# slyforce/MusicStyleTransfer

Hardware: AMD Instinct MI355X
Metric: piano-roll frames/s (VAE train step) (higher is better)
Workload: dtype bf16; 1 GPU; BASELINE configs[1]: single-track piano-roll VAE train step, T=256, pitch=128, latent=64, batch=64/GPU, bf16; encoder 256x2x8h, decoder 128x1x8h (scripts/train-vae.sh), dropout 0.2; Xavier-initialised weights; global_batch=64, seq_len=256, pitches=128, latent=64, parallelism=dp1, params=1885440

## Files before the change

### include/mst_hip.h

```cpp
#ifndef MST_HIP_H
#define MST_HIP_H

#include <stdint.h>

#ifdef __cplusplus
extern "C" {
#endif

typedef void* mst_stream_t;

enum mst_status {
  MST_OK = 0,
  MST_ERR_INVALID = -1,
  MST_ERR_LAUNCH = -2,
  MST_ERR_UNSUPPORTED = -3
};

enum mst_dtype { MST_BF16 = 0, MST_F16 = 1, MST_F32 = 2 };

enum mst_act { MST_ACT_NONE = 0, MST_ACT_RELU = 1 };

int mst_version(void);
const char* mst_last_error(void);

int mst_graph_begin(mst_stream_t stream);
int mst_graph_end(mst_stream_t stream, void** graph_exec_out);
int mst_graph_end_counted(mst_stream_t stream, void** graph_exec_out, int32_t* nodes_out, int32_t* kernel_nodes_out);
int mst_graph_launch(void* graph_exec, mst_stream_t stream);
int mst_graph_destroy(void* graph_exec);

int mst_event_create(void** ev_out);
int mst_event_record(void* ev, mst_stream_t stream);
int mst_event_sync(void* ev);
int mst_event_elapsed_ms(void* ev_start, void* ev_stop, float* ms_out);
int mst_event_destroy(void* ev);

typedef struct mst_gemm_args {
  int32_t dtype;
  int32_t c_f32;
  int64_t M, N, K;
  const void* A; int64_t lda;
  const void* B; int64_t ldb;
  void* C; int64_t ldc;
  const float* bias;
  const void* resid; int64_t ldr;
  int32_t act;
  const void* gate; int64_t ldg;
  float alpha;
  const float* rowadd; int64_t ldra; int64_t rowadd_period;
  const float* grpadd; int64_t ldga; const int32_t* grp_index;
  int64_t a_rows_per_group, a_group_stride, a_group_offset;
  int64_t c_rows_per_group, c_group_stride, c_group_offset;
  float dropout_p; uint64_t dropout_seed; uint32_t dropout_site;
  int32_t self_resid;
  const uint64_t* dropout_seed_ptr;
  int32_t a_u8;
  int32_t resid_phys;
} mst_gemm_args;

int mst_gemm_nt(const mst_gemm_args* args, mst_stream_t stream);
int mst_gemm_nt_form(const mst_gemm_args* args);

int mst_gemm_nt_pair(const mst_gemm_args* args0, const mst_gemm_args* args1, mst_stream_t stream);

typedef struct mst_bce_args {
  const uint8_t* labels;
  int64_t T;
  float label_smoothing;
  int32_t downweight;
  float* loss;
  void* probs; int64_t ldp;
  void* logits; int64_t ldl;
  float gscale;
  uint64_t* counts;
} mst_bce_args;
#define MST_ROLL_SLOTS 256
int mst_gemm_sigmoid_bce(const mst_gemm_args* args, const mst_bce_args* bce, mst_stream_t stream);

typedef struct mst_ln_args {
  int32_t mode;
  const float* gamma;
  const float* beta;
  float eps;
  void* out; int64_t ld_out;
  float* mean; float* rstd;
  const void* x; int64_t ld_x;
  float* dgamma; float* dbeta;
  int32_t mask_mode;
  float* partials;
} mst_ln_args;

int mst_gemm_nt_ln(const mst_gemm_args* args, const mst_ln_args* ln, mst_stream_t stream);
int mst_gemm_sigmoid_bce_dgrad_ln(const mst_gemm_args* args, const mst_bce_args* bce, const mst_gemm_args* dgrad,
                                  const mst_ln_args* ln, mst_stream_t stream);
int64_t mst_gemm_nt_ln_parts(int64_t M);
int mst_gemm_sigmoid_bce_form(const mst_gemm_args* args, const mst_bce_args* bce, const mst_gemm_args* dgrad, const mst_ln_args* ln,
                              int64_t* form);

int mst_ffn_ln_fwd(const mst_gemm_args* ff1, const mst_gemm_args* ff2, const mst_ln_args* ln, mst_stream_t stream);
int mst_ffn_ln_bwd(const mst_gemm_args* ff2_dgrad, const mst_gemm_args* ff1_dgrad, const mst_ln_args* ln, mst_stream_t stream);
typedef struct mst_ln_bwd_in {
  const void* dy; int64_t ld_dy;
  const void* x;  int64_t ld_x;
  const float* gamma; const float* mean; const float* rstd;
  void* dx; int64_t ld_dx;
  void* dx_masked; int64_t ld_dxm;
  float* dgamma; float* dbeta; float* partials;
  int32_t mask_mode;
  float dropout_p; uint64_t dropout_seed; const uint64_t* dropout_seed_ptr; uint32_t dropout_site;
} mst_ln_bwd_in;
int mst_ffn_ln_bwd_lead(const mst_ln_bwd_in* lead, const mst_gemm_args* ff2_dgrad, const mst_gemm_args* ff1_dgrad,
                        const mst_ln_args* ln, mst_stream_t stream);
int mst_proj_ffn_ln_fwd(const mst_gemm_args* proj, const mst_ln_args* ln1, const mst_gemm_args* ff1, const mst_gemm_args* ff2,
                        const mst_ln_args* ln2, mst_stream_t stream);
int mst_dec_tail_step(const mst_gemm_args* proj, const mst_ln_args* ln1, const mst_gemm_args* ff1, const mst_gemm_args* ff2,
                      const mst_ln_args* ln3, const mst_gemm_args* out, const mst_bce_args* bce, const mst_gemm_args* out_dgrad,
                      const mst_ln_args* ln3_bwd, const mst_gemm_args* ff2_dgrad, const mst_gemm_args* ff1_dgrad,
                      const mst_ln_args* ln1_bwd, mst_stream_t stream);

typedef struct mst_partial_sum {
  const float* src; int64_t n_parts; int64_t stride; int64_t len;
  float* dst; float scale;
} mst_partial_sum;
int mst_partial_sums(const mst_partial_sum* jobs, int n, mst_stream_t stream);

typedef struct mst_wgrad_args {
  int32_t dtype;
  int64_t M, N, K;
  const void* A; int64_t lda;
  const void* B; int64_t ldb;
  float* dW; int64_t ldw;
  float* db;
  float scale;
  int64_t a_rows_per_group, a_group_stride, a_group_offset;
  int64_t b_rows_per_group, b_group_stride, b_group_offset;
  int32_t a_u8;
} mst_wgrad_args;

typedef struct mst_outer_job {
  const float* L; const void* R; int32_t r_dtype; int64_t r_stride;
  int64_t B, J, I;
  float* out; float* obias;
} mst_outer_job;
int mst_outer_jobs(const mst_outer_job* jobs, int n, mst_stream_t stream);
int mst_gemm_wgrad_batch_flush(const mst_wgrad_args* list, int n, float* scratch, int64_t scratch_bytes,
                               const mst_partial_sum* sums, int n_sums, const mst_outer_job* outers, int n_outers,
                               mst_stream_t stream);
int mst_class_table_grad(const int32_t* classes, const float* tvec, float* dcls, int64_t ld_cls, int64_t B, int64_t Dd,
                         mst_stream_t stream);
int mst_gemm_wgrad_batch_flush_cls(const mst_wgrad_args* list, int n, float* scratch, int64_t scratch_bytes,
                                   const mst_partial_sum* sums, int n_sums, const mst_outer_job* outers, int n_outers,
                                   const int32_t* cls_classes, const float* cls_tvec, float* cls_dcls, int64_t cls_ld,
                                   int64_t cls_B, int64_t cls_Dd, mst_stream_t stream);
int mst_gemm_wgrad_plan(const mst_wgrad_args* list, int n, int64_t scratch_bytes, int64_t* plan);

int mst_embed_fwd(int dtype, int64_t B, int64_t T, int64_t D,
                  const int32_t* tokens, const float* table, int64_t ldt,
                  const int32_t* classes, const float* cls_table, int64_t ldc,
                  const float* pos, int64_t ldp, float alpha,
                  void* out, int64_t ld_out, int64_t S_out, int64_t s_off,
                  uint8_t* keymask, mst_stream_t stream);

int mst_embed_bwd(int dtype, int64_t B, int64_t T, int64_t D,
                  const int32_t* tokens, float* dtable, int64_t ldt,
                  const int32_t* classes, float* dcls, int64_t ldc, float alpha,
                  const void* dX, int64_t ld_dx, int64_t S_out, int64_t s_off,
                  mst_stream_t stream);

int mst_group_colsum(int dtype, int64_t B, int64_t T, int64_t D, const void* X, int64_t ldx,
                     int64_t S_out, int64_t s_off, const int32_t* idx, float* dst, int64_t ldd,
                     float alpha, mst_stream_t stream);

int mst_mask_from_lengths(int64_t B, int64_t S, const int32_t* lens, int32_t add,
                          uint8_t* keymask, mst_stream_t stream);

int mst_attn_keysoftmax_fwd(int dtype, int64_t B, int64_t S, int64_t H, int64_t dh,
                            const void* qkv, int64_t ld_qkv, int64_t k_off, int64_t q_off, int64_t v_off,
                            const uint8_t* keymask, float* lse,
                            void* out, int64_t ld_out,
                            int64_t q_limit ,
                            mst_stream_t stream);

int mst_attn_qkv_fwd(int dtype, int64_t B, int64_t S, int64_t H, int64_t dh, const void* x, int64_t ld_x, const void* w,
                     int64_t ld_w, const float* bias, void* qkv, int64_t ld_qkv, int64_t k_off, int64_t q_off, int64_t v_off,
                     const uint8_t* keymask, float* lse, void* out, int64_t ld_out, int64_t q_limit, mst_stream_t stream);
int mst_attn_keysoftmax_bwd(int dtype, int64_t B, int64_t S, int64_t H, int64_t dh,
                            const void* qkv, int64_t ld_qkv, int64_t k_off, int64_t q_off, int64_t v_off,
                            const uint8_t* keymask, const float* lse,
                            const void* dout, int64_t ld_dout,
                            void* dqkv, int64_t ld_dqkv, float* delta,
                            int64_t q_limit ,
                            mst_stream_t stream);
int mst_attn_proj_bwd(int dtype, int64_t B, int64_t S, int64_t H, int64_t dh, const void* qkv, int64_t ld_qkv, int64_t k_off,
                      int64_t q_off, int64_t v_off, const uint8_t* keymask, const float* lse, const void* dproj, int64_t ld_dproj,
                      const void* wt, int64_t ld_wt, void* dout_out, int64_t ld_dout, void* dqkv, int64_t ld_dqkv, float* delta,
                      mst_stream_t stream);

int mst_attn_fwd_form(int dtype, int64_t B, int64_t S, int64_t H, int64_t dh, int64_t ld_qkv, int64_t k_off, int64_t q_off,
                      int64_t v_off, int64_t ld_out, int64_t q_limit, int fused, int64_t ld_x, int64_t ld_w, int64_t* form);
int mst_attn_bwd_form(int dtype, int64_t B, int64_t S, int64_t H, int64_t dh, int64_t ld_qkv, int64_t k_off, int64_t q_off,
                      int64_t v_off, int64_t ld_dout, int64_t ld_dqkv, int64_t q_limit, int64_t* form);

int mst_attn_causal_fwd(int dtype, int64_t B, int64_t S, int64_t H, int64_t dh,
                        const void* qkv, int64_t ld_qkv, int64_t k_off, int64_t q_off, int64_t v_off,
                        const uint8_t* keymask, float* lse, void* out, int64_t ld_out, mst_stream_t stream);
int mst_attn_causal_bwd(int dtype, int64_t B, int64_t S, int64_t H, int64_t dh,
                        const void* qkv, int64_t ld_qkv, int64_t k_off, int64_t q_off, int64_t v_off,
                        const uint8_t* keymask, const float* lse, const void* dout, int64_t ld_dout,
                        void* dqkv, int64_t ld_dqkv, float* delta, mst_stream_t stream);

int mst_layernorm_fwd(int dtype, int64_t M, int64_t D, const void* x, int64_t ldx,
                      const float* gamma, const float* beta, float eps,
                      void* y, int64_t ldy, float* mean, float* rstd,
                      int64_t row_id_stride ,
                      mst_stream_t stream);

int mst_layernorm_bwd(int dtype, int64_t M, int64_t D, const void* x, int64_t ldx,
                      const float* gamma, const float* mean, const float* rstd,
                      const void* dy, int64_t ldy, void* dx, int64_t ld_dx,
                      void* dx_masked, int64_t ld_dxm, float* dgamma, float* dbeta,
                      int mask_mode, float dropout_p, uint64_t dropout_seed, uint32_t dropout_site,
                      const uint64_t* dropout_seed_ptr,
                      int64_t row_id_stride ,
                      float* partials ,
                      mst_stream_t stream);
int64_t mst_layernorm_bwd_parts(int64_t M, int64_t D);

int mst_latent_fwd(int dtype, int64_t B, int64_t De, int64_t Z, int64_t Dd,
                   const void* enc_out, int64_t enc_sample_stride,
                   const float* Wl, const float* bl, const float* eps,
                   const float* Wh, const float* bh,
                   const int32_t* classes, const float* cls_d, int64_t ld_cls,
                   const float* pos_d, float alpha_d,
                   float* mu, float* sigma, float* z, float* kl,
                   void* dec_in, int64_t dec_sample_stride, mst_stream_t stream);
int mst_latent_fwd_proj(int dtype, int64_t B, int64_t De, int64_t Z, int64_t Dd,
                        const void* enc_out, int64_t enc_sample_stride,
                        const float* Wl, const float* bl, const float* eps,
                        const float* Wh, const float* bh,
                        const int32_t* classes, const float* cls_d, int64_t ld_cls,
                        const float* pos_d, float alpha_d,
                        float* mu, float* sigma, float* z, float* kl,
                        void* dec_in, int64_t dec_sample_stride,
                        const void* Wq, int64_t ld_wq, const float* bq, void* qkv0, int64_t qkv_sample_stride, int64_t nq,
                        mst_stream_t stream);
int mst_latent_rows(int dtype, int64_t N, int64_t M, int64_t Z, int64_t Dd,
                    const float* zsrc, const float* ssrc, const int32_t* a, const int32_t* b, const float* w, int mode,
                    float tau, uint64_t seed, const uint64_t* seed_ptr, uint32_t site, int64_t row0,
                    const float* Wh, const float* bh,
                    const int32_t* ca, const int32_t* cb, const float* cw, const float* cls_d, int64_t ld_cls, int64_t n_classes,
                    const float* pos_d, float alpha_d,
                    float* z_out, void* dec_in, int64_t dec_stride, mst_stream_t stream);

int mst_latent_bwd_vec(int dtype, int64_t B, int64_t De, int64_t Z, int64_t Dd, const float* Wl, const float* eps, const float* Wh,
                       const int32_t* classes, const float* mu, const float* sigma, const void* d_dec_in, int64_t dec_sample_stride,
                       float alpha_d, float kl_weight, float gscale, float enc_scale, float* dcls_d, int64_t ld_cls,
                       void* d_enc_out, int64_t denc_sample_stride, float* scratch, mst_stream_t stream);
int mst_latent_bwd_vec_proj(int dtype, int64_t B, int64_t De, int64_t Z, int64_t Dd, const float* Wl, const float* eps, const float* Wh,
                            const int32_t* classes, const float* mu, const float* sigma,
                            const void* dq0, int64_t dq_sample_stride, const void* Wt, int64_t ld_wt, int64_t nq,
                            const void* resid0, int64_t resid_sample_stride,
                            float alpha_d, float kl_weight, float gscale, float enc_scale, float* dcls_d, int64_t ld_cls,
                            void* d_enc_out, int64_t denc_sample_stride, float* scratch, mst_stream_t stream);

int mst_latent_bwd_vec_sched(int dtype, int64_t B, int64_t De, int64_t Z, int64_t Dd, const float* Wl, const float* eps, const float* Wh,
                             const int32_t* classes, const float* mu, const float* sigma, const void* d_dec_in, int64_t dec_sample_stride,
                             float alpha_d, const float* sched, const float* kl, float gscale, float enc_scale, float* dcls_d,
                             int64_t ld_cls, void* d_enc_out, int64_t denc_sample_stride, float* scratch, mst_stream_t stream);
int mst_latent_bwd_vec_proj_sched(int dtype, int64_t B, int64_t De, int64_t Z, int64_t Dd, const float* Wl, const float* eps,
                                  const float* Wh, const int32_t* classes, const float* mu, const float* sigma,
                                  const void* dq0, int64_t dq_sample_stride, const void* Wt, int64_t ld_wt, int64_t nq,
                                  const void* resid0, int64_t resid_sample_stride,
                                  float alpha_d, const float* sched, const float* kl, float gscale, float enc_scale, float* dcls_d,
                                  int64_t ld_cls, void* d_enc_out, int64_t denc_sample_stride, float* scratch, mst_stream_t stream);

int mst_latent_form(int64_t De, int64_t Z, int64_t Dd, int64_t nq, const void* Wl, int64_t* form);

int mst_reparam_kl_fwd(int64_t B, int64_t Z, const float* mu, const float* sigma, const float* eps,
                       float* z, float* kl, mst_stream_t stream);
int mst_reparam_kl_bwd(int64_t B, int64_t Z, const float* mu, const float* sigma, const float* eps,
                       const float* dz, float kl_weight, float* dmu, float* dsigma, mst_stream_t stream);

typedef struct mst_row_tail_args {
  int32_t dtype;
  int64_t B, D;
  const void* att; int64_t rs_att;
  const void* resid; int64_t rs_res;
  const void* Wp; int64_t ldwp; const float* bp;
  const float* g1; const float* be1;
  const void* W1; int64_t ldw1; const float* b1;
  const void* W2; int64_t ldw2; const float* b2;
  const float* g2; const float* be2;
  void* h1; void* x1; void* h2; void* x2; int64_t rs_d;
  void* a; int64_t rs_a;
  float* mean1; float* rstd1; float* mean2; float* rstd2; int64_t stat_stride;
  float eps;
  float dropout_p; uint64_t dropout_seed; const uint64_t* dropout_seed_ptr; uint32_t site0;
  int64_t phys_stride;
  uint32_t* sync;
  uint32_t* status;
} mst_row_tail_args;
int mst_row_tail_fwd(const mst_row_tail_args* args, mst_stream_t stream);
int mst_row_tail_fwd_ride(const mst_row_tail_args* args, const mst_gemm_args* rider, uint32_t* queue, mst_stream_t stream);
int mst_row_tail_fwd_ride_shadows(const mst_row_tail_args* args, const mst_gemm_args* rider, uint32_t* queue, int sh_dtype,
                                  const float* sh_w, void* sh_wt16, const int64_t* sh_desc, const int64_t* sh_prefix, int64_t sh_n_mat,
                                  int64_t sh_tiles, mst_stream_t stream);
typedef struct mst_row_tail_bwd_args {
  int32_t dtype;
  int64_t B, D;
  const void* dy; int64_t rs_dy;
  const void* h2; const void* h1; int64_t rs_d;
  const void* a; int64_t rs_a;
  const float* mean1; const float* rstd1; const float* mean2; const float* rstd2; int64_t stat_stride;
  const float* g1; const float* g2;
  const void* W2t; int64_t ldw2t;
  const void* W1t; int64_t ldw1t;
  const void* Wpt; int64_t ldwpt;
  void* dh; void* dhm; void* dx1; void* dh1m; int64_t rs_c;
  void* dpre; int64_t rs_dpre;
  void* dh1; int64_t rs_dh1;
  void* datt; int64_t rs_datt;
  float* dg1; float* db1; float* dg2; float* db2;
  float dropout_p; uint64_t dropout_seed; const uint64_t* dropout_seed_ptr; uint32_t site0;
  int64_t phys_stride;
  uint32_t* sync;
  uint32_t* status;
} mst_row_tail_bwd_args;
int mst_row_tail_bwd(const mst_row_tail_bwd_args* args, mst_stream_t stream);
int mst_row_tail_bwd_ride(const mst_row_tail_bwd_args* args, const mst_gemm_args* rider, uint32_t* queue, mst_stream_t stream);
int mst_row_tail_form(int backward, int dtype, int64_t D, const mst_gemm_args* rider, int64_t sh_tiles, int64_t* form);

int mst_attn_decode(int dtype, int64_t B, int64_t H, int64_t dh, int64_t n_keys, int64_t t_max, const void* cache,
                    int64_t ld, int64_t k_off, int64_t q_off, int64_t v_off, int mode, void* out, int64_t ld_out,
                    mst_stream_t stream);

int mst_beam_step(int64_t B, int64_t K, int64_t V, int64_t i, int64_t L, const float* probs, int64_t ldp, const float* scores_in,
                  float* scores_out, const int32_t* seqs_in, int32_t* seqs_out, int32_t* hyp_src, int32_t* word, int32_t* active,
                  int32_t eos, int32_t pad, mst_stream_t stream);
int mst_beam_gather(const void* in, void* out, const int32_t* src, int64_t N, int64_t n_rows, int64_t row_bytes, int64_t t_max,
                    mst_stream_t stream);
int mst_beam_gather_cols(const void* in, void* out, const int32_t* src, int64_t N, int64_t n_rows, int64_t row_bytes, int64_t t_max,
                         int64_t skip_begin, int64_t skip_bytes, mst_stream_t stream);
int mst_sample_step(int64_t N, int64_t V, int64_t i, int64_t L, const float* probs, int64_t ldp, int32_t* seqs, float* scores,
                    int32_t* word, int32_t* active, uint64_t seed, int32_t eos, int32_t pad, mst_stream_t stream);
int mst_frame_step(int dtype, int64_t N, int64_t P, int64_t i, int64_t L, const void* logits, int64_t ldl, float tau, int mode, float thr,
                   const uint64_t* seed_ptr, uint8_t* frames, int64_t ldf, uint8_t* roll, int64_t ldr, float* scores, float* probs_out,
                   mst_stream_t stream);
int mst_token_step(int dtype, int64_t N, int64_t V, int64_t i, int64_t L, const void* logits, int64_t ldl, float tau, int32_t top_k,
                   float top_p, const uint64_t* seed_ptr, int32_t* seqs, float* scores, int32_t* word, int32_t* active,
                   int32_t* kept_out, int32_t eos, int32_t pad, mst_stream_t stream);

#define MST_CE_MAX_WORKGROUPS 4096
int mst_softmax_ce(int dtype, int64_t B, int64_t T, int64_t V,
                   const void* logits, int64_t ld, const int32_t* labels,
                   float* loss, float* probs, int64_t ldp,
                   void* dlogits, int64_t ldd, float gscale,
                   int pre_zeroed ,
                   float* tok_parts, int top_k, mst_stream_t stream);

int mst_ce_from_probs(int dtype, int64_t B, int64_t T, int64_t V, const void* probs, int64_t ldp,
                      const int32_t* labels, float* loss, mst_stream_t stream);
int mst_bce_from_probs(int dtype, int64_t B, int64_t n_per_sample, const void* probs, const uint8_t* labels,
                       float label_smoothing, int downweight, float* loss, mst_stream_t stream);

int mst_sigmoid_bce(int dtype, int64_t B, int64_t T, int64_t P,
                    const void* logits, int64_t ld, const uint8_t* labels,
                    float label_smoothing, int downweight, int32_t* npos,
                    float* loss, void* probs, int64_t ldp,
                    void* dlogits, int64_t ldd, float gscale,
                    int pre_zeroed , mst_stream_t stream);
int mst_sigmoid_bce_counts(int dtype, int64_t B, int64_t T, int64_t P,
                           const void* logits, int64_t ld, const uint8_t* labels,
                           float label_smoothing, int downweight, int32_t* npos,
                           float* loss, void* probs, int64_t ldp,
                           void* dlogits, int64_t ldd, float gscale,
                           int pre_zeroed, uint64_t* counts, mst_stream_t stream);
int mst_sigmoid_bce_form(int dtype, int64_t B, int64_t T, int64_t P,
                         const void* logits, int64_t ld, const uint8_t* labels,
                         float label_smoothing, int downweight, int32_t* npos,
                         float* loss, void* probs, int64_t ldp,
                         void* dlogits, int64_t ldd, float gscale,
                         int pre_zeroed, int64_t* form);

int mst_loss_combine(int64_t B, const float* recon, const float* kl, float kl_weight,
                     float* total, float* metric_acc, mst_stream_t stream);

typedef struct mst_step_metrics {
  int64_t B; const float* recon; const float* kl; float kl_weight; float* total; float* metric;
  uint32_t* status; const uint32_t* expect_ptr0; uint32_t expect_val0; const uint32_t* expect_ptr1; uint32_t expect_val1;
  const float* fin_recon; const float* fin_kl; int64_t fin_B;
} mst_step_metrics;
#define MST_TAIL_SPIN_FWD 1u
#define MST_TAIL_SPIN_BWD 2u
#define MST_STEP_INCOMPLETE 16u
int mst_adam_flat(int dtype, int64_t n, float* w, const float* grad, float* m, float* v,
                  void* w16, double lr, double beta1, double beta2, float eps, float wd,
                  float rescale, float clip, int32_t* step_state ,
                  int advance_step ,
                  const mst_step_metrics* metrics, mst_stream_t stream);
int mst_loss_combine_v(const mst_step_metrics* metrics, mst_stream_t stream);

int mst_adam_flat_emb(int dtype, int64_t n, float* w, const float* grad, float* m, float* v, void* w16, double lr, double beta1,
                      double beta2, float eps, float wd, float rescale, float clip, int32_t* step_state,
                      const mst_step_metrics* metrics, int64_t base, const int64_t* emb, int64_t n_emb, void* wt16, mst_stream_t stream);

int mst_adam_flat_sched(int dtype, int64_t n, float* w, const float* grad, float* m, float* v, void* w16, double lr, double beta1,
                        double beta2, float eps, float wd, float rescale, float clip, int32_t* step_state,
                        const mst_step_metrics* metrics, const float* sched, mst_stream_t stream);
int mst_adam_flat_emb_sched(int dtype, int64_t n, float* w, const float* grad, float* m, float* v, void* w16, double lr, double beta1,
                            double beta2, float eps, float wd, float rescale, float clip, int32_t* step_state,
                            const mst_step_metrics* metrics, const float* sched, int64_t base, const int64_t* emb, int64_t n_emb,
                            void* wt16, mst_stream_t stream);

int64_t mst_grad_sumsq_parts(void);
int mst_grad_sumsq(int64_t n, const float* grad, int64_t cut, float rescale_lo, float rescale_hi, float* parts, mst_stream_t stream);
// ... 46 lines not shown
```

### musicstyletransfer_amd/csrc/ffn_ln.hip

```cpp
#include "ffn_ln.hpp"
#include "gemm_checks.hpp"

namespace mst {

template <typename T, int BN, int WGM, int WGN, int MODE, bool LEAD, bool FULL, bool EXTRA = false>
__global__ __launch_bounds__(WGM * WGN * 64) void ffn_ln_kernel(mst_gemm_args g1, mst_gemm_args g2, mst_ln_args ln, mst_ln_bwd_in lead,
                                                                mst_gemm_args gx, mst_ln_args lnx) {
  extern __shared__ __attribute__((aligned(16))) unsigned char smem[];
  ffn_ln_body<T, BN, WGM, WGN, MODE, LEAD, FULL, EXTRA>(smem, g1, g2, ln, lead, gx, lnx, nullptr, [] {});
}

template <typename T, int BN>
static int launch_ffn_ln(const mst_gemm_args& g1, const mst_gemm_args& g2, const mst_ln_args& ln, const mst_ln_bwd_in* lead, hipStream_t s,
                         const mst_gemm_args* gx = nullptr, const mst_ln_args* lnx = nullptr) {
  constexpr int BM = 64;
  const int ex = gx ? 1 : 0;
  const size_t lds_loop = (size_t)2 * BN * 64 * 2 + (size_t)2 * BM * (BN + 8) * 2 + (size_t)g1.N * 4 + (size_t)6 * BN * 4;
  const size_t lds_epi = (size_t)BM * (BN + 4) * 4;
  const size_t lds = lds_loop > lds_epi ? lds_loop : lds_epi;
  const int full = g1.M % BM == 0 ? 1 : 0;
  const int mi = ex ? 6 + full : (lead ? 2 : (ln.mode == 2 ? 1 : 0)) * 2 + full;
  typedef void (*kern_t)(mst_gemm_args, mst_gemm_args, mst_ln_args, mst_ln_bwd_in, mst_gemm_args, mst_ln_args);
  const kern_t fns[8] = {&ffn_ln_kernel<T, BN, 2, 4, 1, false, false>, &ffn_ln_kernel<T, BN, 2, 4, 1, false, true>,
                         &ffn_ln_kernel<T, BN, 2, 4, 2, false, false>, &ffn_ln_kernel<T, BN, 2, 4, 2, false, true>,
                         &ffn_ln_kernel<T, BN, 2, 4, 2, true, false>, &ffn_ln_kernel<T, BN, 2, 4, 2, true, true>,
                         &ffn_ln_kernel<T, BN, 2, 4, 1, false, false, true>, &ffn_ln_kernel<T, BN, 2, 4, 1, false, true, true>};
  static size_t granted[8] = {64 * 1024, 64 * 1024, 64 * 1024, 64 * 1024, 64 * 1024, 64 * 1024, 64 * 1024, 64 * 1024};
  if (const int rc = lds_opt_in(reinterpret_cast<const void*>(fns[mi]), lds, &granted[mi], "ffn_ln_kernel")) return rc;
  const mst_ln_bwd_in none = {};
  const mst_gemm_args no_gemm = {};
  const mst_ln_args no_ln = {};
  hipLaunchKernelGGL(fns[mi], dim3((unsigned)cdiv(g1.M, BM)), dim3(512), lds, s, g1, g2, ln, lead ? *lead : none,
                     gx ? *gx : no_gemm, lnx ? *lnx : no_ln);
  MST_CHECK_LAUNCH("ffn_ln_kernel");
  return MST_OK;
}

int check_ffn_ln(const char* who, const mst_gemm_args* first, const mst_gemm_args* second, const mst_ln_args* ln, int mode,
                 const mst_ln_bwd_in* lead, const mst_gemm_args* extra, const mst_ln_args* extra_ln) {
  MST_CHECK_ARG(first != nullptr && second != nullptr && ln != nullptr, "%s: null args", who);
  const mst_gemm_args& a = *first;
  const mst_gemm_args& b = *second;
  const mst_ln_args& l = *ln;
  int rc = check_gemm_common(a);
  if (rc) return rc;
  rc = check_gemm_common(b);
  if (rc) return rc;
  MST_CHECK_ARG(a.dtype == b.dtype && a.M == b.M, "%s: the two GEMMs must share dtype and M", who);
  MST_CHECK_ARG((b.N == 256 || b.N == 128) && a.K == b.N, "%s: the model width (first K = second N) must be 128 or 256 (got %lld, %lld)", who,
                (long long)a.K, (long long)b.N);
  MST_CHECK_ARG(a.N == b.K && a.N % b.N == 0, "%s: the hidden width (first N = second K) must be a multiple of the model width", who);
  MST_CHECK_ARG(b.A == a.C && b.lda == a.ldc, "%s: the second GEMM's A operand must be the first one's output (it is consumed on chip)", who);
  MST_CHECK_ARG(!a.c_f32 && !b.c_f32 && !b.gate && !a.rowadd && !b.rowadd && !a.grpadd && !b.grpadd && !a.resid && !a.self_resid &&
                b.act == MST_ACT_NONE && a.c_rows_per_group <= 0 && b.a_rows_per_group <= 0 && b.c_rows_per_group <= 0,
                "%s: fp32 outputs, row-indexed adds, row remaps, a gate or activation on the second GEMM and a residual on the first are not supported", who);
  MST_CHECK_ARG(a.a_rows_per_group <= 0 || (a.a_rows_per_group % 64 == 0 && a.M % a.a_rows_per_group == 0 && a.a_group_offset >= 0 &&
                                            a.a_group_stride >= a.a_rows_per_group + a.a_group_offset && a.M < (1ll << 31)),
                "%s: row groups must be whole 64-row tiles (rows per group %lld, stride %lld, offset %lld, M %lld)", who,
                (long long)a.a_rows_per_group, (long long)a.a_group_stride, (long long)a.a_group_offset, (long long)a.M);
  MST_CHECK_ARG(a.lda % 8 == 0 && a.ldc % 8 == 0 && a.ldc >= a.N && b.ldc % 8 == 0 && b.ldc >= b.N, "%s: leading dimensions must be multiples of 8", who);
  MST_CHECK_ARG((uint64_t)a.N * (uint64_t)a.ldb < (1ull << 32) && (uint64_t)b.N * (uint64_t)b.ldb < (1ull << 32), "%s: weight matrices too large", who);
  MST_CHECK_ARG(!b.resid || (b.ldr % 8 == 0 && b.ldr >= b.N && (uintptr_t)b.resid % 16 == 0), "%s: bad residual layout", who);
  MST_CHECK_ARG(!a.bias || (uintptr_t)a.bias % 16 == 0, "%s: the first GEMM's bias must be 16-byte aligned", who);
  MST_CHECK_ARG(a.dropout_p == 0.f || a.N % 4 == 0, "%s: dropout needs widths that are multiples of 4", who);
  MST_CHECK_ARG(l.mode == mode && l.gamma && l.mean && l.rstd, "%s: LayerNorm arguments of the wrong form", who);
  if (mode == 1) {
    MST_CHECK_ARG(!a.gate, "%s: a gate belongs to the backward form", who);
    MST_CHECK_ARG(l.beta && l.out && l.ld_out % 8 == 0 && l.ld_out >= b.N && (uintptr_t)l.out % 16 == 0,
                  "%s: the LayerNorm arguments are those of mst_gemm_nt_ln's forward form", who);
  } else {
    MST_CHECK_ARG(a.gate && a.ldg % 8 == 0 && a.ldg >= a.N && (uintptr_t)a.gate % 16 == 0, "%s: the first GEMM needs the forward activation as its gate", who);
    MST_CHECK_ARG(a.act == MST_ACT_NONE && a.dropout_p == 0.f && !b.self_resid, "%s: activation / dropout / self_resid belong to the forward form", who);
    MST_CHECK_ARG(l.x && l.ld_x % 8 == 0 && (uintptr_t)l.x % 16 == 0 && (l.partials || (l.dgamma && l.dbeta)) && (uintptr_t)l.partials % 16 == 0,
                  "%s: backward needs x and dgamma + dbeta (or partials)", who);
    MST_CHECK_ARG(l.mask_mode >= 0 && l.mask_mode <= 2 &&
                  (l.mask_mode != 1 || (l.out && l.ld_out % 8 == 0 && l.ld_out >= b.N && (uintptr_t)l.out % 16 == 0)),
                  "%s: mask_mode must be 0, 1 (with out) or 2", who);
  }
  if (lead) {
    const mst_ln_bwd_in& q = *lead;
    MST_CHECK_ARG(mode == 2, "%s: a leading LayerNorm belongs to the backward form", who);
    MST_CHECK_ARG(q.dy && q.x && q.gamma && q.mean && q.rstd && q.dx && (q.partials || (q.dgamma && q.dbeta)), "%s: leading LayerNorm: null pointer", who);
    MST_CHECK_ARG(q.ld_dy % 8 == 0 && q.ld_x % 8 == 0 && q.ld_dx % 8 == 0 && q.ld_dy >= b.N && q.ld_x >= b.N && q.ld_dx >= b.N &&
                  ((uintptr_t)q.dy | (uintptr_t)q.x | (uintptr_t)q.dx | (uintptr_t)q.partials) % 16 == 0, "%s: leading LayerNorm: bad layout", who);
    MST_CHECK_ARG(q.mask_mode == 0 || (q.mask_mode == 1 && q.dx_masked && q.ld_dxm % 8 == 0 && q.ld_dxm >= b.N && (uintptr_t)q.dx_masked % 16 == 0),
                  "%s: leading LayerNorm: mask_mode must be 0 or 1 (with dx_masked)", who);
    MST_CHECK_ARG(q.dropout_p >= 0.f && q.dropout_p < 1.f, "%s: leading LayerNorm: dropout_p must be in [0,1)", who);
    const void* tile = q.mask_mode == 1 ? q.dx_masked : q.dx;
    const int64_t tile_ld = q.mask_mode == 1 ? q.ld_dxm : q.ld_dx;
    MST_CHECK_ARG(a.A == tile && a.lda == tile_ld, "%s: the first GEMM's A operand must be the leading LayerNorm's (masked) output", who);
  }
  if (extra) {
    const mst_gemm_args& x = *extra;
    rc = check_gemm_common(x);
    if (rc) return rc;
    MST_CHECK_ARG(x.dtype == a.dtype && x.M == a.M && x.N == b.N && x.K == b.N, "%s: the extra GEMM is width x width on the same rows", who);
    MST_CHECK_ARG(!x.c_f32 && !x.gate && !x.rowadd && !x.grpadd && x.act == MST_ACT_NONE && x.a_rows_per_group <= 0 && x.c_rows_per_group <= 0 &&
                  x.ldc % 8 == 0 && x.ldc >= x.N && (uint64_t)x.N * (uint64_t)x.ldb < (1ull << 32),
                  "%s: the extra GEMM takes no gate, activation, row-indexed add or row remap", who);
    MST_CHECK_ARG(mode == 1 && extra_ln != nullptr, "%s: the projection (with its LayerNorm) rides in front of the forward form", who);
    const mst_ln_args& q = *extra_ln;
    MST_CHECK_ARG(q.mode == 1 && q.gamma && q.beta && q.mean && q.rstd && q.out == a.A && q.ld_out == a.lda,
                  "%s: the leading LayerNorm's output must be the first GEMM's A operand", who);
    MST_CHECK_ARG(!x.resid || (x.ldr % 8 == 0 && x.ldr >= x.N && (uintptr_t)x.resid % 16 == 0), "%s: bad residual layout", who);
  }
  return MST_OK;
}

}

using namespace mst;

static int ffn_ln_impl(const char* who, const mst_gemm_args* first, const mst_gemm_args* second, const mst_ln_args* ln, int mode,
                       mst_stream_t stream, const mst_ln_bwd_in* lead = nullptr, const mst_gemm_args* extra = nullptr,
                       const mst_ln_args* extra_ln = nullptr) {
  const int rc = check_ffn_ln(who, first, second, ln, mode, lead, extra, extra_ln);
  if (rc) return rc;
  const mst_gemm_args &a = *first, &b = *second;
  const mst_ln_args& l = *ln;
  hipStream_t s = (hipStream_t)stream;
  return dispatch_act(a.dtype, [&](auto tag) -> int {
    typedef decltype(tag) T;
    if (b.N == 256) return launch_ffn_ln<T, 256>(a, b, l, lead, s, extra, extra_ln);
    return launch_ffn_ln<T, 128>(a, b, l, lead, s, extra, extra_ln);
  });
}

extern "C" int mst_proj_ffn_ln_fwd(const mst_gemm_args* proj, const mst_ln_args* ln1, const mst_gemm_args* ff1, const mst_gemm_args* ff2,
                                   const mst_ln_args* ln2, mst_stream_t stream) {
  MST_CHECK_ARG(proj != nullptr && ln1 != nullptr, "mst_proj_ffn_ln_fwd: null args");
  return ffn_ln_impl("mst_proj_ffn_ln_fwd", ff1, ff2, ln2, 1, stream, nullptr, proj, ln1);
}

extern "C" int mst_ffn_ln_bwd_lead(const mst_ln_bwd_in* lead, const mst_gemm_args* ff2_dgrad, const mst_gemm_args* ff1_dgrad,
                                   const mst_ln_args* ln, mst_stream_t stream) {
  MST_CHECK_ARG(lead != nullptr, "mst_ffn_ln_bwd_lead: null args");
  return ffn_ln_impl("mst_ffn_ln_bwd_lead", ff2_dgrad, ff1_dgrad, ln, 2, stream, lead);
}

extern "C" int mst_ffn_ln_fwd(const mst_gemm_args* ff1, const mst_gemm_args* ff2, const mst_ln_args* ln, mst_stream_t stream) {
  return ffn_ln_impl("mst_ffn_ln_fwd", ff1, ff2, ln, 1, stream);
}
extern "C" int mst_ffn_ln_bwd(const mst_gemm_args* ff2_dgrad, const mst_gemm_args* ff1_dgrad, const mst_ln_args* ln, mst_stream_t stream) {
  return ffn_ln_impl("mst_ffn_ln_bwd", ff2_dgrad, ff1_dgrad, ln, 2, stream);
}

#ifdef MST_FFN_STAMPS
extern "C" int mst_debug_ffn_stamps(uint64_t* host_out) {
  return hipMemcpyFromSymbol(host_out, HIP_SYMBOL(mst::g_ffn_stamps), sizeof(uint64_t) * (8 + 48 * 4)) == hipSuccess ? 0 : -1;
}
#endif
```

### musicstyletransfer_amd/csrc/ffn_ln.hpp

```cpp
#pragma once
#include <type_traits>
#include "gemm_ln.hpp"

namespace mst {

template <typename T, int BN, int WGM, int WGN, int MODE, bool LEAD, bool FULL, bool EXTRA, bool X_IN_LDS = false, bool KEEP_OUT = false,
          bool PAR_READY = false, typename Hook>
__device__ __forceinline__ void ffn_ln_body(unsigned char* smem, mst_gemm_args g1, mst_gemm_args g2, const mst_ln_args ln,
                                            const mst_ln_bwd_in lead, mst_gemm_args gx, const mst_ln_args lnx, float* par,
                                            Hook&& before_epilogue) {
  constexpr bool HEAD = EXTRA;
  static_assert(!(X_IN_LDS && (LEAD || EXTRA)), "a tile left in LDS is the block's own input");
  static_assert(!EXTRA || MODE == 1, "the extra GEMM is the forward form's head");
  constexpr int BM = 64, BK = 64, CHUNKS = BK / 8;
  constexpr int NT = WGM * WGN * 64;
  constexpr int WTM = BM / WGM, WTN = BN / WGN, TM = WTM / 16, TN = WTN / 16;
  constexpr int B_CH = BN * CHUNKS / NT;
  constexpr int LDA = BN + 8;
  constexpr int KST = BN / BK;
  static_assert(BN * CHUNKS % NT == 0 && (BM * BN / 8) % NT == 0, "tile/threads mismatch");
  typedef typename Act<T>::vec8 vec8;
  u32x4* sB = reinterpret_cast<u32x4*>(smem);
  T* sH = reinterpret_cast<T*>(smem + (size_t)2 * BN * BK * 2);
  T* sX = sH + BM * LDA;
  float* sBias1 = PAR_READY ? par : reinterpret_cast<float*>(sX + BM * LDA);
  float* sPar = sBias1 + g1.N;
  const int tid = threadIdx.x, lane = tid & 63, wave = tid >> 6;
  const int wm = wave / WGN, wn = wave % WGN, frow = lane & 15, fq = lane >> 4;
  int64_t m0 = xcd_chunk(blockIdx.x, gridDim.x) * BM;
  if (g1.a_rows_per_group > 0) {
    const uint32_t grp = (uint32_t)m0 / (uint32_t)g1.a_rows_per_group;
    m0 += (int64_t)grp * (g1.a_group_stride - g1.a_rows_per_group) + g1.a_group_offset;
    g1.M = g2.M = gx.M = (g1.M / g1.a_rows_per_group) * g1.a_group_stride;
  }
  const int64_t F = g1.N;
  FFN_STAMP(0); FFN_RT(190);
  const int64_t Mg = FULL ? (int64_t)1 << 62 : g1.M;
  if constexpr (!PAR_READY)
  for (int i = tid * 4; i < (int)F; i += NT * 4)
    *reinterpret_cast<f32x4*>(sBias1 + i) = g1.bias ? *reinterpret_cast<const f32x4*>(g1.bias + i) : f32x4{0.f, 0.f, 0.f, 0.f};
  const uint64_t seed2 = g2.dropout_seed ^ ((g2.dropout_p > 0.f && g2.dropout_seed_ptr) ? g2.dropout_seed_ptr[0] : 0ull);
  const uint64_t seedx = EXTRA ? gx.dropout_seed ^ ((gx.dropout_p > 0.f && gx.dropout_seed_ptr) ? gx.dropout_seed_ptr[0] : 0ull) : 0ull;
  if constexpr (!PAR_READY)
  for (int i = tid; i < BN; i += NT) {
    sPar[i] = g2.bias ? g2.bias[i] : 0.f;
    sPar[BN + i] = ln.gamma[i];
    sPar[2 * BN + i] = (MODE == 1) ? ln.beta[i] : 0.f;
    if constexpr (HEAD) {
      sPar[3 * BN + i] = gx.bias ? gx.bias[i] : 0.f;
      sPar[4 * BN + i] = lnx.gamma[i];
      sPar[5 * BN + i] = lnx.beta[i];
    }
  }
  const int n_chunks = (int)(F / BN);
  const int rot = (int)((blockIdx.x / 8) % (unsigned)n_chunks);
  auto phys = [&](int c) { const int pc = c + rot; return pc >= n_chunks ? pc - n_chunks : pc; };
  const T* __restrict__ W1 = reinterpret_cast<const T*>(g1.B);
  const T* __restrict__ W2 = reinterpret_cast<const T*>(g2.B);
  const T* __restrict__ WX = reinterpret_cast<const T*>(gx.B);

  uint32_t off1[B_CH], off2[B_CH], offx[B_CH];
  int b_lds[B_CH];
#pragma unroll
  for (int i = 0; i < B_CH; ++i) {
    const int c = tid + i * NT;
    const int row = c / CHUNKS, ch = c % CHUNKS;
    off1[i] = (uint32_t)row * (uint32_t)g1.ldb + (uint32_t)ch * 8u;
    off2[i] = (uint32_t)row * (uint32_t)g2.ldb + (uint32_t)ch * 8u;
    offx[i] = EXTRA ? (uint32_t)row * (uint32_t)gx.ldb + (uint32_t)ch * 8u : 0u;
    b_lds[i] = row * CHUNKS + (ch ^ (row & 7));
  }
  constexpr int SPC = 2 * KST;
  constexpr int RING = BN >= 256 ? 4 : 2, AHEAD = RING - 1;
  static_assert(SPC % RING == 0, "ring slots must repeat per chunk");
  u32x4 ring[RING][B_CH];
  auto load_stage = [&](int c, int s, u32x4 (&rb)[B_CH]) {
    if (HEAD && c < 0) {
      const T* base = WX + s * BK;
#pragma unroll
      for (int i = 0; i < B_CH; ++i) rb[i] = *reinterpret_cast<const u32x4*>(base + offx[i]);
    } else if (s < KST) {
      const T* base = W1 + (int64_t)phys(c) * BN * g1.ldb + s * BK;
#pragma unroll
      for (int i = 0; i < B_CH; ++i) rb[i] = *reinterpret_cast<const u32x4*>(base + off1[i]);
    } else {
      const T* base = W2 + (int64_t)phys(c) * BN + (s - KST) * BK;
#pragma unroll
      for (int i = 0; i < B_CH; ++i) rb[i] = *reinterpret_cast<const u32x4*>(base + off2[i]);
    }
  };
  auto load_piece = [&](int c, int s, u32x4 (&rb)[B_CH], auto ic) {
    constexpr int i = decltype(ic)::value;
    const T* base;
    uint32_t off;
    if (HEAD && c < 0) { base = WX + s * BK; off = offx[i]; }
    else if (s < KST) { base = W1 + (int64_t)phys(c) * BN * g1.ldb + s * BK; off = off1[i]; }
    else { base = W2 + (int64_t)phys(c) * BN + (s - KST) * BK; off = off2[i]; }
    rb[i] = *reinterpret_cast<const u32x4*>(base + off);
  };
  auto store_stage = [&](int buf, const u32x4 (&rb)[B_CH]) {
#pragma unroll
    for (int i = 0; i < B_CH; ++i) sB[buf * BN * CHUNKS + b_lds[i]] = rb[i];
  };
  {
    auto pro = [&](auto jc) {
      constexpr int j = decltype(jc)::value;
      if constexpr (HEAD) {
        static_assert(!HEAD || AHEAD <= KST, "the head GEMM's stages cover the prologue");
        if (j < AHEAD) load_stage(-1, j, ring[j % RING]);
      } else {
        if (j < AHEAD && (j < SPC || n_chunks > 1)) load_stage(j / SPC, j % SPC, ring[j % RING]);
      }
    };
    pro(std::integral_constant<int, 0>()); pro(std::integral_constant<int, 1>()); pro(std::integral_constant<int, 2>());
    pro(std::integral_constant<int, 3>()); pro(std::integral_constant<int, 4>()); pro(std::integral_constant<int, 5>());
    pro(std::integral_constant<int, 6>());
    static_assert(AHEAD <= 7, "the prologue list covers seven stages");
  }
  if constexpr (LEAD) {
    constexpr int CPR = BN / 8, RSTEP = NT / CPR, ITERS = BM / RSTEP;
    const int ch = tid % CPR, nc = ch * 8, row0 = tid / CPR;
    const float inv_n = 1.f / (float)BN;
    const bool has_drop = lead.dropout_p > 0.f && lead.mask_mode == 1;
    const uint64_t dseed = lead.dropout_seed ^ ((has_drop && lead.dropout_seed_ptr) ? lead.dropout_seed_ptr[0] : 0ull);
    const uint32_t dkey = dropout_key(dseed, lead.dropout_site), dthr = dropout_thr(lead.dropout_p);
    const float inv_keep = dropout_inv_keep(lead.dropout_p);
    float gam8[8], dg8[8], db8[8];
#pragma unroll
    for (int e = 0; e < 8; ++e) { gam8[e] = lead.gamma[nc + e]; dg8[e] = 0.f; db8[e] = 0.f; }
    u32x4 dyv[ITERS], xv[ITERS];
    float mean_r[ITERS], rstd_r[ITERS];
#pragma unroll
    for (int it = 0; it < ITERS; ++it) {
      const int64_t m = m0 + row0 + it * RSTEP;
      dyv[it] = u32x4{0u, 0u, 0u, 0u}; xv[it] = dyv[it]; mean_r[it] = 0.f; rstd_r[it] = 0.f;
      if (m < Mg) {
        dyv[it] = *reinterpret_cast<const u32x4*>(reinterpret_cast<const T*>(lead.dy) + m * lead.ld_dy + nc);
        xv[it] = *reinterpret_cast<const u32x4*>(reinterpret_cast<const T*>(lead.x) + m * lead.ld_x + nc);
        mean_r[it] = lead.mean[m];
        rstd_r[it] = lead.rstd[m];
      }
    }
#pragma unroll
    for (int it = 0; it < ITERS; ++it) {
      const int row = row0 + it * RSTEP;
      const int64_t m = m0 + row;
      Pack8 db, xb;
      db.u = dyv[it]; xb.u = xv[it];
      float xh[8], g[8], s1 = 0.f, s2 = 0.f;
#pragma unroll
      for (int e = 0; e < 8; ++e) {
        const float d = bits_to_f32<T>(db.h[e]);
        xh[e] = (bits_to_f32<T>(xb.h[e]) - mean_r[it]) * rstd_r[it];
        g[e] = d * gam8[e];
        s1 += g[e];
        s2 += g[e] * xh[e];
        dg8[e] += d * xh[e];
        db8[e] += d;
      }
      s1 = row_sum<CPR>(s1) * inv_n;
      s2 = row_sum<CPR>(s2) * inv_n;
      uint32_t keep8 = 0xFFu;
      if (has_drop) {
        const uint64_t w = (uint64_t)(m * BN + nc) >> 2;
        keep8 = dropout_keep4k(dkey, w, dthr) | (dropout_keep4k(dkey, w + 1, dthr) << 4);
      }
      Pack8 ob, mb;
#pragma unroll
      for (int e = 0; e < 8; ++e) {
        const float o = rstd_r[it] * (g[e] - s1 - xh[e] * s2);
        const float k = has_drop ? (((keep8 >> e) & 1u) ? inv_keep : 0.f) : 1.f;
        ob.h[e] = f32_to_bits<T>(o);
        mb.h[e] = f32_to_bits<T>(o * k);
      }
      if (m < Mg) {
        *reinterpret_cast<u32x4*>(reinterpret_cast<T*>(lead.dx) + m * lead.ld_dx + nc) = ob.u;
        if (lead.mask_mode == 1) *reinterpret_cast<u32x4*>(reinterpret_cast<T*>(lead.dx_masked) + m * lead.ld_dxm + nc) = mb.u;
      }
      *reinterpret_cast<u32x4*>(sX + row * LDA + nc) = (m < Mg) ? (lead.mask_mode == 1 ? mb.u : ob.u) : u32x4{0u, 0u, 0u, 0u};
    }
    float* red = reinterpret_cast<float*>(smem);
    static_assert((size_t)2 * RSTEP * BN * 4 <= (size_t)2 * BN * BK * 2, "reduction scratch must fit the weight stages");
#pragma unroll
    for (int e = 0; e < 8; ++e) {
      red[row0 * BN + nc + e] = dg8[e];
      red[(RSTEP + row0) * BN + nc + e] = db8[e];
    }
    __syncthreads();
    for (int c = tid; c < 2 * BN; c += NT) {
      const int which = c / BN, col = c % BN;
      float sm = 0.f;
      for (int r = 0; r < RSTEP; ++r) sm += red[(which * RSTEP + r) * BN + col];
      if (lead.partials) lead.partials[(int64_t)blockIdx.x * 2 * BN + c] = sm;
      else atomicAdd((which ? lead.dbeta : lead.dgamma) + col, sm);
    }
    __syncthreads();
  } else if constexpr (!X_IN_LDS)
  {
    const T* X = reinterpret_cast<const T*>(HEAD ? gx.A : g1.A);
    const int64_t ldx = HEAD ? gx.lda : g1.lda;
    constexpr int CPR = BN / 8;
#pragma unroll
    for (int i = 0; i < BM * CPR / NT; ++i) {
      const int c = tid + i * NT, row = c / CPR, ch = c % CPR;
      u32x4 v = {0u, 0u, 0u, 0u};
      if (m0 + row < Mg) v = *reinterpret_cast<const u32x4*>(X + (m0 + row) * ldx + ch * 8);
      *reinterpret_cast<u32x4*>(sX + row * LDA + ch * 8) = v;
    }
  }
  auto mma_stage = [&](f32x4 (&acc)[TN][TM], const T* sA, int buf, const u32x4 (&rb)[B_CH], auto&& hook) {
    const u32x4* cB = sB + buf * BN * CHUNKS;
#pragma unroll
    for (int ks = 0; ks < BK / 32; ++ks) {
      vec8 xf[TM], wf[TN];
      const int kc = ks * 4 + fq;
#pragma unroll
      for (int i = 0; i < TM; ++i)
        xf[i] = __builtin_bit_cast(vec8, *reinterpret_cast<const u32x4*>(sA + (wm * WTM + i * 16 + frow) * LDA + kc * 8));
#pragma unroll
      for (int j = 0; j < TN; ++j) {
        const int row = wn * WTN + j * 16 + frow;
        wf[j] = __builtin_bit_cast(vec8, cB[row * CHUNKS + (kc ^ (row & 7))]);
      }
      auto row = [&](auto jc) {
        constexpr int j = decltype(jc)::value;
        if constexpr (j < TN) {
#pragma unroll
          for (int i = 0; i < TM; ++i) acc[j][i] = Act<T>::mfma16(wf[j], xf[i], acc[j][i]);
          if (ks == 0) hook(std::integral_constant<int, j>()); else hook(std::integral_constant<int, TN + j>());
        }
      };
      static_assert(TN <= 4, "row list");
      row(std::integral_constant<int, 0>()); row(std::integral_constant<int, 1>());
      row(std::integral_constant<int, 2>()); row(std::integral_constant<int, 3>());
    }
  };
  auto no_hook = [](auto) {};

  f32x4 acc1[TN][TM], acc2[TN][TM];
#pragma unroll
  for (int j = 0; j < TN; ++j)
#pragma unroll
    for (int i = 0; i < TM; ++i) acc2[j][i] = f32x4{0.f, 0.f, 0.f, 0.f};
  const float p1 = g1.dropout_p;
  const bool drop1 = MODE == 1 && p1 > 0.f;
  const uint64_t seed1 = g1.dropout_seed ^ ((drop1 && g1.dropout_seed_ptr) ? g1.dropout_seed_ptr[0] : 0ull);
  const uint32_t dkey1 = dropout_key(seed1, g1.dropout_site), dthr1 = dropout_thr(p1);
  const float inv_keep1 = dropout_inv_keep(p1);
  const bool idx32 = (uint64_t)g1.M * (uint64_t)F < (1ull << 32);
  const bool relu1 = MODE == 1 && g1.act == MST_ACT_RELU;
  const bool step_form1 = MODE == 1 && relu1 && drop1 && idx32 && g1.alpha == 1.f;
  uint32_t rowmul[TM];
#pragma unroll
  for (int i = 0; i < TM; ++i) rowmul[i] = (uint32_t)(m0 + wm * WTM + i * 16 + frow) * (uint32_t)(F >> 1) * DROPOUT_MUL;
  T* Aout = reinterpret_cast<T*>(g1.C);

  auto extra_gemm = [&](int cx) {
#pragma unroll
    for (int j = 0; j < TN; ++j)
#pragma unroll
      for (int i = 0; i < TM; ++i) acc1[j][i] = f32x4{0.f, 0.f, 0.f, 0.f};
    store_stage(0, ring[0]);
    __syncthreads();
    auto xstage = [&](auto sc) {
      constexpr int s = decltype(sc)::value;
      if constexpr (s < KST) {
        constexpr int t = s + AHEAD;
        if constexpr (t < KST) load_stage(cx, t, ring[t % RING]);
        else if constexpr (HEAD) load_stage(0, t - KST, ring[t % RING]);
        mma_stage(acc1, sX + s * BK, s & 1, ring[s % RING], no_hook);
        if constexpr (s + 1 < KST) store_stage((s + 1) & 1, ring[(s + 1) % RING]);
        __syncthreads();
      }
    };
    static_assert(!EXTRA || (KST <= 4 && KST % RING == 0), "the extra GEMM stage list / ring slots");
    xstage(std::integral_constant<int, 0>()); xstage(std::integral_constant<int, 1>());
    xstage(std::integral_constant<int, 2>()); xstage(std::integral_constant<int, 3>());
  };
  if constexpr (HEAD) {
    extra_gemm(-1);
    gemm_epilogue_ln<T, BM, BN, WGM, WGN, 1>(gx, lnx, smem, acc1, m0, nullptr, 0, sX, LDA, sPar + 3 * BN, &seedx);
    __syncthreads();
  }
  store_stage(0, ring[0]);
  __syncthreads();
  FFN_STAMP(1);
  for (int c = 0; c < n_chunks; ++c) {
    const int pc = phys(c);
#pragma unroll
    for (int j = 0; j < TN; ++j)
#pragma unroll
      for (int i = 0; i < TM; ++i) acc1[j][i] = f32x4{0.f, 0.f, 0.f, 0.f};
    constexpr int OUT_CH = BM * (BN / 8) / NT;
    u32x4 gv[OUT_CH];
    if constexpr (MODE == 2) {
      const T* G = reinterpret_cast<const T*>(g1.gate);
#pragma unroll
      for (int i = 0; i < OUT_CH; ++i) {
        const int cc = tid + i * NT, row = cc / (BN / 8), ch = cc % (BN / 8);
        gv[i] = u32x4{0u, 0u, 0u, 0u};
        if (m0 + row < Mg) gv[i] = *reinterpret_cast<const u32x4*>(G + (m0 + row) * g1.ldg + (int64_t)pc * BN + ch * 8);
      }
    }
    auto stage = [&](auto sc) {
      constexpr int s = decltype(sc)::value;
      if constexpr (s < SPC) {
        constexpr bool IL = BN >= 256 && B_CH <= 2 * TN;
        constexpr int t = s + AHEAD;
        const int tc = t < SPC ? c : (c + 1 < n_chunks ? c + 1 : c);
        const bool more = s + 1 < SPC || c + 1 < n_chunks;
        auto piece = [&](auto kc) {
          constexpr int k = decltype(kc)::value;
          if constexpr (IL && k < B_CH) {
            __builtin_amdgcn_sched_barrier(0);
            load_piece(tc, t % SPC, ring[t % RING], kc);
            if (more) sB[((s + 1) & 1) * BN * CHUNKS + b_lds[k]] = ring[(s + 1) % RING][k];
            __builtin_amdgcn_sched_barrier(0);
          }
        };
        if constexpr (!IL) load_stage(tc, t % SPC, ring[t % RING]);
        FFN_STAMP(8 + (c * SPC + s) * 4);
        if constexpr (s < KST) mma_stage(acc1, sX + s * BK, s & 1, ring[s % RING], piece);
        else mma_stage(acc2, sH + (s - KST) * BK, s & 1, ring[s % RING], piece);
        FFN_STAMP(8 + (c * SPC + s) * 4 + 1);
        if constexpr (s == KST - 1) {
          auto chunk_epilogue = [&](auto step_form) {
            constexpr bool STEP = decltype(step_form)::value;
            const uint32_t cmul = ((uint32_t)pc * (BN / 2) + (uint32_t)((wn * WTN + fq * 4) / 2)) * DROPOUT_MUL;
#pragma unroll
            for (int j = 0; j < TN; ++j) {
              const int n = wn * WTN + j * 16 + fq * 4;
              const int64_t col = (int64_t)pc * BN + n;
              const f32x4 b4 = *reinterpret_cast<const f32x4*>(sBias1 + col);
#pragma unroll
              for (int i = 0; i < TM; ++i) {
                const int row = wm * WTM + i * 16 + frow;
                float tv[4];
                if constexpr (STEP) {
#pragma unroll
                  for (int e = 0; e < 4; ++e) tv[e] = fmaxf(acc1[j][i][e] + b4[e], 0.f);
                  dropout_apply4_pre(dkey1, rowmul[i] + cmul + (uint32_t)(j * 8) * DROPOUT_MUL, dthr1, inv_keep1, tv);
                } else {
#pragma unroll
                  for (int e = 0; e < 4; ++e) {
                    tv[e] = (acc1[j][i][e] + b4[e]) * g1.alpha;
                    if (relu1) tv[e] = fmaxf(tv[e], 0.f);
                  }
                  if (drop1) dropout_apply4(dkey1, (uint64_t)((m0 + row) * F + col) >> 2, dthr1, inv_keep1, tv);
                }
                uint16_t hb[4];
#pragma unroll
                for (int e = 0; e < 4; ++e) hb[e] = f32_to_bits<T>(tv[e]);
                *reinterpret_cast<u32x2*>(sH + row * LDA + n) =
                    u32x2{(uint32_t)hb[0] | ((uint32_t)hb[1] << 16), (uint32_t)hb[2] | ((uint32_t)hb[3] << 16)};
              }
            }
          };
          if (step_form1) chunk_epilogue(std::true_type()); else chunk_epilogue(std::false_type());
        }
        if (!IL && more) store_stage((s + 1) & 1, ring[(s + 1) % RING]);
        FFN_STAMP(8 + (c * SPC + s) * 4 + 2);
        __syncthreads();
        FFN_STAMP(8 + (c * SPC + s) * 4 + 3);
        if constexpr (s == KST - 1) {
          constexpr int CPR = BN / 8;
#pragma unroll
          for (int i = 0; i < BM * CPR / NT; ++i) {
            const int cc = tid + i * NT, row = cc / CPR, ch = cc % CPR;
            u32x4 v = *reinterpret_cast<const u32x4*>(sH + row * LDA + ch * 8);
            if constexpr (MODE == 2) {
              Pack8 pv, pg;
              pv.u = v; pg.u = gv[i];
#pragma unroll
              for (int e = 0; e < 8; ++e)
                if (!(bits_to_f32<T>(pg.h[e]) > 0.f)) pv.h[e] = 0;
              v = pv.u;
              *reinterpret_cast<u32x4*>(sH + row * LDA + ch * 8) = v;
            }
            if (m0 + row < Mg) *reinterpret_cast<u32x4*>(Aout + (m0 + row) * g1.ldc + (int64_t)pc * BN + ch * 8) = v;
          }
          if constexpr (MODE == 2) __syncthreads();
        }
      }
    };
    static_assert(SPC <= 8, "the stage list below covers eight stages per chunk");
    stage(std::integral_constant<int, 0>()); stage(std::integral_constant<int, 1>());
    stage(std::integral_constant<int, 2>()); stage(std::integral_constant<int, 3>());
    stage(std::integral_constant<int, 4>()); stage(std::integral_constant<int, 5>());
    stage(std::integral_constant<int, 6>()); stage(std::integral_constant<int, 7>());
  }
  const bool resid_is_x = g2.resid == g1.A && g2.ldr == g1.lda;
  FFN_STAMP(2);
  before_epilogue();
  gemm_epilogue_ln<T, BM, BN, WGM, WGN, MODE>(g2, ln, smem, acc2, m0, resid_is_x ? sX : nullptr, LDA, KEEP_OUT ? sX : nullptr, KEEP_OUT ? LDA : 0,
                                              sPar, &seed2);
  FFN_STAMP(3); FFN_RT(191);
}

}
```

### musicstyletransfer_amd/csrc/runtime.hip

```cpp
#include <stdarg.h>
#include <string.h>
#include "common.hpp"

namespace mst {
static thread_local char g_err[512] = "";
void set_error(const char* fmt, ...) {
  va_list ap;
  va_start(ap, fmt);
  vsnprintf(g_err, sizeof(g_err), fmt, ap);
  va_end(ap);
}
}

using namespace mst;

extern "C" int mst_version(void) { return 115; }
extern "C" const char* mst_last_error(void) { return g_err; }

#define HIP_TRY(expr)                                             \
  do {                                                            \
    hipError_t e__ = (expr);                                      \
    if (e__ != hipSuccess) {                                      \
      set_error("%s: %s", #expr, hipGetErrorString(e__));         \
      return MST_ERR_LAUNCH;                                      \
    }                                                             \
  } while (0)

extern "C" int mst_graph_begin(mst_stream_t stream) {
  HIP_TRY(hipStreamBeginCapture((hipStream_t)stream, hipStreamCaptureModeThreadLocal));
  return MST_OK;
}
static hipError_t count_nodes(hipGraph_t g, int32_t* nodes_out, int32_t* kernel_nodes_out) {
  size_t n = 0;
  hipError_t e = hipGraphGetNodes(g, nullptr, &n);
  if (e != hipSuccess) return e;
  int32_t kernels = 0;
  if (n > 0 && kernel_nodes_out) {
    hipGraphNode_t* nodes = new hipGraphNode_t[n];
    e = hipGraphGetNodes(g, nodes, &n);
    for (size_t i = 0; e == hipSuccess && i < n; ++i) {
      hipGraphNodeType t;
      e = hipGraphNodeGetType(nodes[i], &t);
      kernels += (e == hipSuccess && t == hipGraphNodeTypeKernel);
    }
    delete[] nodes;
    if (e != hipSuccess) return e;
  }
  if (nodes_out) *nodes_out = (int32_t)n;
  if (kernel_nodes_out) *kernel_nodes_out = kernels;
  return hipSuccess;
}

extern "C" int mst_graph_end(mst_stream_t stream, void** graph_exec_out) {
  return mst_graph_end_counted(stream, graph_exec_out, nullptr, nullptr);
}
extern "C" int mst_graph_end_counted(mst_stream_t stream, void** graph_exec_out, int32_t* nodes_out, int32_t* kernel_nodes_out) {
  MST_CHECK_ARG(graph_exec_out != nullptr, "mst_graph_end: null output");
  hipGraph_t g = nullptr;
  HIP_TRY(hipStreamEndCapture((hipStream_t)stream, &g));
  hipError_t ec = (nodes_out || kernel_nodes_out) ? count_nodes(g, nodes_out, kernel_nodes_out) : hipSuccess;
  if (ec != hipSuccess) {
    (void)hipGraphDestroy(g);
    set_error("hipGraphGetNodes: %s", hipGetErrorString(ec));
    return MST_ERR_LAUNCH;
  }
  hipGraphExec_t ge = nullptr;
  hipError_t e = hipGraphInstantiate(&ge, g, nullptr, nullptr, 0);
  (void)hipGraphDestroy(g);
  if (e != hipSuccess) {
    set_error("hipGraphInstantiate: %s", hipGetErrorString(e));
    return MST_ERR_LAUNCH;
  }
  *graph_exec_out = (void*)ge;
  return MST_OK;
}
extern "C" int mst_graph_launch(void* graph_exec, mst_stream_t stream) {
  HIP_TRY(hipGraphLaunch((hipGraphExec_t)graph_exec, (hipStream_t)stream));
  return MST_OK;
}
extern "C" int mst_graph_destroy(void* graph_exec) {
  if (graph_exec) HIP_TRY(hipGraphExecDestroy((hipGraphExec_t)graph_exec));
  return MST_OK;
}

extern "C" int mst_event_create(void** ev_out) {
  MST_CHECK_ARG(ev_out != nullptr, "mst_event_create: null output");
  hipEvent_t ev;
  HIP_TRY(hipEventCreate(&ev));
  *ev_out = (void*)ev;
  return MST_OK;
}
extern "C" int mst_event_record(void* ev, mst_stream_t stream) {
  HIP_TRY(hipEventRecord((hipEvent_t)ev, (hipStream_t)stream));
  return MST_OK;
}
extern "C" int mst_event_sync(void* ev) {
  HIP_TRY(hipEventSynchronize((hipEvent_t)ev));
  return MST_OK;
}
extern "C" int mst_event_elapsed_ms(void* a, void* b, float* ms_out) {
  HIP_TRY(hipEventElapsedTime(ms_out, (hipEvent_t)a, (hipEvent_t)b));
  return MST_OK;
}
extern "C" int mst_event_destroy(void* ev) {
  if (ev) HIP_TRY(hipEventDestroy((hipEvent_t)ev));
  return MST_OK;
}

__global__ void selftest_kernel(int32_t* flags) {
  __shared__ __bf16 tile[32 * 32];
  const int l = threadIdx.x;
  auto Aval = [](int i, int k) { return (float)(((i * 3 + k * 5) % 7) - 3); };
  auto Bval = [](int k, int j) { return (float)(((k * 2 + j * 7) % 5) - 2); };

  {
    bf16x8 a, b;
    for (int j = 0; j < 8; ++j) {
      a[j] = (__bf16)Aval(l & 15, 8 * (l >> 4) + j);
      b[j] = (__bf16)Bval(8 * (l >> 4) + j, l & 15);
    }
    f32x4 d = {0, 0, 0, 0};
    d = __builtin_amdgcn_mfma_f32_16x16x32_bf16(a, b, d, 0, 0, 0);
    int ok = 1;
    for (int r = 0; r < 4; ++r) {
      int row = 4 * (l >> 4) + r, col = l & 15;
      float ref = 0;
      for (int k = 0; k < 32; ++k) ref += Aval(row, k) * Bval(k, col);
      ok &= (d[r] == ref);
    }
    ok = __all(ok);
    if (l == 0) flags[0] = ok;
  }
  f32x16 X;
  {
    bf16x8 a, b;
    for (int j = 0; j < 8; ++j) {
      a[j] = (__bf16)Aval(l & 31, 8 * (l >> 5) + j);
      b[j] = (__bf16)Bval(8 * (l >> 5) + j, l & 31);
    }
    f32x16 d;
    for (int r = 0; r < 16; ++r) d[r] = 0;
    d = __builtin_amdgcn_mfma_f32_32x32x16_bf16(a, b, d, 0, 0, 0);
    int ok = 1;
    for (int r = 0; r < 16; ++r) {
      int row = (r & 3) + 8 * (r >> 2) + 4 * (l >> 5), col = l & 31;
      float ref = 0;
      for (int k = 0; k < 16; ++k) ref += Aval(row, k) * Bval(k, col);
      ok &= (d[r] == ref);
    }
    ok = __all(ok);
    if (l == 0) flags[1] = ok;
    X = d;
  }
  auto Tval = [](int r, int c) { return (float)((r * 37 + c * 11) % 251); };
  for (int i = l; i < 32 * 32; i += 64) tile[i] = (__bf16)Tval(i / 32, i % 32);
  __syncthreads();
  {
    int g_i = l & 15, q = g_i >> 2, p = g_i & 3;
    int r0 = 8 + 4 * (l >> 5), c0 = 16 * ((l >> 4) & 1);
    const __bf16* addr = &tile[(r0 + q) * 32 + c0 + 4 * p];
    i16x4 v = __builtin_amdgcn_ds_read_tr16_b64_v4i16(
        (__attribute__((address_space(3))) i16x4*)(uintptr_t)(addr));
    int ok = 1;
    for (int e = 0; e < 4; ++e) {
      uint16_t bits = (uint16_t)v[e];
      float got = bits_to_f32<__bf16>(bits);
      ok &= (got == Tval(r0 + e, c0 + g_i));
    }
    ok = __all(ok);
    if (l == 0) flags[2] = ok;
  }
  {
    auto B2 = [](int r, int n) { return (float)(((r * 3 + n * 2) % 3) - 1); };
    f32x16 y;
    for (int r = 0; r < 16; ++r) y[r] = 0;
    for (int s = 0; s < 2; ++s) {
      bf16x8 a, b;
      for (int j = 0; j < 8; ++j) {
        a[j] = (__bf16)X[8 * s + j];
        int xr = 16 * s + 8 * (j >> 2) + 4 * (l >> 5) + (j & 3);
        b[j] = (__bf16)B2(xr, l & 31);
      }
      y = __builtin_amdgcn_mfma_f32_32x32x16_bf16(a, b, y, 0, 0, 0);
    }
    int ok = 1;
    for (int r = 0; r < 16; ++r) {
      int c = (r & 3) + 8 * (r >> 2) + 4 * (l >> 5), n = l & 31;
      float ref = 0;
      for (int xr = 0; xr < 32; ++xr) {
        float x = 0;
        for (int k = 0; k < 16; ++k) x += Aval(xr, k) * Bval(k, c);
        ref += x * B2(xr, n);
      }
      ok &= (y[r] == ref);
    }
    ok = __all(ok);
    if (l == 0) flags[3] = ok;
  }
}

extern "C" int mst_selftest(int32_t* out_flags_device, mst_stream_t stream) {
  MST_CHECK_ARG(out_flags_device != nullptr, "mst_selftest: null output");
  hipLaunchKernelGGL(selftest_kernel, dim3(1), dim3(64), 0, (hipStream_t)stream, out_flags_device);
  MST_CHECK_LAUNCH("selftest_kernel");
  return MST_OK;
}
```

### musicstyletransfer_amd/engine.py

```python
import contextlib
import math
import os
import warnings
from collections import OrderedDict, namedtuple

import numpy as np
import torch

from . import ops as o
from ._lib import CE_MAX_WORKGROUPS, ROLL_SLOTS
from .ops import roundup


class VAEConfig:

    def __init__(self, kind, in_dim, out_dim, num_classes, latent_dim, e_model, e_layers, e_heads, d_model, d_layers,
                 d_heads, e_dropout=0.0, d_dropout=0.0, d_causal=False):
        assert kind in ("token", "pianoroll")
        assert e_model % e_heads == 0 and d_model % d_heads == 0
        self.kind = kind
        self.in_dim, self.out_dim = in_dim, out_dim
        self.num_classes, self.latent_dim = num_classes, latent_dim
        self.e_model, self.e_layers, self.e_heads = e_model, e_layers, e_heads
        self.d_model, self.d_layers, self.d_heads = d_model, d_layers, d_heads
# ... 149 lines not shown
        self.tail_checked = False
        self.tail_policy = os.environ.get("MST_TAIL_FAILURE", "fallback")
        self.tail_failures = []
        self._tail_listeners = []
        self._rng_state_infer = None
        self.tok_parts = torch.zeros(CE_MAX_WORKGROUPS, 4, **f32) if cfg.kind == "token" else None
        self.roll_counts = torch.zeros(ROLL_SLOTS, 4, dtype=torch.int64, device=device) if cfg.kind == "pianoroll" else None
        if params_np is None:
            params_np = xavier_init(cfg, np.random.default_rng(seed))
        self.load_numpy(params_np)

    def rng_state(self, seed=0):
        if self._rng_state is None:
            self._rng_state = torch.tensor([0, 0, seed ^ 0x5DEECE66D, 0], dtype=torch.int64, device=self.device)
        return self._rng_state

    def grad_parts(self):
        if self._grad_parts is None:
            self._grad_parts = torch.zeros(o.grad_sumsq_parts(), dtype=torch.float32, device=self.device)
        return self._grad_parts

    def enable_ema(self):
        if self.ema is None:
            self.ema = self.w.clone()
        return self.ema

    def swap_ema(self):
        if self.ema is None:
            raise RuntimeError("this store keeps no average of its weights (StepPlan(ema_decay=...) / enable_ema())")
        o.ema_swap(self.w, self.ema, self.w16)
        self.refresh_shadows()
        self.ema_swapped = not self.ema_swapped

    @contextlib.contextmanager
    def ema_weights(self):
        self.swap_ema()
        try:
            yield self
        finally:
            self.swap_ema()

    def rng_state_inference(self):
        if self._rng_state_infer is None:
            self._rng_state_infer = torch.tensor([0, 0, 0x1F123BB5 ^ 0x5DEECE66D, 0], dtype=torch.int64, device=self.device)
        return self._rng_state_infer

    def on_tail_failure(self, callback):
        self._tail_listeners.append(callback)

    def handle_step_status(self, flags, skipped):
        o.zero(self._metric_buf[4:6])
        self.tail_failures.append((int(flags), int(skipped)))
        self.tail_fused = False
        msg = (f"the one-launch position-0 tail of the top encoder layer failed (status flags {int(flags):#x}: "
               f"{'forward barrier timed out; ' if flags & 1 else ''}{'backward barrier timed out; ' if flags & 2 else ''}"
               f"{'tail incomplete at the end of a step; ' if flags & 16 else ''}"
               f"{int(skipped)} step(s) skipped without touching the model)")
        if self.tail_policy == "raise":
            raise RuntimeError(msg + " — MST_TAIL_FAILURE=raise")
        warnings.warn(msg + "; falling back to the five-launch form for the rest of the run", RuntimeWarning)
        for cb in self._tail_listeners:
            cb()

    def poll_status(self, reduce=None):
        if getattr(self, "_poll_host", None) is None:
            self._poll_host = torch.zeros(2, dtype=torch.float32).pin_memory()
            self._poll_dev = torch.zeros(2, dtype=torch.float32, device=self.device)
            self._poll_event = torch.cuda.Event()
            self._poll_pending = False
        handled = False
        if self._poll_pending and self._poll_event.query():
            self._poll_pending = False
            flags, skipped = (int(v) for v in self._poll_host.tolist())
            if flags or skipped:
                if reduce is not None:
                    self.tail_fused = False
                    raise RuntimeError(f"a one-launch position-0 tail failed on at least one rank (status words summed over the ranks: "
                                       f"{flags}, {skipped} skipped step(s)); the replicas are no longer identical — restart from the "
                                       "last checkpoint with MST_ROW_TAIL=0")
                cur = self.step_status[:2].tolist()
                self.handle_step_status(cur[0] or flags, cur[1] or skipped)
                handled = True
        if not self._poll_pending:
            self._poll_dev.copy_(self.step_status[:2])
            if reduce is not None:
                reduce(self._poll_dev)
            self._poll_host.copy_(self._poll_dev, non_blocking=True)
            self._poll_event.record()
            self._poll_pending = True
        return handled

    def read_metrics(self, reset=True):
        buf = self._metric_buf.cpu()
        acc = buf[:3].tolist()
        flags, skipped, nonfinite = buf[4:7].view(torch.int32).tolist()
        if nonfinite:
            self.nonfinite_steps += int(nonfinite)
            o.zero(self._metric_buf[6:7])
            warnings.warn(f"{int(nonfinite)} training step(s) skipped: a per-sample loss was not finite (an fp16 activation overflow or "
                          "sigma = 0 under log(sigma^2)); parameters, moments and the step count were left as they were", RuntimeWarning)
        if flags or skipped:
            self.handle_step_status(flags, skipped)
        out = {"kl_sum": acc[0], "total_sum": acc[1], "count": acc[2], "skipped_steps": skipped, "nonfinite_steps": int(nonfinite)}
        beta_t, _, f_lr, sched_t = buf[8:12].tolist()
        if sched_t > 0:
            out.update(kl_weight=beta_t, lr_scale=f_lr)
        _, _, norm_sum, norm_max, g_steps, g_clipped = buf[12:18].tolist()
        if g_steps > 0:
            out.update(grad_norm=norm_sum / g_steps, grad_norm_max=norm_max, clip_frac=g_clipped / g_steps)
        if self.tok_parts is not None:
            t = self.tok_parts.cpu().double().sum(0).tolist()
            out.update(nll_sum=t[0], acc_hits=t[1], topk_hits=t[2], n_tokens=t[3])
        if self.roll_counts is not None:
            c = self.roll_counts.cpu().sum(0).tolist()
            out.update(roll_tp=int(c[0]), roll_pred=int(c[1]), roll_pos=int(c[2]), roll_cells=int(c[3]))
        if reset:
            o.zero(self.metric_acc)
            if g_steps > 0:
                o.zero(self.gstat[2:6])
            if self.tok_parts is not None:
                o.zero(self.tok_parts)
            if self.roll_counts is not None:
                o.zero(self.roll_counts)
        return out

    def wgrad_scratch(self, n_floats=16 * 1024 * 1024 + 256 * 256):
        for t in self._wgrad_scratch:
            if t.numel() >= n_floats:
                return t
        t = torch.empty(n_floats, dtype=torch.float32, device=self.device)
        self._wgrad_scratch.append(t)
        return t

    def _view(self, flat, name):
        shape = self.shapes[name]
        off = self.offsets[name]
        return flat[off: off + int(np.prod(shape))].view(*shape)

    def p(self, name):
        return self._view(self.w, name)

    def grad(self, name):
        return self._view(self.g, name)

    def h(self, name):
        return self._view(self.w16, name)

    def fused(self, flat, prefix, what):
        D = self.shapes[f"{prefix}.att.W_k.weight"][0]
        off = self.offsets[f"{prefix}.att.W_k.{what}"]
        return flat[off: off + 3 * D * D].view(3 * D, D) if what == "weight" else flat[off: off + 3 * D]

    def t(self, name):
        so, r, c = self.t_specs[name]
        off = self.t_off[name]
        return self.wt16[off: off + c * roundup(r, 8)].view(c, roundup(r, 8))

    def _layer_params(self, side, i):
        pre = f"{side}.layer{i}"

        def dense(name):
            w, b = f"{pre}.{name}.weight", f"{pre}.{name}.bias"
            return Dense(self.h(w), self.p(b), self.t(w), self.grad(w), self.grad(b))

        def norm(name):
            g, b = f"{pre}.{name}.gamma", f"{pre}.{name}.beta"
            return Norm(self.p(g), self.p(b), self.grad(g), self.grad(b), f"{pre}.{name}")

        kqv = Dense(self.fused(self.w16, pre, "weight"), self.fused(self.w, pre, "bias"), self.t(f"{pre}.att.W_kqv"),
                    self.fused(self.g, pre, "weight"), self.fused(self.g, pre, "bias"))
        dec = side == "decoder"
        return LayerParams(kqv, dense("att.W_proj"), dense("ff1"), dense("ff2"), norm("ln1"), norm("ln3" if dec else "ln2"),
                           self_resid=dec, mask_mode=2 if dec else 1)

    def layer(self, side, i):
        return self._layers[side, i]

    def load_numpy(self, params_np):
        host = np.zeros(self.n, np.float32)
        for name, shape in self.shapes.items():
            a = np.asarray(params_np[name], np.float32)
            assert tuple(a.shape) == tuple(shape), f"{name}: expected {shape}, got {a.shape}"
            host[self.offsets[name]: self.offsets[name] + a.size] = a.reshape(-1)
        self.w.copy_(torch.from_numpy(host))
        self.refresh_shadows()

    def to_numpy(self, which="w"):
        if which == "ema" and self.ema is None:
            raise RuntimeError("this store keeps no average of its weights (StepPlan(ema_decay=...) / enable_ema())")
        host = getattr(self, which).detach().cpu().numpy()
        return OrderedDict((n, host[self.offsets[n]: self.offsets[n] + int(np.prod(s))].reshape(s).copy())
                           for n, s in self.shapes.items())

    def shadowed_names(self):
        names = set()
        for key in self.t_specs:
            if key.endswith(".att.W_kqv"):
                p = key[: -len("W_kqv")]
                names.update({p + "W_k.weight", p + "W_q.weight", p + "W_v.weight"})
            else:
                names.add(key)
        return names

    def as_consumed_numpy(self):
        w = self.to_numpy("w")
        w16 = self.w16.detach().float().cpu().numpy()
        for n in self.shadowed_names():
            s = self.shapes[n]
            w[n] = w16[self.offsets[n]: self.offsets[n] + int(np.prod(s))].reshape(s).copy()
        return w

    def load_ema_numpy(self, params_np=None):
        self.enable_ema()
        if params_np is None:
            self.ema.copy_(self.w)
            return
        host = np.zeros(self.n, np.float32)
        for name, shape in self.shapes.items():
            a = np.asarray(params_np[name], np.float32)
            assert tuple(a.shape) == tuple(shape), f"{name}: expected {shape}, got {a.shape}"
            host[self.offsets[name]: self.offsets[name] + a.size] = a.reshape(-1)
        self.ema.copy_(torch.from_numpy(host))

    def refresh_shadows(self):
        o.cast_to_act(self.w, self.w16)
        o.transpose_shadows(self.w, self.wt16, self.t_desc, self.t_prefix, len(self.t_specs), self.t_tiles)


class _Layer:
    pass


Dense = namedtuple("Dense", "w b t dw db")
Norm = namedtuple("Norm", "gamma beta dgamma dbeta site")
LayerParams = namedtuple("LayerParams", "kqv proj ff1 ff2 ln1 ln2 self_resid mask_mode")

Rows = namedtuple("Rows", "view c_remap ln")
ALL_ROWS = Rows(lambda buf: buf, (0, 0, 0), {})


def position0_rows(B, S):
    return Rows(lambda buf: buf.view(B, S, -1)[:, 0, :], (1, S, 0), dict(M=B, row_id_stride=S))


class Dropout(namedtuple("Dropout", "p seed_ptr site0")):

    def at(self, k):
        return dict(dropout_p=self.p, dropout_site=self.site0 + k, dropout_seed_ptr=self.seed_ptr) if self.p > 0 else {}


NO_DROPOUT = Dropout(0.0, None, 0)


def row_block_fwd(P, L, x_in, rows, drop, form, row_groups=None, tail=None, launch=True):
    D, v = P.proj.w.shape[0], rows.view
    if form == "tail":
        o.row_tail_fwd(v(L.att), v(x_in), P.proj.w, P.proj.b, P.ln1.gamma, P.ln1.beta, P.ff1.w, P.ff1.b, P.ff2.w, P.ff2.b, P.ln2.gamma,
                       P.ln2.beta, v(L.h1), v(L.x1), v(L.a), v(L.h2), v(L.x2), L.mean1, L.rstd1, L.mean2, L.rstd2, dropout_p=drop.p,
                       dropout_seed_ptr=drop.seed_ptr, site0=drop.site0, **tail)
        return L.x2
    proj = dict(N=D, K=D, bias=P.proj.b, resid=v(x_in), **drop.at(0))
    ff1 = dict(K=D, bias=P.ff1.b, act=o.ACT_RELU, **drop.at(1))
    ff2 = dict(K=4 * D, bias=P.ff2.b, **drop.at(2))
    ff2.update(dict(self_resid=True) if P.self_resid else dict(resid=v(L.x1)))
    if form == "fused":
        head = dict(att=L.att, W=P.proj.w, h1=L.h1, gamma=P.ln1.gamma, beta=P.ln1.beta, mean=L.mean1, rstd=L.rstd1, **proj)
        kw = dict(x=L.x1, W1=P.ff1.w, a_out=L.a, W2=P.ff2.w, h_out=L.h2, gamma=P.ln2.gamma, beta=P.ln2.beta, y_out=L.x2, mean=L.mean2,
                  rstd=L.rstd2, ff1=ff1, ff2=ff2, proj=head, row_groups=row_groups)
        if not launch:
            return kw
        o.ffn_ln_fwd(**kw)
        return L.x2
    o.gemm_nt(v(L.att), P.proj.w, L.h1, c_remap=rows.c_remap, **proj)
    o.layernorm_fwd(v(L.h1), P.ln1.gamma, P.ln1.beta, v(L.x1), L.mean1, L.rstd1, D=D, **rows.ln)
    o.gemm_nt(v(L.x1), P.ff1.w, L.a, c_remap=rows.c_remap, **ff1)
    o.gemm_nt(v(L.a), P.ff2.w, L.h2, c_remap=rows.c_remap, **ff2)
    o.layernorm_fwd(v(L.h2), P.ln2.gamma, P.ln2.beta, v(L.x2), L.mean2, L.rstd2, D=D, **rows.ln)
    return L.x2


def _lead_mask(P, t, drop):
    if P.mask_mode == 2:
        return dict(mask_mode=2, **drop.at(2))
    return dict(mask_mode=1, dx_masked=t.dhm, **drop.at(2)) if drop.p > 0 else {}


def no_partials(norm, parts):
    return None


def ffn_bwd_parts(L, row_groups=None):
    M = L.h1.shape[0]
    return o.gemm_nt_ln_parts(M if row_groups is None else M // row_groups[1] * row_groups[0])


def ffn_bwd_kw(P, L, t, drop, partials_buf, row_groups=None):
    dff = t.dhm if (drop.p > 0 and not P.self_resid) else t.dh
    ln1 = dict(dx_masked=t.dh1m, mask_mode=1, **drop.at(0)) if drop.p > 0 else {}
    return dict(dff=dff, W2t=P.ff2.t, dpre_out=t.dpre, gate=L.a, W1t=P.ff1.t, dx_out=t.dh1, x=L.h1, gamma=P.ln1.gamma, mean=L.mean1,
                rstd=L.rstd1, dgamma=P.ln1.dgamma, dbeta=P.ln1.dbeta, alpha=1.0 / (1.0 - drop.p) if drop.p > 0 else 1.0,
                resid=None if P.self_resid else t.dh, partials=partials_buf, row_groups=row_groups, **ln1)


def row_block_bwd(P, L, t, dy, rows, drop, form, partials, dy_done=False, row_groups=None, tail=None, launch=True, proj_dgrad=True):
    D, v = P.proj.w.shape[0], rows.view
    if form == "tail":
        o.row_tail_bwd(v(dy), v(L.h2), v(L.h1), v(L.a), L.mean1, L.rstd1, L.mean2, L.rstd2, P.ln1.gamma, P.ln2.gamma, P.ff2.t, P.ff1.t,
                       P.proj.t, t.dh, t.dhm, t.dx1, t.dh1m, t.dpre, v(t.dh1), v(t.datt), P.ln1.dgamma, P.ln1.dbeta, P.ln2.dgamma,
                       P.ln2.dbeta, dropout_p=drop.p, dropout_seed_ptr=drop.seed_ptr, site0=drop.site0, **tail)
        return t.dhm, t.dh1m
    M = L.h1.shape[0]
    lead = None
    if not dy_done and form == "fused" and P.mask_mode == 1:
        lead = dict(dy=dy, x=L.h2, gamma=P.ln2.gamma, mean=L.mean2, rstd=L.rstd2, dx=t.dh, dgamma=P.ln2.dgamma, dbeta=P.ln2.dbeta,
                    partials=partials(P.ln2, o.gemm_nt_ln_parts(M)), **_lead_mask(P, t, drop))
    elif not dy_done:
        mask = _lead_mask(P, t, drop)
        if P.mask_mode == 2:
            mask["dropout_site"] = drop.site0 + 2
        o.layernorm_bwd(v(L.h2), P.ln2.gamma, L.mean2, L.rstd2, v(dy), t.dh, P.ln2.dgamma, P.ln2.dbeta, D=D,
                        partials=partials(P.ln2, o.layernorm_bwd_parts(M, D)), **rows.ln, **mask)
    dff = t.dhm if (drop.p > 0 and not P.self_resid) else t.dh
    resid_ff = None if P.self_resid else t.dh
    inv_keep = 1.0 / (1.0 - drop.p) if drop.p > 0 else 1.0
    ln1 = dict(dx_masked=t.dh1m, mask_mode=1, **drop.at(0)) if drop.p > 0 else {}
    if form == "fused":
        buf = partials(P.ln1, ffn_bwd_parts(L, row_groups))
        if launch:
            o.ffn_ln_bwd(lead=lead, **ffn_bwd_kw(P, L, t, drop, buf, row_groups))
        elif lead is not None:
            raise ValueError("row_block_bwd(launch=False) needs dy_done: the block that ran elsewhere has no leading LayerNorm backward")
    else:
        o.gemm_nt(dff, P.ff2.t, t.dpre, N=4 * D, K=D, gate=v(L.a), alpha=inv_keep)
        if form == "ln_fused":
            o.gemm_nt_ln_bwd(t.dpre, P.ff1.t, t.dh1, L.h1, P.ln1.gamma, L.mean1, L.rstd1, P.ln1.dgamma, P.ln1.dbeta, N=D, K=4 * D,
                             resid=resid_ff, partials=partials(P.ln1, o.gemm_nt_ln_parts(M)), **ln1)
        else:
            o.gemm_nt(t.dpre, P.ff1.t, t.dx1, N=D, K=4 * D, resid=resid_ff)
            o.layernorm_bwd(v(L.h1), P.ln1.gamma, L.mean1, L.rstd1, t.dx1, v(t.dh1), P.ln1.dgamma, P.ln1.dbeta, D=D,
                            partials=partials(P.ln1, o.layernorm_bwd_parts(M, D)), **rows.ln, **ln1)
    dproj = t.dh1m if drop.p > 0 else v(t.dh1)
    if proj_dgrad:
        o.gemm_nt(dproj, P.proj.t, t.datt, N=D, K=D, c_remap=rows.c_remap)
    return dff, dproj


def layer_wgrads(P, L, t, x_in, dff, dproj, rows):
    D, v = P.proj.w.shape[0], rows.view
    return [o.wgrad_problem(dff, v(L.a), P.ff2.dw, P.ff2.db, N=D, K=4 * D),
            o.wgrad_problem(t.dpre, v(L.x1), P.ff1.dw, P.ff1.db, N=4 * D, K=D),
            o.wgrad_problem(dproj, v(L.att), P.proj.dw, P.proj.db, N=D, K=D),
            o.wgrad_problem(t.dqkv, x_in, P.kqv.dw, P.kqv.db, N=3 * D, K=D)]


def row_tail_selfcheck(store, B=64, S=2):
    store.tail_checked = True
    cfg, dev, adt = store.cfg, store.device, store.act_dtype
    D, F = cfg.e_model, 4 * cfg.e_model
    if not (o.can_row_tail(B, D) and store.tail_fused and cfg.e_layers >= 1):
        return True
    f32 = dict(dtype=torch.float32, device=dev)
    P = store.layer("encoder", cfg.e_layers - 1)
    scratch = lambda n: n._replace(dgamma=torch.zeros(D, **f32), dbeta=torch.zeros(D, **f32))
    P = P._replace(ln1=scratch(P.ln1), ln2=scratch(P.ln2))

    def rnd(n, width, site):
        a = torch.zeros(n, width, **f32)
        o.randn(a, seed=0x7A11, site=site)
        t = torch.zeros(n, width, dtype=adt, device=dev)
        o.cast_to_act(a, t)
        return t

    z = lambda n, w: torch.zeros(n, w, dtype=adt, device=dev)
    att, xin = rnd(B * S, D, 1), rnd(B * S, D, 2)
    status = torch.zeros(2, dtype=torch.int32, device=dev)
    sync = torch.zeros(8, dtype=torch.int32, device=dev)
    rows = position0_rows(B, S)

    def fbufs():
        L = _Layer()
        L.att, L.h1, L.x1, L.a, L.h2, L.x2 = att, z(B * S, D), z(B * S, D), z(B * S, F), z(B * S, D), z(B * S, D)
        L.mean1, L.rstd1, L.mean2, L.rstd2 = (torch.zeros(B * S, **f32) for _ in range(4))
        return L

    u, f = fbufs(), fbufs()
    tail = dict(stat_stride=S, phys_stride=S, status=status[0:1])
    row_block_fwd(P, u, xin, rows, NO_DROPOUT, "launches")
    row_block_fwd(P, f, xin, rows, NO_DROPOUT, "tail", tail=dict(tail, sync=sync[0:3]))
    dy = rnd(B * S, D, 3)

    def bbufs():
        t = _Layer()
        t.dh, t.dhm, t.dx1, t.dh1m, t.dpre, t.dh1, t.datt = z(B, D), z(B, D), z(B, D), z(B, D), z(B, F), z(B * S, D), z(B * S, D)
        return t

    ub, fb = bbufs(), bbufs()
    row_block_bwd(P, u, ub, dy, rows, NO_DROPOUT, "launches", no_partials)
    row_block_bwd(P, u, fb, dy, rows, NO_DROPOUT, "tail", no_partials, tail=dict(tail, sync=sync[4:7]))
    torch.cuda.current_stream().synchronize()
    want_f, want_b = o.row_tail_barriers(D)
    sy, stv = sync.cpu().tolist(), status.cpu().tolist()
    why = []
    if stv[0]:
        why.append(f"status flags {stv[0]:#x}")
    if sy[0] != want_f or sy[4] != want_b:
        why.append(f"barrier counters {sy[0]} / {sy[4]} instead of {want_f} / {want_b}")
    ulp = 2.0 ** -7 if adt == torch.bfloat16 else 2.0 ** -10
    host = lambda t: t.float().cpu().numpy()
    for k in ("h1", "x1", "a", "h2", "x2"):
        a, b = host(rows.view(getattr(f, k))), host(rows.view(getattr(u, k)))
        if not np.all(np.abs(a - b) <= 4 * ulp * np.maximum(np.abs(b), 1.0)):
            why.append(f"forward {k}: max difference {np.abs(a - b).max():.3g}")
    for k in ("dh", "dpre", "dx1", "dh1", "datt"):
        a, b = host(getattr(fb, k)), host(getattr(ub, k))
        if not np.abs(a - b).max() <= 4 * ulp * max(float(np.abs(b).max()), 1e-6) + 1e-6:
            why.append(f"backward {k}: max difference {np.abs(a - b).max():.3g} (scale {np.abs(b).max():.3g})")
    if why:
        store.tail_fused = False
        warnings.warn("the one-launch position-0 tail failed its start-up check on this device (" + "; ".join(why) +
                      "): using the five-launch form", RuntimeWarning)
    return not why


Forms = namedtuple("Forms", "tails riders shadows fuse_bce bce_dgrad skip_row0 cls_fold ffn_e ffn_d ln_bwd_e ln_bwd_d sched dec_tail gnorm ema "
                            "attn_proj_e attn_proj_d")


def roll_scores(tp, pred, pos, cells):
    nan = float("nan")
    return dict(precision=tp / pred if pred else nan, recall=tp / pos if pos else nan,
                f1=2 * tp / (pred + pos) if pred + pos else nan,
                cell_acc=(cells - pred - pos + 2 * tp) / cells if cells else nan)


def check_schedule(kl_warmup_steps=0, kl_cycle_steps=0, kl_free_bits=0.0, lr_warmup_steps=0):
    for name, val in (("kl_warmup_steps", kl_warmup_steps), ("kl_cycle_steps", kl_cycle_steps), ("lr_warmup_steps", lr_warmup_steps)):
        if int(val) != val or val < 0:
            raise ValueError(f"{name} must be a non-negative integer, not {val!r}")
    if not kl_free_bits >= 0:
        raise ValueError(f"kl_free_bits must be >= 0 nats per sample, not {kl_free_bits!r}")
    if kl_cycle_steps > 0 and kl_warmup_steps == 0:
        raise ValueError("kl_cycle_steps restarts the KL warm-up: it needs kl_warmup_steps > 0")
    if kl_cycle_steps > 0 and kl_warmup_steps > kl_cycle_steps:
        raise ValueError(f"kl_warmup_steps ({kl_warmup_steps}) must not exceed kl_cycle_steps ({kl_cycle_steps})")


def check_clip(clip_global_norm=0.0):
    if not (0 <= clip_global_norm < float("inf")):
        raise ValueError(f"clip_global_norm must be 0 (off) or a positive finite norm, not {clip_global_norm!r}")


def clip_scale(norm, max_norm):
    c = np.float32(max_norm) / (np.float32(norm) + np.float32(1e-8))
    return c if c < np.float32(1) else np.float32(1)


def check_ema(ema_decay=0.0):
    if not (0 <= ema_decay < 1):
        raise ValueError(f"ema_decay must be 0 (off) or lie in (0, 1), not {ema_decay!r}")


def ema_decay_at(t, decay):
    tf = np.float32(t)
    d = (np.float32(1) + tf) / (np.float32(10) + tf)
    return min(np.float32(decay), d)


def ema_update(e, w_new, d):
    d = np.float32(d)
    omd = np.float32(1) - d
    a = d * np.asarray(e, np.float32)
    b = omd * np.asarray(w_new, np.float32)
    return a + b


def schedule_values(t, kl_weight=1.0, kl_warmup_steps=0, kl_cycle_steps=0, lr_warmup_steps=0):
    f_lr = min(1.0, t / lr_warmup_steps) if lr_warmup_steps > 0 else 1.0
    u = (t - 1) % kl_cycle_steps + 1 if kl_cycle_steps > 0 else t
    ramp = min(1.0, u / kl_warmup_steps) if kl_warmup_steps > 0 else 1.0
    return float(np.float32(float(np.float32(kl_weight)) * ramp)), f_lr


class StepPlan:

    def __init__(self, store, B, T, lr=3e-4, clip_gradient=1.0, kl_weight=1.0, label_smoothing=0.0,
                 negative_label_downscaling=False, global_batch=None, gscale=None, want_probs=False, seed=0,
                 internal_eps=False, optimizer_params=None, sample_offset=0, site_base=0,
                 kl_warmup_steps=0, kl_cycle_steps=0, kl_free_bits=0.0, lr_warmup_steps=0, clip_global_norm=0.0, ema_decay=0.0):
        cfg = store.cfg
        self.store, self.cfg, self.B, self.T = store, cfg, B, T
        self.dev, self.adt = store.device, store.act_dtype
        self.lr, self.clip, self.kl_weight = lr, clip_gradient, kl_weight
        check_schedule(kl_warmup_steps, kl_cycle_steps, kl_free_bits, lr_warmup_steps)
        self.schedule = dict(kl_warmup_steps=int(kl_warmup_steps), kl_cycle_steps=int(kl_cycle_steps), kl_free_bits=float(kl_free_bits),
                             lr_warmup_steps=int(lr_warmup_steps))
        self.scheduled = any(self.schedule.values())
        check_clip(clip_global_norm)
        self.clip_global_norm = float(clip_global_norm)
        self.grad_parts = store.grad_parts() if self.clip_global_norm > 0 else None
        check_ema(ema_decay)
        self.ema_decay = float(ema_decay)
        if self.ema_decay > 0:
            store.enable_ema()
        self.ls, self.nld = label_smoothing, negative_label_downscaling
        self.global_batch = global_batch or B
        self.sample_offset, self.site_base = int(sample_offset), int(site_base)
        if (self.sample_offset * cfg.latent_dim) % 2:
            raise ValueError("sample_offset * latent_dim must be even (eps is drawn in Box-Muller pairs)")
        self.gscale = gscale if gscale is not None else (1024.0 if self.adt == torch.float16 else 1.0)
        self.gscale_enc = 1.0
        self.want_probs, self.internal_eps = want_probs, internal_eps
        self.opt = dict(beta1=0.9, beta2=0.999, eps=1e-8, wd=0.0)
        if optimizer_params:
            for k_src, k_dst in (("beta1", "beta1"), ("beta2", "beta2"), ("epsilon", "eps"), ("wd", "wd")):
                if k_src in optimizer_params:
                    self.opt[k_dst] = float(optimizer_params[k_src])
        dev, adt = self.dev, self.adt
        De, Dd, Z = cfg.e_model, cfg.d_model, cfg.latent_dim
        Se, Sd = T, T + 1
        self.Me, self.Md = B * Se, B * Sd
        f32 = dict(dtype=torch.float32, device=dev)

        def act(rows, width):
            return torch.zeros(rows, roundup(width, 8), dtype=adt, device=dev)

        self.ride = (cfg.kind != "token" and cfg.d_layers >= 1 and cfg.e_layers >= 1 and Dd in (128, 256) and
                     o.can_ride(B * T, 3 * Dd, Dd, T) and o.can_ride(B * T, Dd, 3 * Dd, T))
        self.shadows_on_tail = True
        self.dec_tail = True
        self.n_cu = torch.cuda.get_device_properties(self.dev).multi_processor_count if self.dev.type == "cuda" else 0
        self.forms = self._resolve_forms()
        if cfg.kind == "token":
            seg = [("tokens", B * T * 4), ("labels", B * T * 4)]
        else:
            self.ld_roll = roundup(cfg.in_dim + (cfg.num_classes if self.forms.cls_fold else 0), 8)
            seg = [("roll", B * T * self.ld_roll), ("labels", B * T * cfg.out_dim)]
        seg += [("seq_lens", B * 4), ("classes", B * 4)]
        self.in_layout, off = {}, 0
        for name, nbytes in seg:
            self.in_layout[name] = (off, nbytes)
            off = roundup(off + nbytes, 16)
        self.own_inbuf = torch.zeros(off, dtype=torch.uint8, device=dev)
        self.bind_inputs(self.own_inbuf)
        self.eps = torch.zeros(B, Z, **f32)
        self.rng_state = store.rng_state(seed)
        self._outers = []
        self._cls_job = None

        self.pos_e = torch.from_numpy(positional_table(De, Se)).to(dev)
        self.pos_d = torch.from_numpy(positional_table(Dd, Sd)).to(dev)
        self.keymask_e = torch.zeros(B, Se, dtype=torch.uint8, device=dev)
        self.keymask_d = torch.zeros(B, Sd, dtype=torch.uint8, device=dev)

        def layers(n, M, D, H, S):
            out = []
            for _ in range(n):
                L = _Layer()
                L.qkv, L.att, L.h1, L.x1 = act(M, 3 * D), act(M, D), act(M, D), act(M, D)
                L.a, L.h2, L.x2 = act(M, 4 * D), act(M, D), act(M, D)
                L.lse = torch.zeros(2, B, H, S, **f32)
                L.mean1, L.rstd1 = torch.zeros(M, **f32), torch.zeros(M, **f32)
                L.mean2, L.rstd2 = torch.zeros(M, **f32), torch.zeros(M, **f32)
                out.append(L)
            return out

        self.x0_e = act(self.Me, De)
        self.enc = layers(cfg.e_layers, self.Me, De, cfg.e_heads, Se)
        self.x0_d = act(self.Md, Dd)
        self.dec = layers(cfg.d_layers, self.Md, Dd, cfg.d_heads, Sd)
        self.mu, self.sigma, self.z = torch.zeros(B, Z, **f32), torch.zeros(B, Z, **f32), torch.zeros(B, Z, **f32)
        self.kl, self.total = torch.zeros(B, **f32), torch.zeros(B, **f32)
        nb4 = (B + 3) // 4 * 4
        self._recon_buf = torch.zeros(nb4 + 8 + 24 + 64, **f32)
        self.recon = self._recon_buf[:B]
        self.sync_words = self._recon_buf[nb4: nb4 + 8].view(torch.int32)
        self.ride_queues = self._recon_buf[nb4 + 32:].view(torch.int32)
        self.metric_acc = store.metric_acc
        self.track_token_metrics = False
        self.track_roll_metrics = False
        self.logits = None if self.forms.fuse_bce else act(B * T, cfg.out_dim)
        self.dlogits = act(B * T, cfg.out_dim)
        if cfg.kind == "token":
            self.probs = torch.zeros(B * T, cfg.out_dim, **f32) if want_probs else None
        else:
            self.probs = act(B * T, cfg.out_dim) if want_probs else None
        self.npos = torch.zeros(B, dtype=torch.int32, device=dev)

        def bwd_bufs(M, D, H, S):
            t = _Layer()
            t.dx_a, t.dx_b = act(M, D), act(M, D)
            t.dh, t.dhm = act(M, D), act(M, D)
            t.dh1, t.dh1m = act(M, D), act(M, D)
            t.dpre, t.dx1 = act(M, 4 * D), act(M, D)
            t.datt, t.dqkv = act(M, D), act(M, 3 * D)
            t.delta = torch.zeros(B, H, S, **f32)
            return t

        self.be_l = [bwd_bufs(self.Me, De, cfg.e_heads, Se) for _ in range(cfg.e_layers)]
        self.bd_l = [bwd_bufs(self.Md, Dd, cfg.d_heads, Sd) for _ in range(cfg.d_layers)]
        self._wgrads = []
        self.wgrad_scratch = store.wgrad_scratch()
        self._ln_part, self._psums = {}, []
        for side, n_l, M, D in (("encoder", cfg.e_layers, self.Me, De), ("decoder", cfg.d_layers, self.Md, Dd)):
            rows = max(o.layernorm_bwd_parts(M, D), o.gemm_nt_ln_parts(M))
            for i in range(n_l):
                for ln in ("ln1", "ln2" if side == "encoder" else "ln3"):
                    self._ln_part[f"{side}.layer{i}.{ln}"] = torch.zeros(rows, 2 * D, **f32)
        self.lat_scratch = torch.zeros(B * (Dd + 2 * Z), **f32)
        self.d_dec_out = act(self.Md, Dd)
        self.d_enc_out = act(self.Me, De)
        c = _Layer()
        c.dh, c.dhm, c.dx1, c.dh1m = act(B, De), act(B, De), act(B, De), act(B, De)
        c.dpre = act(B, 4 * De)
        self.sp_dh1 = c.dh1 = act(self.Me, De)
        self.sp_datt = c.datt = act(self.Me, De)
        c.dqkv, c.delta = self.be_l[-1].dqkv, self.be_l[-1].delta
        self.top = c
        self.graph = None
        self.graph_late = None
        self.graph_opt = None
        self._tick_adam = False
        self._infer = False
        self._tail_used = dict(fwd=False, bwd=False)
        if o.can_row_tail(B, De) and store.tail_fused and not store.tail_checked:
            row_tail_selfcheck(store)

    @property
    def e_p(self):
        return 0.0 if self._infer else self.cfg.e_dropout

    @property
    def d_p(self):
        return 0.0 if self._infer else self.cfg.d_dropout

    def _resolve_forms(self, with_grad=False):
        cfg, st, B, T = self.cfg, self.store, self.B, self.T
        De, Dd = cfg.e_model, cfg.d_model
        roll = cfg.kind == "pianoroll"
        tails = bool(o.can_row_tail(B, De) and st.tail_fused)
        riders = bool(self.ride and tails)
        shadows = "own" if not st.shadows_deferred else ("tail" if self.shadows_on_tail and riders else "begin")
        fuse_bce = roll and o.can_fuse_bce(cfg.out_dim, T, self.nld) and o.bce_fusion_pays(cfg.out_dim)
        ffn_d, ln_bwd_d = o.ffn_fusion_pays(Dd, 4 * Dd), o.ln_bwd_fusion_pays(Dd)
        bce_dgrad = fuse_bce and ln_bwd_d
        skip_row0 = cfg.d_layers > 0 and T % 64 == 0 and ffn_d
        return Forms(
            tails=tails, riders=riders, shadows=shadows, fuse_bce=fuse_bce,
            bce_dgrad=bce_dgrad,
            skip_row0=skip_row0,
            dec_tail=bool(with_grad and not self._infer and self.dec_tail and bce_dgrad and ffn_d and skip_row0 and
                          o.dec_tail_pays(Dd, 4 * Dd, cfg.out_dim, T, B * T // 64, self.n_cu)),
            cls_fold=(roll and cfg.in_dim % 8 == 0 and roundup(cfg.in_dim + cfg.num_classes, 256) == roundup(cfg.in_dim, 256) and
                      st.offsets["encoder.class2hid.weight"] == st.offsets["encoder.embedding.weight"] + cfg.in_dim * De),
            ffn_e=o.ffn_fusion_pays(De, 4 * De), ffn_d=ffn_d, ln_bwd_e=o.ln_bwd_fusion_pays(De), ln_bwd_d=ln_bwd_d,
            sched=self.scheduled,
            gnorm=self.clip_global_norm > 0,
            ema=self.ema_decay > 0,
            attn_proj_e=self._attn_proj(T, cfg.e_heads, De), attn_proj_d=not cfg.d_causal and self._attn_proj(T + 1, cfg.d_heads, Dd))

    def _attn_proj(self, S, H, D):
        return bool(o.attn_bwd_form(self.adt, self.B, S, H, D // H, 0, D, 2 * D, 3 * D, D, 3 * D, proj=True)["proj"])

    def _guard(self):
        fwd, bwd = o.row_tail_barriers(self.cfg.e_model)
        exp = []
        if self._tail_used["fwd"]:
            exp.append((self.sync_words[0:1], fwd))
        if self._tail_used["bwd"]:
            exp.append((self.sync_words[4:5], bwd))
        g = dict(status=self.store.step_status, expect=exp)
        if self.global_batch == self.B:
            g["finite"] = (self.recon, self.kl)
        return g

    def bind_inputs(self, buf):
        cfg, B, T = self.cfg, self.B, self.T
        need = max(a + n for a, n in self.in_layout.values())
        if not (buf.dtype == torch.uint8 and buf.is_contiguous() and buf.is_cuda and buf.data_ptr() % 16 == 0 and buf.numel() >= need):
            raise ValueError("bind_inputs: need a contiguous, 16-byte aligned device uint8 blob of pack_batch()'s size")
        self.inbuf = buf

        def inview(name, dtype, *shape):
            a, n = self.in_layout[name]
            return buf[a: a + n].view(dtype).view(*shape)

        if cfg.kind == "token":
            self.tokens = inview("tokens", torch.int32, B, T)
            self.labels = inview("labels", torch.int32, B, T)
        else:
            self.roll_cls = inview("roll", torch.uint8, B * T, self.ld_roll)
            self.roll = self.roll_cls[:, : roundup(cfg.in_dim, 8)]
            self.labels = inview("labels", torch.uint8, B * T, cfg.out_dim)
        self.seq_lens = inview("seq_lens", torch.int32, B)
        self.classes = inview("classes", torch.int32, B)

    def load_batch(self, x, seq_lens, classes, labels, eps=None):
        def dev(a, dtype):
            t = torch.as_tensor(np.asarray(a)) if not torch.is_tensor(a) else a
            return t.to(device=self.dev, dtype=dtype, non_blocking=True)

        cfg, B, T = self.cfg, self.B, self.T
        if cfg.kind == "token":
            self.tokens.copy_(dev(x, torch.int32).view(B, T))
            self.labels.copy_(dev(labels, torch.int32).view(B, T))
        else:
            self.roll[:, : cfg.in_dim].copy_(dev(x, torch.uint8).view(B * T, cfg.in_dim))
            self.labels.copy_(dev(labels, torch.uint8).view(B * T, cfg.out_dim))
        self.seq_lens.copy_(dev(seq_lens, torch.int32))
        self.classes.copy_(dev(classes, torch.int32))
        if self.forms.cls_fold:
            w = self.ld_roll - cfg.in_dim
            onehot = (self.classes.view(B, 1).to(torch.int64) == torch.arange(w, device=self.dev).view(1, w)).to(torch.uint8)
            self.roll_cls.view(B, T, -1)[:, :, cfg.in_dim:].copy_(onehot.view(B, 1, w).expand(B, T, w))
        if eps is not None:
            self.eps.copy_(dev(eps, torch.float32))

    def pack_into(self, blob, x, seq_lens, classes, labels):
        cfg, B, T = self.cfg, self.B, self.T
        assert blob.dtype == torch.uint8 and not blob.is_cuda and blob.numel() >= self.inbuf.numel()
        raw = blob.numpy()

        def seg(name, dtype, *shape):
            a, n = self.in_layout[name]
            return raw[a: a + n].view(dtype).reshape(*shape)

        def as_np(a):
            return a.cpu().numpy() if torch.is_tensor(a) else np.asarray(a)

        if cfg.kind == "token":
            np.copyto(seg("tokens", np.int32, B, T), as_np(x).reshape(B, T), casting="unsafe")
            np.copyto(seg("labels", np.int32, B, T), as_np(labels).reshape(B, T), casting="unsafe")
        else:
            ldp = self.ld_roll
            roll = seg("roll", np.uint8, B * T, ldp)
            np.copyto(roll[:, : cfg.in_dim], as_np(x).reshape(B * T, cfg.in_dim), casting="unsafe")
            if self.forms.cls_fold:
                w = ldp - cfg.in_dim
                roll.reshape(B, T, ldp)[:, :, cfg.in_dim:] = (as_np(classes).reshape(B, 1, 1).astype(np.int64) ==
                                                              np.arange(w).reshape(1, 1, w)).astype(np.uint8)
            elif ldp != cfg.in_dim:
                roll[:, cfg.in_dim:] = 0
            np.copyto(seg("labels", np.uint8, B * T, cfg.out_dim), as_np(labels).reshape(B * T, cfg.out_dim), casting="unsafe")
        np.copyto(seg("seq_lens", np.int32, B), as_np(seq_lens).reshape(B), casting="unsafe")
        np.copyto(seg("classes", np.int32, B), as_np(classes).reshape(B), casting="unsafe")
        return blob

    def pack_batch(self, x, seq_lens, classes, labels):
        return self.pack_into(torch.zeros(self.inbuf.numel(), dtype=torch.uint8), x, seq_lens, classes, labels)

    def load_packed(self, blob):
        self.inbuf.copy_(blob, non_blocking=True)

    def _drop(self, p, site):
        return dict(dropout_p=p, dropout_site=site, dropout_seed_ptr=self.rng_state) if p > 0 else {}

    def _dropout(self, p, site0):
        return Dropout(p, self.rng_state if p > 0 else None, site0)

    def _site_e(self, i):
        return self.site_base + 3 * i

    def _site_d(self, i):
        return self.site_base + 3 * (self.cfg.e_layers + i)

    def _late_shadows(self):
        st = self.store
        return dict(w=st.w, wt16=st.wt16, desc=st.t_desc_late, prefix=st.t_prefix_late, n_mat=st.t_n_late, tiles=st.t_tiles_late)

    def _top_encoder_layer_fwd(self, i, L, x_in):
        cfg, st, B, S, F = self.cfg, self.store, self.B, self.T, self.forms
        D, H = cfg.e_model, cfg.e_heads
        P = st.layer("encoder", i)
        o.attn_qkv_fwd(x_in, P.kqv.w, P.kqv.b, L.qkv, self.keymask_e, L.lse, L.att, B, S, H, D // H, 0, D, 2 * D, q_limit=1)
        self._tail_used["fwd"] = F.tails
        tail = None
        if F.tails:
            tail = dict(sync=self.sync_words[0:3], stat_stride=S, phys_stride=S, status=st.step_status[0:1], queue=self.ride_queues[0:1])
            if F.riders:
                Pd, Dd, Sd = st.layer("decoder", 0), cfg.d_model, S + 1
                tail["rider"] = dict(A=self.x0_d, B=Pd.kqv.w, C_out=self.dec[0].qkv, M=B * S, N=3 * Dd, K=Dd, bias=Pd.kqv.b,
                                     a_remap=(S, Sd, 1), c_remap=(S, Sd, 1))
                if F.shadows == "tail":
                    tail["shadows"] = self._late_shadows()
        return row_block_fwd(P, L, x_in, position0_rows(B, S), self._dropout(self.e_p, self._site_e(i)),
                             "tail" if F.tails else "launches", tail=tail)

    def _layer_fwd(self, side, i, L, x_in, keymask, D, H, S, p, site0):
        F = self.forms
        dh = D // H
        if side == "encoder" and i == self.cfg.e_layers - 1:
            return self._top_encoder_layer_fwd(i, L, x_in)
        P = self.store.layer(side, i)
        causal = side == "decoder" and self.cfg.d_causal
        if side == "decoder" and i == 0 and F.riders:
            (o.attn_causal_fwd if causal else o.attn_fwd)(L.qkv, keymask, L.lse, L.att, self.B, S, H, dh, 0, D, 2 * D)
        elif causal:
            o.gemm_nt(x_in, P.kqv.w, L.qkv, N=3 * D, K=D, bias=P.kqv.b)
            o.attn_causal_fwd(L.qkv, keymask, L.lse, L.att, self.B, S, H, dh, 0, D, 2 * D)
        else:
            o.attn_qkv_fwd(x_in, P.kqv.w, P.kqv.b, L.qkv, keymask, L.lse, L.att, self.B, S, H, dh, 0, D, 2 * D)
        fused = F.ffn_e if side == "encoder" else F.ffn_d
        if F.dec_tail and side == "decoder" and i == self.cfg.d_layers - 1:
            return L.x2
        return row_block_fwd(P, L, x_in, ALL_ROWS, self._dropout(p, site0), "fused" if fused else "launches",
                             row_groups=self._row0_groups(side, i))

    def _row0_groups(self, side, i):
        if side == "decoder" and i == self.cfg.d_layers - 1 and self.forms.skip_row0:
            return (self.T, self.T + 1, 1)
        return None

    def forward(self, inference=False, upto=None, with_grad=False):
        if with_grad and (inference or upto):
            raise ValueError("forward(with_grad=True) is the forward pass of a training step")
        if upto not in (None, "latent") or (upto and not inference):
            raise ValueError("forward(upto=...) takes 'latent', in inference mode only")
        cfg, st, B, T = self.cfg, self.store, self.B, self.T
        self._infer = bool(inference)
        F = self.forms = self._resolve_forms(with_grad)
        self._tail_used = dict(fwd=False, bwd=False)
        De, Dd = cfg.e_model, cfg.d_model
        Se, Sd = T, T + 1
        sq_e, sq_d = math.sqrt(float(De)), math.sqrt(float(Dd))
        self._wgrads, self._psums, self._outers, self._cls_job = [], [], [], None
        need_rng = self.e_p > 0 or self.d_p > 0 or self.internal_eps
        rng = st.rng_state_inference() if self._infer else self.rng_state
        tick = self._tick_adam and not self._infer
        begin = dict(rng_state=rng if need_rng else None,
                     adam_state=st.step_state if tick else None, lr=self.lr, beta1=self.opt["beta1"],
                     beta2=self.opt["beta2"], eps_out=self.eps if self.internal_eps else None,
                     eps_index0=self.sample_offset * cfg.latent_dim, lens=self.seq_lens,
                     mask_e=self.keymask_e if cfg.kind != "token" else None, add_e=0, mask_d=self.keymask_d, add_d=1,
                     zero_a=self._recon_buf, zero_b=st.g if tick else None)
        if F.shadows == "begin":
            begin["shadows"] = self._late_shadows()
        if F.sched and tick:
            begin["schedule"] = dict(block=st.sched, kl_weight=self.kl_weight, **self.schedule)
        ride = cfg.kind != "token"
        if not ride:
            o.step_begin(**begin)
        if cfg.kind == "token":
            o.embed_fwd(self.tokens, st.p("encoder.embedding.weight"), self.pos_e, self.x0_e.view(B, Se, -1), 0, sq_e,
                        classes=self.classes, cls_table=st.p("encoder.class2hid.weight"), keymask=self.keymask_e)
        else:
            o.gemm_nt_pair(dict(A=self.roll, B=st.t("encoder.embedding.weight"), C_out=self.x0_e, N=De, alpha=sq_e,
                                grpadd=st.p("encoder.class2hid.weight"), grp_index=self.classes, rowadd=self.pos_e, rowadd_period=T),
                           dict(A=self.roll, B=st.t("decoder.embedding.weight"), C_out=self.x0_d, M=B * T, N=Dd, alpha=sq_d,
                                rowadd=self.pos_d[1:], rowadd_period=T, c_remap=(T, Sd, 1)),
                           begin=begin if ride else None)
        x = self.x0_e
        for i, L in enumerate(self.enc):
            x = self._layer_fwd("encoder", i, L, x, self.keymask_e, De, cfg.e_heads, Se, self.e_p, self._site_e(i))
        self.enc_out = x
        lat = (x.view(B, Se, -1), st.p("encoder.latent_proj.weight"), st.p("encoder.latent_proj.bias"), self.eps,
               st.p("decoder.latent2hid.weight"), st.p("decoder.latent2hid.bias"), self.classes,
               st.p("decoder.class2hid.weight"), self.pos_d, sq_d, self.mu, self.sigma, self.z, self.kl,
               self.x0_d.view(B, Sd, -1))
        proj0 = None
        if F.riders:
            Pd = st.layer("decoder", 0)
            proj0 = (Pd.kqv.w, Pd.kqv.b, self.dec[0].qkv.view(B, Sd, -1))
        o.latent_fwd(*lat, proj=proj0)
        if upto == "latent":
            return
        if cfg.kind == "token":
            o.embed_fwd(self.tokens, st.p("decoder.embedding.weight"), self.pos_d, self.x0_d.view(B, Sd, -1), 1, sq_d)
        x = self.x0_d
        site_d = self._site_d(0)
        for i, L in enumerate(self.dec):
            x = self._layer_fwd("decoder", i, L, x, self.keymask_d, Dd, cfg.d_heads, Sd, self.d_p, site_d + 3 * i)
        self.dec_out = x
        if not F.fuse_bce:
            o.gemm_nt(x, st.h("decoder.output_layer.weight"), self.logits, M=B * T, K=Dd, bias=st.p("decoder.output_layer.bias"),
                      a_remap=(T, Sd, 1))

    def losses(self, with_grad=True, combine=True):
        cfg, B, T, F = self.cfg, self.B, self.T, self.forms
        dl = self.dlogits if with_grad else None
        counts = self.store.roll_counts if self.track_roll_metrics else None
        if cfg.kind == "token":
            o.softmax_ce(self.logits, self.labels, self.recon, B, T, cfg.out_dim, probs=self.probs, dlogits=dl,
                         gscale=self.gscale, pre_zeroed=True,
                         tok_parts=self.store.tok_parts if self.track_token_metrics else None)
        elif F.fuse_bce:
            dgrad = None
            if F.dec_tail and not with_grad:
                raise RuntimeError("forward(with_grad=True) left the last decoder layer to losses(with_grad=True)")
            if with_grad and F.bce_dgrad:
                last, Dd, Sd = cfg.d_layers - 1, cfg.d_model, T + 1
                dgrad = dict(A=self.dlogits, B=self.store.t("decoder.output_layer.weight"), dX_out=self.bd_l[last].dh, M=B * T, N=Dd,
                             K=self.dlogits.shape[1], c_remap=(T, Sd, 1),
                             **self._out_ln_bwd("decoder", last, self.dec[last], cfg.d_dropout, self._site_d(0) + 3 * last,
                                                self.bd_l[last], B * T))
            loss = dict(A=self.dec_out, B=self.store.h("decoder.output_layer.weight"), labels=self.labels, loss=self.recon, T=T,
                        dlogits=dl, probs=self.probs, label_smoothing=self.ls, downweight=self.nld, gscale=self.gscale, M=B * T,
                        K=cfg.d_model, bias=self.store.p("decoder.output_layer.bias"), a_remap=(T, T + 1, 1), counts=counts)
            if F.dec_tail:
                L, t, P = self.dec[last], self.bd_l[last], self.store.layer("decoder", last)
                drop, groups = self._dropout(self.d_p, self._site_d(0) + 3 * last), self._row0_groups("decoder", last)
                x_in = self.dec[last - 1].x2 if last > 0 else self.x0_d
                o.dec_tail_step(row_block_fwd(P, L, x_in, ALL_ROWS, drop, "fused", row_groups=groups, launch=False), loss, dgrad,
                                ffn_bwd_kw(P, L, t, drop, self._ln_partials_buf(P.ln1, ffn_bwd_parts(L, groups)), groups))
            else:
                o.gemm_sigmoid_bce(dgrad=dgrad, **loss)
        else:
            o.sigmoid_bce(self.logits, self.labels, self.recon, B, T, cfg.out_dim, label_smoothing=self.ls,
                          downweight=self.nld, npos=self.npos, probs=self.probs, dlogits=dl, gscale=self.gscale,
                          pre_zeroed=True, counts=counts)
        if combine:
            o.loss_combine(self.recon, self.kl, self.kl_weight, self.total, self.metric_acc, guard=self._guard())

    LN_PARTIALS_MIN = 32

    def _ln_partials_buf(self, norm, parts):
        return self._ln_part[norm.site] if parts >= self.LN_PARTIALS_MIN else None

    def _ln_partials(self, norm, parts):
        buf, dg, db = self._ln_partials_buf(norm, parts), norm.dgamma, norm.dbeta
        if buf is None:
            return None
        D = dg.numel()
        if db.data_ptr() == dg.data_ptr() + 4 * D:
            self._psums.append(o.partial_sum_job(buf, parts, dg, length=2 * D))
        else:
            self._psums += [o.partial_sum_job(buf, parts, dg, length=D), o.partial_sum_job(buf, parts, db, col_off=D, length=D)]
        return buf

    def _flush_grads(self):
        o.gemm_wgrad_batch(self._wgrads, scratch=self.wgrad_scratch, sums=self._psums, outers=self._outers, cls=self._cls_job)
        self.last_wgrad_launch = (self._wgrads, self._psums)
        self._wgrads, self._psums, self._outers, self._cls_job = [], [], [], None

    def _out_ln_bwd(self, side, i, L, p, site0, t, M):
        P = self.store.layer(side, i)
        return dict(x=L.h2, gamma=P.ln2.gamma, mean=L.mean2, rstd=L.rstd2, dgamma=P.ln2.dgamma, dbeta=P.ln2.dbeta,
                    partials=self._ln_partials(P.ln2, o.gemm_nt_ln_parts(M)), **_lead_mask(P, t, self._dropout(p, site0)))

    def _layer_bwd(self, side, i, L, x_in, dy, dx_in, keymask, D, H, S, p, site0, t, dy_done=False, next_ln=None, ride=False):
        F, P = self.forms, self.store.layer(side, i)
        ffn, ln = (F.ffn_e, F.ln_bwd_e) if side == "encoder" else (F.ffn_d, F.ln_bwd_d)
        in_loss = F.dec_tail and side == "decoder" and i == self.cfg.d_layers - 1
        proj = F.attn_proj_e if side == "encoder" else F.attn_proj_d
        dff, dproj = row_block_bwd(P, L, t, dy, ALL_ROWS, self._dropout(p, site0), "fused" if ffn else ("ln_fused" if ln else "launches"),
                                   self._ln_partials, dy_done=dy_done, row_groups=self._row0_groups(side, i), launch=not in_loss,
                                   proj_dgrad=not proj)
        if side == "decoder" and self.cfg.d_causal:
            o.attn_causal_bwd(L.qkv, keymask, L.lse, t.datt, t.dqkv, t.delta, self.B, S, H, D // H, 0, D, 2 * D)
        elif proj:
            o.attn_proj_bwd(L.qkv, keymask, L.lse, dproj, P.proj.t, t.dqkv, t.delta, self.B, S, H, D // H, 0, D, 2 * D)
        else:
            o.attn_bwd(L.qkv, keymask, L.lse, t.datt, t.dqkv, t.delta, self.B, S, H, D // H, 0, D, 2 * D)
        handed = None
        if next_ln is not None:
            kw, t_below = next_ln
            o.gemm_nt_ln_bwd(t.dqkv, P.kqv.t, t_below.dh, N=D, K=3 * D, resid=t.dh1, **kw)
        elif ride:
            T_ = self.T
            handed = (dict(A=t.dqkv, B=P.kqv.t, C_out=dx_in, M=self.B * T_, N=D, K=3 * D, resid=t.dh1, resid_phys=True,
                           a_remap=(T_, T_ + 1, 1), c_remap=(T_, T_ + 1, 1)),
                      (t.dqkv.view(self.B, S, -1), P.kqv.t, t.dh1.view(self.B, S, -1)))
        else:
            o.gemm_nt(t.dqkv, P.kqv.t, dx_in, N=D, K=3 * D, resid=t.dh1)
        self._wgrads += layer_wgrads(P, L, t, x_in, dff, dproj, ALL_ROWS)
        return handed

    def _top_encoder_layer_bwd(self, i, L, x_in, dx_in, next_ln=None, rider=None):
        cfg, st, B, S, F = self.cfg, self.store, self.B, self.T, self.forms
        D, H = cfg.e_model, cfg.e_heads
        P, c, rows = st.layer("encoder", i), self.top, position0_rows(B, S)
        self._tail_used["bwd"] = F.tails
        tail = None
        if F.tails:
            tail = dict(sync=self.sync_words[4:7], stat_stride=S, phys_stride=S, status=st.step_status[0:1], rider=rider,
                        queue=self.ride_queues[32:33])
        dff, dproj = row_block_bwd(P, L, c, self.d_enc_out, rows, self._dropout(cfg.e_dropout, self._site_e(i)),
                                   "tail" if F.tails else "launches", no_partials, tail=tail)
        o.attn_bwd(L.qkv, self.keymask_e, L.lse, c.datt, c.dqkv, c.delta, B, S, H, D // H, 0, D, 2 * D, q_limit=1)
        if next_ln is not None:
            kw, t_below = next_ln
            o.gemm_nt_ln_bwd(c.dqkv, P.kqv.t, t_below.dh, N=D, K=3 * D, resid=c.dh1, **kw)
        else:
            o.gemm_nt(c.dqkv, P.kqv.t, dx_in, N=D, K=3 * D, resid=c.dh1)
        self._wgrads += layer_wgrads(P, L, c, x_in, dff, dproj, rows)

    def backward(self):
        self.backward_early(flush=False)
        self.backward_late()

    def grad_cut(self):
        cfg, st = self.cfg, self.store
        if cfg.e_layers < 2:
            return 0
        return st.offsets[f"encoder.layer{cfg.e_layers - 1}.att.W_k.weight"]

    def _below(self, side, i, fuse):
        if not (fuse and i > 0):
            return None
        if side == "encoder":
            layers, bufs, p, site0, M = self.enc, self.be_l, self.cfg.e_dropout, self._site_e(i - 1), self.Me
        else:
            layers, bufs, p, site0, M = self.dec, self.bd_l, self.cfg.d_dropout, self._site_d(i - 1), self.Md
        return self._out_ln_bwd(side, i - 1, layers[i - 1], p, site0, bufs[i - 1], M), bufs[i - 1]

    def backward_early(self, flush):
        cfg, st, B, T, F = self.cfg, self.store, self.B, self.T, self.forms
        De, Dd = cfg.e_model, cfg.d_model
        Se, Sd = T, T + 1
        sq_d = math.sqrt(float(Dd))
        ldv = self.dlogits.shape[1]
        site_d = self._site_d(0)
        last = cfg.d_layers - 1
        if F.bce_dgrad:
            pass
        elif F.ln_bwd_d:
            o.gemm_nt_ln_bwd(self.dlogits, st.t("decoder.output_layer.weight"), self.bd_l[last].dh, M=B * T, N=Dd, K=ldv,
                             c_remap=(T, Sd, 1),
                             **self._out_ln_bwd("decoder", last, self.dec[last], cfg.d_dropout, site_d + 3 * last, self.bd_l[last], B * T))
        else:
            o.gemm_nt(self.dlogits, st.t("decoder.output_layer.weight"), self.d_dec_out, M=B * T, N=Dd, K=ldv, c_remap=(T, Sd, 1))
        self._wgrads.append(o.wgrad_problem(self.dlogits, self.dec_out, st.grad("decoder.output_layer.weight"),
                                            st.grad("decoder.output_layer.bias"), M=B * T, N=cfg.out_dim, K=Dd, b_remap=(T, Sd, 1)))
        dy, pingpong, handed = self.d_dec_out, (self.bd_l[0].dx_a, self.bd_l[0].dx_b), None
        for n, i in enumerate(reversed(range(cfg.d_layers))):
            x_in = self.dec[i - 1].x2 if i > 0 else self.x0_d
            handed = self._layer_bwd("decoder", i, self.dec[i], x_in, dy, pingpong[n % 2], self.keymask_d, Dd, cfg.d_heads, Sd,
                                     cfg.d_dropout, site_d + 3 * i, self.bd_l[i], dy_done=F.ln_bwd_d,
                                     next_ln=self._below("decoder", i, F.ln_bwd_d), ride=F.riders and i == 0)
            dy = pingpong[n % 2]
        d_x0_d = dy
        rider, dx0 = handed or (None, None)
        if cfg.kind == "token":
            o.embed_bwd(self.tokens, st.grad("decoder.embedding.weight"), d_x0_d.view(B, Sd, -1), 1, sq_d)
        else:
            self._wgrads.append(o.wgrad_problem(self.roll, d_x0_d, st.grad("decoder.embedding.weight"), M=B * T, N=cfg.out_dim,
                                                K=Dd, scale=sq_d, b_remap=(T, Sd, 1)))
        d_enc = self.d_enc_out
        o.latent_bwd_vec(st.p("encoder.latent_proj.weight"), self.eps, st.p("decoder.latent2hid.weight"), self.classes, self.mu,
                         self.sigma, d_x0_d.view(B, Sd, -1), sq_d, self.kl_weight, self.gscale_enc,
                         None, d_enc.view(B, Se, -1), self.lat_scratch,
                         enc_scale=self.gscale_enc / self.gscale, proj=dx0, sched=(st.sched, self.kl) if F.sched else None)
        self._cls_job = o.class_job(self.classes, self.lat_scratch, st.grad("decoder.class2hid.weight"), B, Dd)
        self._outers += o.latent_outer_jobs(self.lat_scratch, self.enc_out.view(B, Se, -1), self.z,
                                            st.grad("encoder.latent_proj.weight"), st.grad("encoder.latent_proj.bias"),
                                            st.grad("decoder.latent2hid.weight"), st.grad("decoder.latent2hid.bias"))
        top = cfg.e_layers - 1
        x_in = self.enc[top - 1].x2 if top > 0 else self.x0_e
        self._top_encoder_layer_bwd(top, self.enc[top], x_in, self.be_l[0].dx_a, next_ln=self._below("encoder", top, F.ln_bwd_e),
                                    rider=rider)
        if flush and cfg.e_layers >= 2:
            self._flush_grads()

    def backward_late(self):
        cfg, st, B, T, F = self.cfg, self.store, self.B, self.T, self.forms
        De, Se = cfg.e_model, T
        sq_e = math.sqrt(float(De))
        dy, pingpong = self.be_l[0].dx_a, (self.be_l[0].dx_b, self.be_l[0].dx_a)
        for n, i in enumerate(reversed(range(cfg.e_layers - 1))):
            x_in = self.enc[i - 1].x2 if i > 0 else self.x0_e
            self._layer_bwd("encoder", i, self.enc[i], x_in, dy, pingpong[n % 2], self.keymask_e, De, cfg.e_heads, Se, cfg.e_dropout,
                            self._site_e(i), self.be_l[i], dy_done=F.ln_bwd_e, next_ln=self._below("encoder", i, F.ln_bwd_e))
            dy = pingpong[n % 2]
        d_x0_e = dy
        if cfg.kind == "token":
            o.embed_bwd(self.tokens, st.grad("encoder.embedding.weight"), d_x0_e.view(B, Se, -1), 0, sq_e,
                        classes=self.classes, dcls=st.grad("encoder.class2hid.weight"))
        else:
            self._wgrads.append(o.wgrad_problem(self.roll_cls, d_x0_e, st.grad("encoder.embedding.weight"), M=B * T,
                                                N=cfg.in_dim + (cfg.num_classes if F.cls_fold else 0), K=De, scale=sq_e))
            if not F.cls_fold:
                o.group_colsum(d_x0_e.view(B, Se, -1), T, De, 0, self.classes, st.grad("encoder.class2hid.weight"), sq_e)
        self._flush_grads()

    def optimizer(self):
        st = self.store
        deferred = self.forms.shadows != "own"
        sched = st.sched if self.forms.sched else None
        clip = self.clip if self.clip is not None else -1.0
        guard = self._guard()
        mt = dict(recon=self.recon, kl=self.kl, kl_weight=self.kl_weight, total=self.total, metric=self.metric_acc, **guard)
        emb = (lambda base: dict(base=base, specs=st.emb_specs, wt16=st.wt16)) if deferred else (lambda base: None)
        gn = ((lambda a: dict(gnorm=dict(parts=self.grad_parts, max_norm=self.clip_global_norm, gstat=st.gstat if a == 0 else None)))
              if self.forms.gnorm else (lambda a: {}))
        av = (lambda a, b: dict(ema=dict(buf=st.ema[a:b], decay=self.ema_decay))) if self.forms.ema else (lambda a, b: {})
        if self.gscale == self.gscale_enc:
            r = 1.0 / (self.global_batch * self.gscale)
            if self.forms.gnorm:
                o.grad_sumsq(st.g, 0, r, r, self.grad_parts)
            o.adam_flat(st.w, st.g, st.m, st.v, st.w16, st.step_state, lr=self.lr,
                        rescale=r, clip=clip, advance_step=False, metrics=mt, emb=emb(0),
                        sched=sched, **gn(0), **av(0, st.n), **self.opt)
        else:
            cut = st.offsets["decoder.latent2hid.weight"]
            rng = [(0, cut, self.gscale_enc, False), (cut, st.n, self.gscale, False)]
            if self.forms.gnorm:
                o.grad_sumsq(st.g, cut, 1.0 / (self.global_batch * self.gscale_enc), 1.0 / (self.global_batch * self.gscale), self.grad_parts)
            for a, b, gs, adv in rng:
                o.adam_flat(st.w[a:b], st.g[a:b], st.m[a:b], st.v[a:b], st.w16[a:b], st.step_state, lr=self.lr,
                            rescale=1.0 / (self.global_batch * gs), clip=clip, advance_step=adv,
                            metrics=mt if a == 0 else (guard or None), emb=emb(a), sched=sched if a == 0 else None, **gn(a),
                            **av(a, b), **self.opt)
        if not deferred:
            o.transpose_shadows(st.w, st.wt16, st.t_desc, st.t_prefix, len(st.t_specs), st.t_tiles)

    def fwd_bwd_kernels(self, is_train=True):
        self._tick_adam = is_train
        self.forward(with_grad=is_train)
        self.losses(with_grad=is_train, combine=not is_train)
        if is_train:
            self.backward()

    def step_kernels(self, is_train=True, reduce_fn=None):
        self.fwd_bwd_kernels(is_train)
        if is_train:
            if reduce_fn is not None:
                reduce_fn(self.store.g)
            self.optimizer()

    def capture(self, is_train=True, split_optimizer=False, overlap=False):
        self.is_train, self.split = is_train, split_optimizer
        self.graph_late = None
        if is_train and split_optimizer and overlap and self.grad_cut() > 0:
            def early():
                self._tick_adam = True
                self.forward(with_grad=True)
                self.losses(with_grad=True, combine=False)
                self.backward_early(flush=True)
            self.graph = o.Graph().capture(early)
            self.graph_late = o.Graph().capture(self.backward_late)
            self.graph_opt = o.Graph().capture(self.optimizer)
        elif split_optimizer or not is_train:
            self.graph = o.Graph().capture(lambda: self.fwd_bwd_kernels(is_train))
            self.graph_opt = o.Graph().capture(self.optimizer) if is_train else None
        else:
            self.graph = o.Graph().capture(lambda: self.step_kernels(True))
            self.graph_opt = None
        return self

    def graph_nodes(self):
        gs = [g for g in (self.graph, self.graph_late, self.graph_opt) if g is not None]
        return sum(g.nodes for g in gs), sum(g.kernel_nodes for g in gs)

    def run(self, reduce_fn=None, reducer=None, stamps=None):
        if self.graph is None:
            raise RuntimeError("call capture() first")
        self.graph.launch()
        if self.graph_late is not None:
            g, cut = self.store.g, self.grad_cut()
            pending = [reducer.start(g[cut:])] if reducer is not None else []
            self.graph_late.launch()
            if stamps is not None:
                stamps[0].record()
            if reducer is not None:
                pending.append(reducer.start(g[:cut]))
                reducer.finish(pending)
            elif reduce_fn is not None:
                reduce_fn(g)
            if stamps is not None:
                stamps[1].record()
            self.graph_opt.launch()
            return
        if self.graph_opt is not None:
            if stamps is not None:
                stamps[0].record()
            if reducer is not None:
                reducer.finish([reducer.start(self.store.g)])
            elif reduce_fn is not None:
                reduce_fn(self.store.g)
            if stamps is not None:
                stamps[1].record()
            self.graph_opt.launch()

    def metrics(self, reset=True):
        m = self.store.read_metrics(reset)
        n = max(m["count"], 1.0)
        return {"kl_loss": m["kl_sum"] / n, "total_loss": m["total_sum"] / n, "count": m["count"], "nonfinite_steps": m["nonfinite_steps"],
                "kl_weight": m.get("kl_weight", self.kl_weight) if self.scheduled else self.kl_weight,
                "lr_scale": m.get("lr_scale", 1.0) if self.scheduled else 1.0,
                **{k: m[k] for k in ("grad_norm", "grad_norm_max", "clip_frac") if k in m}}
```

### musicstyletransfer_amd/ops.py

```python
import ctypes as C
import math

import torch

from . import _lib
from ._lib import LnArgs, LnBwdIn, PartialSum, OuterJob, StepBeginArgs, StepMetrics, ACT_NONE, ACT_RELU, MST_BF16, MST_F16, GemmArgs, WgradArgs, call

_DT = {torch.bfloat16: MST_BF16, torch.float16: MST_F16}


def dt(x):
    try:
        return _DT[x if isinstance(x, torch.dtype) else x.dtype]
    except KeyError:
        raise TypeError(f"activation dtype must be bfloat16 or float16, got {x}") from None


def ptr(t):
    if t is None:
        return None
    assert t.is_cuda, "mst ops need device tensors (there is no CPU fallback)"
    if t.device.index != torch.cuda.current_device():
        raise RuntimeError(f"tensor on cuda:{t.device.index} but the current device is cuda:{torch.cuda.current_device()}: "
                           "call torch.cuda.set_device() for this rank's GPU first")
    return t.data_ptr()


def stream():
    return torch.cuda.current_stream().cuda_stream


def roundup(a, b):
    return (a + b - 1) // b * b


def ld(t):
    assert t.dim() == 2 and t.stride(1) == 1
    return t.stride(0)


def _gemm_args(A, B, C_out, M=None, N=None, K=None, bias=None, resid=None, act=ACT_NONE, gate=None, alpha=1.0,
               rowadd=None, rowadd_period=0, grpadd=None, grp_index=None, a_remap=(0, 0, 0), c_remap=(0, 0, 0),
               dropout_p=0.0, dropout_seed=0, dropout_site=0, self_resid=False, dropout_seed_ptr=None, resid_phys=False):
    g = GemmArgs()
    g.a_u8 = 1 if A.dtype == torch.uint8 else 0
    g.dtype = dt(B if g.a_u8 else A)
    g.c_f32 = 1 if C_out.dtype == torch.float32 else 0
    g.M = A.shape[0] if M is None else M
    g.N = B.shape[0] if N is None else N
    g.K = A.shape[1] if K is None else K
    g.A, g.lda = ptr(A), ld(A)
    g.B, g.ldb = ptr(B), ld(B)
    g.C, g.ldc = ptr(C_out), ld(C_out)
    g.bias = ptr(bias)
    g.resid, g.ldr = ptr(resid), (ld(resid) if resid is not None else 0)
    g.act = act
    g.gate, g.ldg = ptr(gate), (ld(gate) if gate is not None else 0)
    g.alpha = alpha
    g.rowadd, g.ldra = ptr(rowadd), (ld(rowadd) if rowadd is not None else 0)
    g.rowadd_period = rowadd_period
    g.grpadd, g.ldga = ptr(grpadd), (ld(grpadd) if grpadd is not None else 0)
    g.grp_index = ptr(grp_index)
    g.a_rows_per_group, g.a_group_stride, g.a_group_offset = a_remap
    g.c_rows_per_group, g.c_group_stride, g.c_group_offset = c_remap
    g.dropout_p, g.dropout_seed, g.dropout_site = dropout_p, dropout_seed, dropout_site
    g.self_resid = 1 if self_resid else 0
    g.resid_phys = 1 if resid_phys else 0
    g.dropout_seed_ptr = ptr(dropout_seed_ptr)
    return g


def gemm_nt(A, B, C_out, **kw):
    call("mst_gemm_nt", C.byref(_gemm_args(A, B, C_out, **kw)), stream())


def gemm_nt_form(A, B, C_out, **kw):
    rc = _lib.load().mst_gemm_nt_form(C.byref(_gemm_args(A, B, C_out, **kw)))
    if rc < 0:
        _lib.check(rc, "mst_gemm_nt_form")
    return rc


def gemm_nt_pair(first, second, begin=None):
    if begin is None:
        call("mst_gemm_nt_pair", C.byref(_gemm_args(**first)), C.byref(_gemm_args(**second)), stream())
    else:
        call("mst_gemm_nt_pair_begin", C.byref(_gemm_args(**first)), C.byref(_gemm_args(**second)), C.byref(_step_begin_args(**begin)),
             stream())


def can_ride(M, N, K, T=0):
    return M % 128 == 0 and N % 128 == 0 and K % 64 == 0 and (T == 0 or T % 128 == 0)


def can_row_tail(B, D):
    return D in (128, 256) and 0 < B <= 64


def row_tail_barriers(D):
    return 3 * (D // 16), 2 * (D // 16)


def row_tail_fwd(att, resid, Wp, bp, g1, be1, W1, b1, W2, b2, g2, be2, h1, x1, a, h2, x2, mean1, rstd1, mean2, rstd2, sync, stat_stride,
                 phys_stride, eps=1e-5, dropout_p=0.0, dropout_seed_ptr=None, site0=0, status=None, rider=None, queue=None, shadows=None,
                 dropout_seed=0):
    assert sync.numel() >= 3 and (rider is None or queue is not None) and (shadows is None or rider is not None)
    q = _lib.RowTailArgs()
    q.dtype, q.B, q.D = dt(att), att.shape[0], Wp.shape[0]
    q.att, q.rs_att, q.resid, q.rs_res = ptr(att), att.stride(0), ptr(resid), resid.stride(0)
    q.Wp, q.ldwp, q.bp, q.g1, q.be1 = ptr(Wp), ld(Wp), ptr(bp), ptr(g1), ptr(be1)
    q.W1, q.ldw1, q.b1, q.W2, q.ldw2, q.b2, q.g2, q.be2 = ptr(W1), ld(W1), ptr(b1), ptr(W2), ld(W2), ptr(b2), ptr(g2), ptr(be2)
    assert h1.stride(0) == x1.stride(0) == h2.stride(0) == x2.stride(0)
    q.h1, q.x1, q.h2, q.x2, q.rs_d, q.a, q.rs_a = ptr(h1), ptr(x1), ptr(h2), ptr(x2), h1.stride(0), ptr(a), a.stride(0)
    q.mean1, q.rstd1, q.mean2, q.rstd2, q.stat_stride = ptr(mean1), ptr(rstd1), ptr(mean2), ptr(rstd2), stat_stride
    q.eps, q.dropout_p, q.dropout_seed, q.dropout_seed_ptr, q.site0 = eps, dropout_p, dropout_seed, ptr(dropout_seed_ptr), site0
    q.phys_stride, q.sync, q.status = phys_stride, ptr(sync), ptr(status)
    if shadows is not None:
        call("mst_row_tail_fwd_ride_shadows", C.byref(q), C.byref(_gemm_args(**rider)), ptr(queue), dt(shadows["wt16"]), ptr(shadows["w"]),
             ptr(shadows["wt16"]), ptr(shadows["desc"]), ptr(shadows["prefix"]), shadows["n_mat"], shadows["tiles"], stream())
    elif rider is not None:
        call("mst_row_tail_fwd_ride", C.byref(q), C.byref(_gemm_args(**rider)), ptr(queue), stream())
    else:
        call("mst_row_tail_fwd", C.byref(q), stream())


def row_tail_bwd(dy, h2, h1, a, mean1, rstd1, mean2, rstd2, g1, g2, W2t, W1t, Wpt, dh, dhm, dx1, dh1m, dpre, dh1, datt, dg1, db1, dg2, db2,
                 sync, stat_stride, phys_stride, dropout_p=0.0, dropout_seed_ptr=None, site0=0, status=None, rider=None, queue=None,
                 dropout_seed=0):
    assert sync.numel() >= 3 and (rider is None or queue is not None)
    q = _lib.RowTailBwdArgs()
    q.dtype, q.B, q.D = dt(dy), dy.shape[0], Wpt.shape[0]
    q.dy, q.rs_dy = ptr(dy), dy.stride(0)
    assert h2.stride(0) == h1.stride(0)
    q.h2, q.h1, q.rs_d, q.a, q.rs_a = ptr(h2), ptr(h1), h2.stride(0), ptr(a), a.stride(0)
    q.mean1, q.rstd1, q.mean2, q.rstd2, q.stat_stride = ptr(mean1), ptr(rstd1), ptr(mean2), ptr(rstd2), stat_stride
    q.g1, q.g2 = ptr(g1), ptr(g2)
    q.W2t, q.ldw2t, q.W1t, q.ldw1t, q.Wpt, q.ldwpt = ptr(W2t), ld(W2t), ptr(W1t), ld(W1t), ptr(Wpt), ld(Wpt)
    assert dh.stride(0) == dhm.stride(0) == dx1.stride(0) == dh1m.stride(0)
    q.dh, q.dhm, q.dx1, q.dh1m, q.rs_c = ptr(dh), ptr(dhm), ptr(dx1), ptr(dh1m), dh.stride(0)
    q.dpre, q.rs_dpre, q.dh1, q.rs_dh1, q.datt, q.rs_datt = ptr(dpre), dpre.stride(0), ptr(dh1), dh1.stride(0), ptr(datt), datt.stride(0)
    q.dg1, q.db1, q.dg2, q.db2 = ptr(dg1), ptr(db1), ptr(dg2), ptr(db2)
    q.dropout_p, q.dropout_seed, q.dropout_seed_ptr, q.site0 = dropout_p, dropout_seed, ptr(dropout_seed_ptr), site0
    q.phys_stride, q.sync, q.status = phys_stride, ptr(sync), ptr(status)
    if rider is not None:
        call("mst_row_tail_bwd_ride", C.byref(q), C.byref(_gemm_args(**rider)), ptr(queue), stream())
    else:
        call("mst_row_tail_bwd", C.byref(q), stream())


def row_tail_form(backward, dtype, D, rider=None, sh_tiles=0):
    form = (C.c_int64 * 6)()
    g = None if rider is None else C.byref(rider if isinstance(rider, GemmArgs) else _gemm_args(**rider))
    call("mst_row_tail_form", 1 if backward else 0, dt(dtype), D, g, sh_tiles, form)
    return dict(zip(("kernel", "ride_rows", "tiles", "grid", "lds", "tickets"), form))


def can_fuse_bce(P, T, downweight=False):
    return (P == 128 or (P % 256 == 0 and (P == 256 or not downweight))) and T % 64 == 0


def bce_fusion_pays(P):
    return P <= 256


def _roll_counts(counts):
    if counts is not None:
        assert counts.dtype == torch.int64 and counts.is_contiguous() and tuple(counts.shape) == (_lib.ROLL_SLOTS, 4)
    return ptr(counts)


def _gemm_bce_args(A, B, labels, loss, T, dlogits=None, probs=None, logits=None, label_smoothing=0.0, downweight=False, gscale=1.0,
                   counts=None, **kw):
    g = _gemm_args(A, B, dlogits if dlogits is not None else A, N=B.shape[0], **kw)
    if dlogits is None:
        g.C, g.ldc = None, 0
    q = _lib.BceArgs()
    q.labels, q.T, q.label_smoothing, q.downweight, q.loss = ptr(labels), T, label_smoothing, 1 if downweight else 0, ptr(loss)
    q.probs, q.ldp = ptr(probs), (ld(probs) if probs is not None else 0)
    q.logits, q.ldl = ptr(logits), (ld(logits) if logits is not None else 0)
    q.gscale = gscale
    q.counts = _roll_counts(counts)
    return g, q


def gemm_sigmoid_bce(A, B, labels, loss, T, dgrad=None, **kw):
    g, q = _gemm_bce_args(A, B, labels, loss, T, **kw)
    if dgrad is None:
        call("mst_gemm_sigmoid_bce", C.byref(g), C.byref(q), stream())
    else:
        g2, l = _gemm_ln_bwd_args(**dgrad)
        call("mst_gemm_sigmoid_bce_dgrad_ln", C.byref(g), C.byref(q), C.byref(g2), C.byref(l), stream())


def gemm_sigmoid_bce_form(g, q, g2=None, l=None):
    form = (C.c_int64 * 4)()
    call("mst_gemm_sigmoid_bce_form", C.byref(g), C.byref(q), C.byref(g2) if g2 is not None else None, C.byref(l) if l is not None else None,
         form)
    return dict(BN=form[0], col_tiles=form[1], launches=form[2])


def can_fuse_ln(D):
    return D in (128, 256)


def ln_bwd_fusion_pays(D):
    return D == 128


def gemm_nt_ln_fwd(A, B, H_out, gamma, beta, Y_out, mean, rstd, eps=1e-5, **kw):
    g = _gemm_args(A, B, H_out, **kw)
    l = LnArgs()
    l.mode, l.gamma, l.beta, l.eps = 1, ptr(gamma), ptr(beta), eps
    l.out, l.ld_out = ptr(Y_out), ld(Y_out)
    l.mean, l.rstd = ptr(mean), ptr(rstd)
    call("mst_gemm_nt_ln", C.byref(g), C.byref(l), stream())


def can_fuse_ffn(D, F):
    return D in (128, 256) and F % D == 0


def ffn_fusion_pays(D, F):
    return can_fuse_ffn(D, F)


def _row_groups(n_rows, row_groups):
    rpg, stride, off = row_groups
    assert n_rows % stride == 0 and rpg % 64 == 0 and off + rpg <= stride
    return (n_rows // stride) * rpg, (rpg, stride, off)


def ffn_ln_fwd(x, W1, a_out, W2, h_out, gamma, beta, y_out, mean, rstd, eps=1e-5, ff1=None, ff2=None, proj=None, row_groups=None):
    g0, l0, g1, g2, l = _ffn_ln_fwd_args(x, W1, a_out, W2, h_out, gamma, beta, y_out, mean, rstd, eps, ff1, ff2, proj, row_groups)
    if proj is None:
        call("mst_ffn_ln_fwd", C.byref(g1), C.byref(g2), C.byref(l), stream())
    else:
        call("mst_proj_ffn_ln_fwd", C.byref(g0), C.byref(l0), C.byref(g1), C.byref(g2), C.byref(l), stream())


def _ffn_ln_fwd_args(x, W1, a_out, W2, h_out, gamma, beta, y_out, mean, rstd, eps=1e-5, ff1=None, ff2=None, proj=None, row_groups=None):
    ff1, ff2 = dict(ff1 or {}), dict(ff2 or {})
    if row_groups is not None:
        M, remap = _row_groups(x.shape[0], row_groups)
        ff1.update(M=M, a_remap=remap)
        ff2.update(M=M)
        if proj is not None:
            proj = dict(proj, M=M)
    g1 = _gemm_args(x, W1, a_out, **ff1)
    g2 = _gemm_args(a_out, W2, h_out, **ff2)
    l = LnArgs()
    l.mode, l.gamma, l.beta, l.eps = 1, ptr(gamma), ptr(beta), eps
    l.out, l.ld_out = ptr(y_out), ld(y_out)
    l.mean, l.rstd = ptr(mean), ptr(rstd)
    if proj is None:
        return None, None, g1, g2, l
    kw = {k: v for k, v in proj.items() if k not in ("att", "W", "h1", "gamma", "beta", "mean", "rstd")}
    g0 = _gemm_args(proj["att"], proj["W"], proj["h1"], **kw)
    l0 = LnArgs()
    l0.mode, l0.gamma, l0.beta, l0.eps = 1, ptr(proj["gamma"]), ptr(proj["beta"]), eps
    l0.out, l0.ld_out = ptr(x), ld(x)
    l0.mean, l0.rstd = ptr(proj["mean"]), ptr(proj["rstd"])
    return g0, l0, g1, g2, l


def _ffn_ln_bwd_args(dff, W2t, dpre_out, gate, W1t, dx_out, x, gamma, mean, rstd, dgamma, dbeta, alpha=1.0, dx_masked=None, mask_mode=0,
                     partials=None, row_groups=None, **kw):
    rg = {}
    if row_groups is not None:
        M, remap = _row_groups(dff.shape[0], row_groups)
        rg, kw = dict(M=M, a_remap=remap), dict(kw, M=M)
    g1 = _gemm_args(dff, W2t, dpre_out, gate=gate, alpha=alpha, **rg)
    g2 = _gemm_args(dpre_out, W1t, dx_out, **kw)
    l = LnArgs()
    l.mode, l.gamma = 2, ptr(gamma)
    l.mean, l.rstd = ptr(mean), ptr(rstd)
    l.x, l.ld_x = ptr(x), ld(x)
    l.dgamma, l.dbeta = ptr(dgamma), ptr(dbeta)
    l.out, l.ld_out = ptr(dx_masked), (ld(dx_masked) if dx_masked is not None else 0)
    l.mask_mode = mask_mode
    l.partials = ptr(partials)
    if partials is not None:
        assert partials.shape[0] >= gemm_nt_ln_parts(g1.M) and partials.shape[1] == 2 * g2.N and partials.is_contiguous()
    return g1, g2, l


def can_dec_tail(D, F, P, T):
    return D == 128 and F == 512 and P == 128 and T > 0 and T % 64 == 0


def dec_tail_pays(D, F, P, T, tiles, n_cu=256):
    return can_dec_tail(D, F, P, T) and 0 < tiles <= n_cu


def dec_tail_step(fwd, loss, dgrad, bwd):
    g0, l0, g1, g2, l3 = _ffn_ln_fwd_args(**fwd)
    go, q = _gemm_bce_args(**loss)
    gd, l3b = _gemm_ln_bwd_args(**dgrad)
    b1, b2, l1b = _ffn_ln_bwd_args(**bwd)
    call("mst_dec_tail_step", C.byref(g0), C.byref(l0), C.byref(g1), C.byref(g2), C.byref(l3), C.byref(go), C.byref(q), C.byref(gd),
         C.byref(l3b), C.byref(b1), C.byref(b2), C.byref(l1b), stream())


def ffn_ln_bwd(dff, W2t, dpre_out, gate, W1t, dx_out, x, gamma, mean, rstd, dgamma, dbeta, alpha=1.0, dx_masked=None, mask_mode=0,
               partials=None, lead=None, row_groups=None, **kw):
    g1, g2, l = _ffn_ln_bwd_args(dff, W2t, dpre_out, gate, W1t, dx_out, x, gamma, mean, rstd, dgamma, dbeta, alpha, dx_masked, mask_mode,
                                 partials, row_groups, **kw)
    if lead is None:
        call("mst_ffn_ln_bwd", C.byref(g1), C.byref(g2), C.byref(l), stream())
        return
    q = LnBwdIn()
    q.dy, q.ld_dy = ptr(lead["dy"]), ld(lead["dy"])
    q.x, q.ld_x = ptr(lead["x"]), ld(lead["x"])
    q.gamma, q.mean, q.rstd = ptr(lead["gamma"]), ptr(lead["mean"]), ptr(lead["rstd"])
    q.dx, q.ld_dx = ptr(lead["dx"]), ld(lead["dx"])
    dxm = lead.get("dx_masked")
    q.dx_masked, q.ld_dxm = ptr(dxm), (ld(dxm) if dxm is not None else 0)
    q.dgamma, q.dbeta, q.partials = ptr(lead.get("dgamma")), ptr(lead.get("dbeta")), ptr(lead.get("partials"))
    q.mask_mode = 1 if dxm is not None else 0
    q.dropout_p, q.dropout_seed = lead.get("dropout_p", 0.0), lead.get("dropout_seed", 0)
    q.dropout_seed_ptr, q.dropout_site = ptr(lead.get("dropout_seed_ptr")), lead.get("dropout_site", 0)
    if lead.get("partials") is not None:
        assert lead["partials"].shape[0] >= gemm_nt_ln_parts(g1.M) and lead["partials"].shape[1] == 2 * g2.N
    call("mst_ffn_ln_bwd_lead", C.byref(q), C.byref(g1), C.byref(g2), C.byref(l), stream())


def gemm_nt_ln_bwd(A, B, dX_out, x, gamma, mean, rstd, dgamma, dbeta, dx_masked=None, mask_mode=0, partials=None, **kw):
    g, l = _gemm_ln_bwd_args(A, B, dX_out, x, gamma, mean, rstd, dgamma, dbeta, dx_masked, mask_mode, partials, **kw)
    call("mst_gemm_nt_ln", C.byref(g), C.byref(l), stream())


def _gemm_ln_bwd_args(A, B, dX_out, x, gamma, mean, rstd, dgamma, dbeta, dx_masked=None, mask_mode=0, partials=None, **kw):
    g = _gemm_args(A, B, dX_out, **kw)
    l = LnArgs()
    l.mode, l.gamma = 2, ptr(gamma)
    l.mean, l.rstd = ptr(mean), ptr(rstd)
    l.x, l.ld_x = ptr(x), ld(x)
    l.dgamma, l.dbeta = ptr(dgamma), ptr(dbeta)
    l.out, l.ld_out = ptr(dx_masked), (ld(dx_masked) if dx_masked is not None else 0)
    l.mask_mode = mask_mode
    l.partials = ptr(partials)
    if partials is not None:
        assert partials.shape[0] >= gemm_nt_ln_parts(g.M) and partials.shape[1] == 2 * g.N and partials.is_contiguous()
    return g, l


def gemm_nt_ln_parts(M):
    return int(_lib.load().mst_gemm_nt_ln_parts(M))


def layernorm_bwd_parts(M, D):
    return int(_lib.load().mst_layernorm_bwd_parts(M, D))


PARTIAL_SUM_MAX_JOBS = 20


def partial_sum_job(src, n_parts, dst, scale=1.0, col_off=0, length=None):
    j = PartialSum()
    length = dst.numel() if length is None else length
    assert src.dtype == dst.dtype and src.element_size() == 4 and src.shape[0] >= n_parts
    j.src = src.data_ptr() + 4 * col_off
    j.n_parts, j.stride, j.len = n_parts, src.stride(0), length
    j.dst, j.scale = ptr(dst), scale
    return j


def partial_sums(jobs):
    for i in range(0, len(jobs), PARTIAL_SUM_MAX_JOBS):
        chunk = jobs[i:i + PARTIAL_SUM_MAX_JOBS]
        call("mst_partial_sums", (PartialSum * len(chunk))(*chunk), len(chunk), stream())


def wgrad_problem(A, B, dW, db=None, M=None, N=None, K=None, scale=1.0, a_remap=(0, 0, 0), b_remap=(0, 0, 0)):
    w = WgradArgs()
    w.a_u8 = 1 if A.dtype == torch.uint8 else 0
    w.dtype = dt(B if w.a_u8 else A)
    w.M = A.shape[0] if M is None else M
    w.N = dW.shape[0] if N is None else N
    w.K = dW.shape[1] if K is None else K
    w.A, w.lda = ptr(A), ld(A)
    w.B, w.ldb = ptr(B), ld(B)
    w.dW, w.ldw = ptr(dW), ld(dW)
    w.db = ptr(db)
    w.scale = scale
    w.a_rows_per_group, w.a_group_stride, w.a_group_offset = a_remap
    w.b_rows_per_group, w.b_group_stride, w.b_group_offset = b_remap
    return w


WGRAD_MAX_PROBLEMS = 16
OUTER_MAX_JOBS = 2


def outer_job(L, R, out, obias=None):
    q = OuterJob()
    assert L.dtype == torch.float32 and L.is_contiguous() and out.dtype == torch.float32 and out.is_contiguous() and R.stride(1) == 1
    q.L, q.R, q.r_stride = ptr(L), ptr(R), R.stride(0)
    q.r_dtype = 2 if R.dtype == torch.float32 else dt(R)
    q.B, q.J, q.I = L.shape[0], L.shape[1], R.shape[1]
    assert out.numel() == q.J * q.I and R.shape[0] == q.B and (obias is None or obias.numel() == q.J)
    q.out, q.obias = ptr(out), ptr(obias)
    return q


def outer_jobs(jobs):
    for i in range(0, len(jobs), OUTER_MAX_JOBS):
        chunk = jobs[i:i + OUTER_MAX_JOBS]
        call("mst_outer_jobs", (OuterJob * len(chunk))(*chunk), len(chunk), stream())


def class_job(classes, scratch, dcls, B, Dd):
    assert classes.dtype == torch.int32 and classes.numel() == B and scratch.dtype == dcls.dtype == torch.float32
    assert scratch.is_contiguous() and scratch.numel() >= B * Dd and dcls.stride(1) == 1 and dcls.shape[1] >= Dd
    return (ptr(classes), ptr(scratch), ptr(dcls), dcls.stride(0), B, Dd)


def class_table_grad(job):
    call("mst_class_table_grad", *job, stream())


def gemm_wgrad_batch(problems, scratch=None, sums=None, outers=None, cls=None):
    sums, outers = list(sums or []), list(outers or [])
    for i in range(0, len(problems), WGRAD_MAX_PROBLEMS):
        chunk = problems[i:i + WGRAD_MAX_PROBLEMS]
        take, tko, tkc = [], [], None
        if i + WGRAD_MAX_PROBLEMS >= len(problems):
            take, sums = sums[:PARTIAL_SUM_MAX_JOBS], sums[PARTIAL_SUM_MAX_JOBS:]
            tko, outers = outers[:OUTER_MAX_JOBS], outers[OUTER_MAX_JOBS:]
            tkc, cls = cls, None
        head = ((WgradArgs * len(chunk))(*chunk), len(chunk), ptr(scratch),
                (scratch.numel() * scratch.element_size() if scratch is not None else 0),
                (PartialSum * len(take))(*take) if take else None, len(take),
                (OuterJob * len(tko))(*tko) if tko else None, len(tko))
        if tkc is not None:
            call("mst_gemm_wgrad_batch_flush_cls", *head, *tkc, stream())
        else:
            call("mst_gemm_wgrad_batch_flush", *head, stream())
    if sums:
        partial_sums(sums)
    if outers:
        outer_jobs(outers)
    if cls is not None:
        class_table_grad(cls)


def gemm_wgrad_plan(problems, scratch_bytes=0):
    plan = (C.c_int64 * (4 + WGRAD_MAX_PROBLEMS))()
    call("mst_gemm_wgrad_plan", (WgradArgs * len(problems))(*problems), len(problems), scratch_bytes, plan)
    return dict(form=plan[0], narrow=plan[1], items=plan[2], two_pass=plan[3], splits=list(plan[4:4 + len(problems)]))


def flush_jobs_ride(problems, scratch_bytes=0):
    return bool(gemm_wgrad_plan(problems, scratch_bytes)["two_pass"] & 1)


def gemm_wgrad(A, B, dW, db=None, **kw):
    gemm_wgrad_batch([wgrad_problem(A, B, dW, db, **kw)])


def attn_fwd(qkv, keymask, lse, out, B, S, H, dh, k_off, q_off, v_off, q_limit=0):
    call("mst_attn_keysoftmax_fwd", dt(qkv), B, S, H, dh, ptr(qkv), ld(qkv), k_off, q_off, v_off, ptr(keymask),
         ptr(lse), ptr(out), ld(out), q_limit, stream())


def attn_qkv_fwd(x, W, bias, qkv, keymask, lse, out, B, S, H, dh, k_off, q_off, v_off, q_limit=0):
    call("mst_attn_qkv_fwd", dt(qkv), B, S, H, dh, ptr(x), ld(x), ptr(W), ld(W), ptr(bias), ptr(qkv), ld(qkv), k_off, q_off, v_off,
         ptr(keymask), ptr(lse), ptr(out), ld(out), q_limit, stream())


def attn_bwd(qkv, keymask, lse, dout, dqkv, delta, B, S, H, dh, k_off, q_off, v_off, q_limit=0):
    call("mst_attn_keysoftmax_bwd", dt(qkv), B, S, H, dh, ptr(qkv), ld(qkv), k_off, q_off, v_off, ptr(keymask),
         ptr(lse), ptr(dout), ld(dout), ptr(dqkv), ld(dqkv), ptr(delta), q_limit, stream())


def attn_proj_bwd(qkv, keymask, lse, dproj, Wt, dqkv, delta, B, S, H, dh, k_off, q_off, v_off, dout_out=None):
    call("mst_attn_proj_bwd", dt(qkv), B, S, H, dh, ptr(qkv), ld(qkv), k_off, q_off, v_off, ptr(keymask), ptr(lse), ptr(dproj), ld(dproj),
         ptr(Wt), ld(Wt), ptr(dout_out), ld(dout_out) if dout_out is not None else 0, ptr(dqkv), ld(dqkv), ptr(delta), stream())


ATTN_FWD_PATHS = ("resident-3", "resident-2", "chunked", "fused", "stream")
ATTN_BWD_PATHS = ("resident", "stream+chunked-dq", "stream")


def attn_fwd_form(dtype, B, S, H, dh, k_off, q_off, v_off, ld_qkv, ld_out, q_limit=0, fused=False, ld_x=0, ld_w=0):
    form = (C.c_int64 * 8)()
    call("mst_attn_fwd_form", dt(dtype), B, S, H, dh, ld_qkv, k_off, q_off, v_off, ld_out, q_limit, 1 if fused else 0, ld_x, ld_w, form)
    return dict(path=ATTN_FWD_PATHS[form[0]], waves=form[1], lds=form[2], lone=form[3], grid_stats=form[4], grid_out=form[5])


def attn_bwd_form(dtype, B, S, H, dh, k_off, q_off, v_off, ld_qkv, ld_dout, ld_dqkv, q_limit=0, proj=False):
    form = (C.c_int64 * 8)()
    call("mst_attn_bwd_form", dt(dtype), B, S, H, dh, ld_qkv, k_off, q_off, v_off, ld_dout, ld_dqkv, q_limit, form)
    d = dict(path=ATTN_BWD_PATHS[form[0]], waves=form[1], lds=form[2], sparse=form[3], lone=form[4], dq_chunks=form[5],
             dq_waves=form[6])
    if proj:
        d["proj"] = form[7]
    return d


def attn_causal_fwd(qkv, keymask, lse, out, B, S, H, dh, k_off, q_off, v_off):
    call("mst_attn_causal_fwd", dt(qkv), B, S, H, dh, ptr(qkv), ld(qkv), k_off, q_off, v_off, ptr(keymask), ptr(lse), ptr(out),
         ld(out), stream())


def attn_causal_bwd(qkv, keymask, lse, dout, dqkv, delta, B, S, H, dh, k_off, q_off, v_off):
    call("mst_attn_causal_bwd", dt(qkv), B, S, H, dh, ptr(qkv), ld(qkv), k_off, q_off, v_off, ptr(keymask), ptr(lse), ptr(dout),
         ld(dout), ptr(dqkv), ld(dqkv), ptr(delta), stream())


def attn_decode(cache3, n_keys, H, dh, k_off, q_off, v_off, out, mode=0):
    B, t_max = cache3.shape[0], cache3.shape[1]
    assert cache3.stride(2) == 1 and cache3.stride(0) == t_max * cache3.stride(1)
    call("mst_attn_decode", dt(cache3), B, H, dh, n_keys, t_max, ptr(cache3), cache3.stride(1), k_off, q_off, v_off, mode, ptr(out),
         ld(out), stream())


def beam_step(probs, scores_in, scores_out, seqs_in, seqs_out, hyp_src, word, i, K, eos, pad, active=None):
    N, V = probs.shape[0], probs.shape[1]
    call("mst_beam_step", N // K, K, V, i, seqs_in.shape[1], ptr(probs), probs.stride(0), ptr(scores_in), ptr(scores_out), ptr(seqs_in),
         ptr(seqs_out), ptr(hyp_src), ptr(word), ptr(active), eos, pad, stream())


def sample_step(probs, seqs, scores, word, i, seed, eos, pad, active=None):
    call("mst_sample_step", probs.shape[0], probs.shape[1], i, seqs.shape[1], ptr(probs), probs.stride(0), ptr(seqs), ptr(scores), ptr(word),
         ptr(active), seed, eos, pad, stream())


FRAME_MODES = {"draw": 0, "threshold": 1}


def frame_step(logits, P, i, seed_ptr, frames, roll, scores, tau=1.0, mode="draw", thr=0.5, probs_out=None):
    N, L = roll.shape[0], roll.shape[1]
    assert roll.is_contiguous() and (probs_out is None or (probs_out.is_contiguous() and tuple(probs_out.shape) == (N, L, P)))
    call("mst_frame_step", dt(logits), N, P, i, L, ptr(logits), ld(logits), tau, FRAME_MODES[mode], thr, ptr(seed_ptr), ptr(frames), ld(frames),
         ptr(roll), roll.stride(1), ptr(scores), ptr(probs_out), stream())


def token_step(logits, V, i, seed_ptr, seqs, scores, word, eos, pad, tau=1.0, top_k=0, top_p=1.0, active=None, kept_out=None):
    assert seqs.is_contiguous()
    call("mst_token_step", dt(logits), seqs.shape[0], V, i, seqs.shape[1], ptr(logits), ld(logits), tau, top_k, top_p, ptr(seed_ptr), ptr(seqs),
         ptr(scores), ptr(word), ptr(active), ptr(kept_out), eos, pad, stream())


def beam_gather(cache_in, cache_out, src, n_rows, skip_cols=None):
    N, t_max, width = cache_in.shape
    es = cache_in.element_size()
    if skip_cols is None:
        call("mst_beam_gather", ptr(cache_in), ptr(cache_out), ptr(src), N, n_rows, width * es, t_max, stream())
    else:
        call("mst_beam_gather_cols", ptr(cache_in), ptr(cache_out), ptr(src), N, n_rows, width * es, t_max, skip_cols[0] * es,
             skip_cols[1] * es, stream())


def layernorm_fwd(x, gamma, beta, y, mean, rstd, D=None, eps=1e-5, M=None, row_id_stride=1):
    M = x.shape[0] if M is None else M
    D = x.shape[1] if D is None else D
    call("mst_layernorm_fwd", dt(x), M, D, ptr(x), ld(x), ptr(gamma), ptr(beta), eps, ptr(y), ld(y), ptr(mean),
         ptr(rstd), row_id_stride, stream())


def layernorm_bwd(x, gamma, mean, rstd, dy, dx, dgamma, dbeta, D=None, dx_masked=None, mask_mode=0, dropout_p=0.0,
                  dropout_seed=0, dropout_site=0, dropout_seed_ptr=None, M=None, row_id_stride=1, partials=None):
    M = x.shape[0] if M is None else M
    D = x.shape[1] if D is None else D
    if partials is not None:
        assert partials.shape[0] >= layernorm_bwd_parts(M, D) and partials.shape[1] == 2 * D and partials.is_contiguous()
    call("mst_layernorm_bwd", dt(x), M, D, ptr(x), ld(x), ptr(gamma), ptr(mean), ptr(rstd), ptr(dy), ld(dy), ptr(dx),
         ld(dx), ptr(dx_masked), (ld(dx_masked) if dx_masked is not None else 0), ptr(dgamma), ptr(dbeta), mask_mode,
         dropout_p, dropout_seed, dropout_site, ptr(dropout_seed_ptr), row_id_stride, ptr(partials), stream())


def embed_fwd(tokens, table, pos, out3, s_off, alpha, classes=None, cls_table=None, keymask=None):
    B, T = tokens.shape
    D = table.shape[1]
    call("mst_embed_fwd", dt(out3), B, T, D, ptr(tokens), ptr(table), table.stride(0), ptr(classes), ptr(cls_table),
         (cls_table.stride(0) if cls_table is not None else 0), ptr(pos), pos.stride(0), alpha, ptr(out3),
         out3.stride(1), out3.shape[1], s_off, ptr(keymask), stream())


def embed_bwd(tokens, dtable, dX3, s_off, alpha, classes=None, dcls=None):
    B, T = tokens.shape
    D = dtable.shape[1]
    call("mst_embed_bwd", dt(dX3), B, T, D, ptr(tokens), ptr(dtable), dtable.stride(0), ptr(classes), ptr(dcls),
         (dcls.stride(0) if dcls is not None else 0), alpha, ptr(dX3), dX3.stride(1), dX3.shape[1], s_off, stream())


def group_colsum(X3, T, D, s_off, idx, dst, alpha):
    B = X3.shape[0]
    call("mst_group_colsum", dt(X3), B, T, D, ptr(X3), X3.stride(1), X3.shape[1], s_off, ptr(idx), ptr(dst),
         dst.stride(0), alpha, stream())


def mask_from_lengths(lens, add, keymask):
    B, S = keymask.shape
    call("mst_mask_from_lengths", B, S, ptr(lens), add, ptr(keymask), stream())


def latent_fwd(enc_out3, Wl, bl, eps, Wh, bh, classes, cls_d, pos_d, alpha_d, mu, sigma, z, kl, dec_in3, proj=None):
    B = enc_out3.shape[0]
    De, Z, Dd = Wl.shape[1], Wh.shape[1], Wh.shape[0]
    args = (dt(enc_out3), B, De, Z, Dd, ptr(enc_out3), enc_out3.stride(0), ptr(Wl), ptr(bl), ptr(eps),
            ptr(Wh), ptr(bh), ptr(classes), ptr(cls_d), cls_d.stride(0), ptr(pos_d), alpha_d, ptr(mu), ptr(sigma), ptr(z),
            ptr(kl), ptr(dec_in3), dec_in3.stride(0))
    if proj is None:
        call("mst_latent_fwd", *args, stream())
    else:
        Wq, bq, qkv3 = proj
        call("mst_latent_fwd_proj", *args, ptr(Wq), ld(Wq), ptr(bq), ptr(qkv3), qkv3.stride(0), Wq.shape[0], stream())


def latent_form(De, Z, Dd, nq=0, Wl=0, part=None):
    form = (C.c_int64 * 8)(*([-1] * 8))
    addr = Wl.data_ptr() if isinstance(Wl, torch.Tensor) else Wl
    rc = _lib.load().mst_latent_form(De, Z, Dd, nq, addr, form)
    names = ("fwd_pre", "loader_l", "loader_h", "proj_vec", "fwd_lds", "bwd_pre", "dh0", "bwd_lds")
    if part == "fwd" and form[0] >= 0:
        return dict(zip(names[:5], form[:5]))
    _lib.check(rc, "mst_latent_form")
    return dict(zip(names[5:], form[5:8])) if part == "bwd" else dict(zip(names, form))


LATENT_ROWS_SITE = 0x7FFE0000
INTERP = {"lerp": 0, "slerp": 1}


# ... 297 lines not shown
```

Baseline: 27.16 million frames/s.

## Fuse encoder KQV dgrad GEMM into the next layer's FFN+LN backward kernel

```diff
diff --git a/include/mst_hip.h b/include/mst_hip.h
--- a/include/mst_hip.h
+++ b/include/mst_hip.h
@@ -111,6 +111,10 @@
 } mst_ln_bwd_in;
 int mst_ffn_ln_bwd_lead(const mst_ln_bwd_in* lead, const mst_gemm_args* ff2_dgrad, const mst_gemm_args* ff1_dgrad,
                         const mst_ln_args* ln, mst_stream_t stream);
+int mst_kqv_ffn_ln_bwd(const mst_gemm_args* kqv_dgrad, const mst_ln_bwd_in* lead, const mst_gemm_args* ff2_dgrad,
+                       const mst_gemm_args* ff1_dgrad, const mst_ln_args* ln, mst_stream_t stream);
+int mst_kqv_ffn_ln_bwd_form(const mst_gemm_args* kqv_dgrad, const mst_gemm_args* ff2_dgrad, const mst_gemm_args* ff1_dgrad,
+                            int64_t* form);
 int mst_proj_ffn_ln_fwd(const mst_gemm_args* proj, const mst_ln_args* ln1, const mst_gemm_args* ff1, const mst_gemm_args* ff2,
                         const mst_ln_args* ln2, mst_stream_t stream);
 int mst_dec_tail_step(const mst_gemm_args* proj, const mst_ln_args* ln1, const mst_gemm_args* ff1, const mst_gemm_args* ff2,
diff --git a/musicstyletransfer_amd/csrc/ffn_ln.hip b/musicstyletransfer_amd/csrc/ffn_ln.hip
--- a/musicstyletransfer_amd/csrc/ffn_ln.hip
+++ b/musicstyletransfer_amd/csrc/ffn_ln.hip
@@ -19,13 +19,14 @@
   const size_t lds_epi = (size_t)BM * (BN + 4) * 4;
   const size_t lds = lds_loop > lds_epi ? lds_loop : lds_epi;
   const int full = g1.M % BM == 0 ? 1 : 0;
-  const int mi = ex ? 6 + full : (lead ? 2 : (ln.mode == 2 ? 1 : 0)) * 2 + full;
+  const int mi = ex ? (ln.mode == 2 ? 8 : 6) + full : (lead ? 2 : (ln.mode == 2 ? 1 : 0)) * 2 + full;
   typedef void (*kern_t)(mst_gemm_args, mst_gemm_args, mst_ln_args, mst_ln_bwd_in, mst_gemm_args, mst_ln_args);
-  const kern_t fns[8] = {&ffn_ln_kernel<T, BN, 2, 4, 1, false, false>, &ffn_ln_kernel<T, BN, 2, 4, 1, false, true>,
+  const kern_t fns[10] = {&ffn_ln_kernel<T, BN, 2, 4, 1, false, false>, &ffn_ln_kernel<T, BN, 2, 4, 1, false, true>,
                          &ffn_ln_kernel<T, BN, 2, 4, 2, false, false>, &ffn_ln_kernel<T, BN, 2, 4, 2, false, true>,
                          &ffn_ln_kernel<T, BN, 2, 4, 2, true, false>, &ffn_ln_kernel<T, BN, 2, 4, 2, true, true>,
-                         &ffn_ln_kernel<T, BN, 2, 4, 1, false, false, true>, &ffn_ln_kernel<T, BN, 2, 4, 1, false, true, true>};
-  static size_t granted[8] = {64 * 1024, 64 * 1024, 64 * 1024, 64 * 1024, 64 * 1024, 64 * 1024, 64 * 1024, 64 * 1024};
+                         &ffn_ln_kernel<T, BN, 2, 4, 1, false, false, true>, &ffn_ln_kernel<T, BN, 2, 4, 1, false, true, true>,
+                          &ffn_ln_kernel<T, BN, 2, 4, 2, true, false, true>, &ffn_ln_kernel<T, BN, 2, 4, 2, true, true, true>};
+  static size_t granted[10] = {64 * 1024, 64 * 1024, 64 * 1024, 64 * 1024, 64 * 1024, 64 * 1024, 64 * 1024, 64 * 1024, 64 * 1024, 64 * 1024};
   if (const int rc = lds_opt_in(reinterpret_cast<const void*>(fns[mi]), lds, &granted[mi], "ffn_ln_kernel")) return rc;
   const mst_ln_bwd_in none = {};
   const mst_gemm_args no_gemm = {};
@@ -80,8 +81,10 @@
   if (lead) {
     const mst_ln_bwd_in& q = *lead;
     MST_CHECK_ARG(mode == 2, "%s: a leading LayerNorm belongs to the backward form", who);
-    MST_CHECK_ARG(q.dy && q.x && q.gamma && q.mean && q.rstd && q.dx && (q.partials || (q.dgamma && q.dbeta)), "%s: leading LayerNorm: null pointer", who);
-    MST_CHECK_ARG(q.ld_dy % 8 == 0 && q.ld_x % 8 == 0 && q.ld_dx % 8 == 0 && q.ld_dy >= b.N && q.ld_x >= b.N && q.ld_dx >= b.N &&
+    const bool dy_on_chip = extra != nullptr;
+    MST_CHECK_ARG((q.dy || dy_on_chip) && q.x && q.gamma && q.mean && q.rstd && q.dx && (q.partials || (q.dgamma && q.dbeta)),
+                  "%s: leading LayerNorm: null pointer", who);
+    MST_CHECK_ARG((dy_on_chip || (q.ld_dy % 8 == 0 && q.ld_dy >= b.N)) && q.ld_x % 8 == 0 && q.ld_dx % 8 == 0 && q.ld_x >= b.N && q.ld_dx >= b.N &&
                   ((uintptr_t)q.dy | (uintptr_t)q.x | (uintptr_t)q.dx | (uintptr_t)q.partials) % 16 == 0, "%s: leading LayerNorm: bad layout", who);
     MST_CHECK_ARG(q.mask_mode == 0 || (q.mask_mode == 1 && q.dx_masked && q.ld_dxm % 8 == 0 && q.ld_dxm >= b.N && (uintptr_t)q.dx_masked % 16 == 0),
                   "%s: leading LayerNorm: mask_mode must be 0 or 1 (with dx_masked)", who);
@@ -90,7 +93,8 @@
     const int64_t tile_ld = q.mask_mode == 1 ? q.ld_dxm : q.ld_dx;
     MST_CHECK_ARG(a.A == tile && a.lda == tile_ld, "%s: the first GEMM's A operand must be the leading LayerNorm's (masked) output", who);
   }
-  if (extra) {
+  if (extra && mode == 2) {
+  } else if (extra) {
     const mst_gemm_args& x = *extra;
     rc = check_gemm_common(x);
     if (rc) return rc;
@@ -138,6 +142,49 @@
   return ffn_ln_impl("mst_ffn_ln_bwd_lead", ff2_dgrad, ff1_dgrad, ln, 2, stream, lead);
 }
 
+static int kqv_head_form(const mst_gemm_args& x, const mst_gemm_args& a, const mst_gemm_args& b) {
+  const bool shape = (b.N == 256 || b.N == 128) && x.N == b.N && x.K == 3 * b.N && x.M == a.M && x.dtype == a.dtype;
+  const bool plain = !x.c_f32 && !x.a_u8 && !x.bias && !x.gate && !x.rowadd && !x.grpadd && x.act == MST_ACT_NONE && x.alpha == 1.f &&
+                     x.dropout_p == 0.f && !x.self_resid && x.a_rows_per_group <= 0 && x.c_rows_per_group <= 0 && a.a_rows_per_group <= 0;
+  const bool layout = x.resid && ((uintptr_t)x.A | (uintptr_t)x.B | (uintptr_t)x.resid | (uintptr_t)x.C) % 16 == 0 && x.lda % 8 == 0 &&
+                      x.lda >= x.K && x.ldb % 8 == 0 && x.ldb >= x.K && x.ldr % 8 == 0 && x.ldr >= x.N &&
+                      (!x.C || (x.ldc % 8 == 0 && x.ldc >= x.N)) && (uint64_t)x.N * (uint64_t)x.ldb < (1ull << 32);
+  return shape && plain && layout ? 1 : 0;
+}
+
+static int check_kqv_head_call(const char* who, const mst_gemm_args* head, const mst_gemm_args* ff2_dgrad, const mst_gemm_args* ff1_dgrad) {
+  MST_CHECK_ARG(head != nullptr && ff2_dgrad != nullptr && ff1_dgrad != nullptr, "%s: null args", who);
+  MST_CHECK_ARG(head->M > 0 && head->N > 0 && head->K > 0, "%s: the head's M,N,K must be positive (got %lld,%lld,%lld)", who,
+                (long long)head->M, (long long)head->N, (long long)head->K);
+  MST_CHECK_ARG(head->A && head->B, "%s: the head's A and B operands are missing", who);
+  MST_CHECK_ARG(head->M == ff2_dgrad->M && head->N == ff1_dgrad->N, "%s: the head's result is the block's incoming gradient: M x width (got %lld x %lld)",
+                who, (long long)head->M, (long long)head->N);
+  return MST_OK;
+}
+
+extern "C" int mst_kqv_ffn_ln_bwd_form(const mst_gemm_args* kqv_dgrad, const mst_gemm_args* ff2_dgrad, const mst_gemm_args* ff1_dgrad,
+                                       int64_t* form) {
+  MST_CHECK_ARG(form != nullptr, "mst_kqv_ffn_ln_bwd_form: null form");
+  if (const int rc = check_kqv_head_call("mst_kqv_ffn_ln_bwd_form", kqv_dgrad, ff2_dgrad, ff1_dgrad)) return rc;
+  form[0] = kqv_head_form(*kqv_dgrad, *ff2_dgrad, *ff1_dgrad);
+  return MST_OK;
+}
+
+extern "C" int mst_kqv_ffn_ln_bwd(const mst_gemm_args* kqv_dgrad, const mst_ln_bwd_in* lead, const mst_gemm_args* ff2_dgrad,
+                                  const mst_gemm_args* ff1_dgrad, const mst_ln_args* ln, mst_stream_t stream) {
+  if (const int rc = check_kqv_head_call("mst_kqv_ffn_ln_bwd", kqv_dgrad, ff2_dgrad, ff1_dgrad)) return rc;
+  MST_CHECK_ARG(lead != nullptr, "mst_kqv_ffn_ln_bwd: null args");
+  MST_CHECK_ARG(lead->dy == kqv_dgrad->C && (!lead->dy || lead->ld_dy == kqv_dgrad->ldc),
+                "mst_kqv_ffn_ln_bwd: lead->dy is the head's C (both NULL: the gradient is not stored)");
+  if (kqv_head_form(*kqv_dgrad, *ff2_dgrad, *ff1_dgrad))
+    return ffn_ln_impl("mst_kqv_ffn_ln_bwd", ff2_dgrad, ff1_dgrad, ln, 2, stream, lead, kqv_dgrad);
+  MST_CHECK_ARG(kqv_dgrad->C != nullptr, "mst_kqv_ffn_ln_bwd: this shape runs the GEMM launch first and needs the head's C");
+  if (const int rc = check_ffn_ln("mst_kqv_ffn_ln_bwd", ff2_dgrad, ff1_dgrad, ln, 2, lead)) return rc;
+  if (const int f = mst_gemm_nt_form(kqv_dgrad); f < 0) return f;
+  if (const int rc = mst_gemm_nt(kqv_dgrad, stream)) return rc;
+  return ffn_ln_impl("mst_kqv_ffn_ln_bwd", ff2_dgrad, ff1_dgrad, ln, 2, stream, lead);
+}
+
 extern "C" int mst_ffn_ln_fwd(const mst_gemm_args* ff1, const mst_gemm_args* ff2, const mst_ln_args* ln, mst_stream_t stream) {
   return ffn_ln_impl("mst_ffn_ln_fwd", ff1, ff2, ln, 1, stream);
 }
diff --git a/musicstyletransfer_amd/csrc/ffn_ln.hpp b/musicstyletransfer_amd/csrc/ffn_ln.hpp
--- a/musicstyletransfer_amd/csrc/ffn_ln.hpp
+++ b/musicstyletransfer_amd/csrc/ffn_ln.hpp
@@ -9,15 +9,16 @@
 __device__ __forceinline__ void ffn_ln_body(unsigned char* smem, mst_gemm_args g1, mst_gemm_args g2, const mst_ln_args ln,
                                             const mst_ln_bwd_in lead, mst_gemm_args gx, const mst_ln_args lnx, float* par,
                                             Hook&& before_epilogue) {
-  constexpr bool HEAD = EXTRA;
+  constexpr bool HEAD = EXTRA, FHEAD = EXTRA && MODE == 1, BHEAD = EXTRA && MODE == 2;
   static_assert(!(X_IN_LDS && (LEAD || EXTRA)), "a tile left in LDS is the block's own input");
-  static_assert(!EXTRA || MODE == 1, "the extra GEMM is the forward form's head");
+  static_assert(!BHEAD || LEAD, "the backward form's head computes the gradient tile of the leading LayerNorm backward");
   constexpr int BM = 64, BK = 64, CHUNKS = BK / 8;
   constexpr int NT = WGM * WGN * 64;
   constexpr int WTM = BM / WGM, WTN = BN / WGN, TM = WTM / 16, TN = WTN / 16;
   constexpr int B_CH = BN * CHUNKS / NT;
   constexpr int LDA = BN + 8;
   constexpr int KST = BN / BK;
+  constexpr int XST = BHEAD ? 3 * KST : KST;
   static_assert(BN * CHUNKS % NT == 0 && (BM * BN / 8) % NT == 0, "tile/threads mismatch");
   typedef typename Act<T>::vec8 vec8;
   u32x4* sB = reinterpret_cast<u32x4*>(smem);
@@ -40,13 +41,13 @@
   for (int i = tid * 4; i < (int)F; i += NT * 4)
     *reinterpret_cast<f32x4*>(sBias1 + i) = g1.bias ? *reinterpret_cast<const f32x4*>(g1.bias + i) : f32x4{0.f, 0.f, 0.f, 0.f};
   const uint64_t seed2 = g2.dropout_seed ^ ((g2.dropout_p > 0.f && g2.dropout_seed_ptr) ? g2.dropout_seed_ptr[0] : 0ull);
-  const uint64_t seedx = EXTRA ? gx.dropout_seed ^ ((gx.dropout_p > 0.f && gx.dropout_seed_ptr) ? gx.dropout_seed_ptr[0] : 0ull) : 0ull;
+  const uint64_t seedx = FHEAD ? gx.dropout_seed ^ ((gx.dropout_p > 0.f && gx.dropout_seed_ptr) ? gx.dropout_seed_ptr[0] : 0ull) : 0ull;
   if constexpr (!PAR_READY)
   for (int i = tid; i < BN; i += NT) {
     sPar[i] = g2.bias ? g2.bias[i] : 0.f;
     sPar[BN + i] = ln.gamma[i];
     sPar[2 * BN + i] = (MODE == 1) ? ln.beta[i] : 0.f;
-    if constexpr (HEAD) {
+    if constexpr (FHEAD) {
       sPar[3 * BN + i] = gx.bias ? gx.bias[i] : 0.f;
       sPar[4 * BN + i] = lnx.gamma[i];
       sPar[5 * BN + i] = lnx.beta[i];
@@ -106,7 +107,7 @@
     auto pro = [&](auto jc) {
       constexpr int j = decltype(jc)::value;
       if constexpr (HEAD) {
-        static_assert(!HEAD || AHEAD <= KST, "the head GEMM's stages cover the prologue");
+        static_assert(!HEAD || AHEAD <= XST, "the head GEMM's stages cover the prologue");
         if (j < AHEAD) load_stage(-1, j, ring[j % RING]);
       } else {
         if (j < AHEAD && (j < SPC || n_chunks > 1)) load_stage(j / SPC, j % SPC, ring[j % RING]);
@@ -117,28 +118,50 @@
     pro(std::integral_constant<int, 6>());
     static_assert(AHEAD <= 7, "the prologue list covers seven stages");
   }
-  if constexpr (LEAD) {
-    constexpr int CPR = BN / 8, RSTEP = NT / CPR, ITERS = BM / RSTEP;
-    const int ch = tid % CPR, nc = ch * 8, row0 = tid / CPR;
-    const float inv_n = 1.f / (float)BN;
+  constexpr int L_CPR = BN / 8, L_RSTEP = NT / L_CPR, L_ITERS = BM / L_RSTEP;
+  const int lnc = (tid % L_CPR) * 8, lrow0 = tid / L_CPR;
+  uint32_t ldkey = 0u, ldthr = 0u;
+  float linv_keep = 1.f, gam8[8], dg8[8], db8[8];
+  u32x4 dyv[L_ITERS], xv[L_ITERS];
+  float mean_r[L_ITERS], rstd_r[L_ITERS];
+  u32x4 ha2[L_ITERS], hres[L_ITERS];
+  auto lead_loads = [&] {
+    constexpr int RSTEP = L_RSTEP, ITERS = L_ITERS;
+    const int nc = lnc, row0 = lrow0;
     const bool has_drop = lead.dropout_p > 0.f && lead.mask_mode == 1;
     const uint64_t dseed = lead.dropout_seed ^ ((has_drop && lead.dropout_seed_ptr) ? lead.dropout_seed_ptr[0] : 0ull);
-    const uint32_t dkey = dropout_key(dseed, lead.dropout_site), dthr = dropout_thr(lead.dropout_p);
-    const float inv_keep = dropout_inv_keep(lead.dropout_p);
-    float gam8[8], dg8[8], db8[8];
+    ldkey = dropout_key(dseed, lead.dropout_site); ldthr = dropout_thr(lead.dropout_p);
+    linv_keep = dropout_inv_keep(lead.dropout_p);
 #pragma unroll
     for (int e = 0; e < 8; ++e) { gam8[e] = lead.gamma[nc + e]; dg8[e] = 0.f; db8[e] = 0.f; }
-    u32x4 dyv[ITERS], xv[ITERS];
-    float mean_r[ITERS], rstd_r[ITERS];
 #pragma unroll
     for (int it = 0; it < ITERS; ++it) {
       const int64_t m = m0 + row0 + it * RSTEP;
       dyv[it] = u32x4{0u, 0u, 0u, 0u}; xv[it] = dyv[it]; mean_r[it] = 0.f; rstd_r[it] = 0.f;
       if (m < Mg) {
-        dyv[it] = *reinterpret_cast<const u32x4*>(reinterpret_cast<const T*>(lead.dy) + m * lead.ld_dy + nc);
+        if constexpr (!BHEAD) dyv[it] = *reinterpret_cast<const u32x4*>(reinterpret_cast<const T*>(lead.dy) + m * lead.ld_dy + nc);
         xv[it] = *reinterpret_cast<const u32x4*>(reinterpret_cast<const T*>(lead.x) + m * lead.ld_x + nc);
         mean_r[it] = lead.mean[m];
         rstd_r[it] = lead.rstd[m];
+      }
+    }
+  };
+  auto lead_rows = [&] {
+    constexpr int CPR = L_CPR, RSTEP = L_RSTEP, ITERS = L_ITERS;
+    const int nc = lnc, row0 = lrow0;
+    const float inv_n = 1.f / (float)BN;
+    const bool has_drop = lead.dropout_p > 0.f && lead.mask_mode == 1;
+    const uint32_t dkey = ldkey, dthr = ldthr;
+    const float inv_keep = linv_keep;
+    if constexpr (BHEAD) {
+#pragma unroll
+      for (int it = 0; it < ITERS; ++it) {
+        const int row = row0 + it * RSTEP;
+        const int64_t m = m0 + row;
+        if (m < Mg) {
+          dyv[it] = *reinterpret_cast<const u32x4*>(sX + row * LDA + nc);
+          if (gx.C) *reinterpret_cast<u32x4*>(reinterpret_cast<T*>(gx.C) + m * gx.ldc + nc) = dyv[it];
+        }
       }
     }
 #pragma unroll
@@ -195,6 +218,34 @@
       else atomicAdd((which ? lead.dbeta : lead.dgamma) + col, sm);
     }
     __syncthreads();
+  };
+  if constexpr (BHEAD) {
+    constexpr int RSTEP = L_RSTEP, ITERS = L_ITERS;
+    const T* HA = reinterpret_cast<const T*>(gx.A);
+    const T* HR = reinterpret_cast<const T*>(gx.resid);
+    u32x4 ha0[ITERS], ha1[ITERS];
+#pragma unroll
+    for (int it = 0; it < ITERS; ++it) {
+      const int64_t m = m0 + lrow0 + it * RSTEP;
+      ha0[it] = u32x4{0u, 0u, 0u, 0u}; ha1[it] = ha0[it]; ha2[it] = ha0[it]; hres[it] = ha0[it];
+      if (m < Mg) {
+        const T* ap = HA + m * gx.lda + lnc;
+        ha0[it] = *reinterpret_cast<const u32x4*>(ap);
+        ha1[it] = *reinterpret_cast<const u32x4*>(ap + BN);
+        ha2[it] = *reinterpret_cast<const u32x4*>(ap + 2 * BN);
+        hres[it] = *reinterpret_cast<const u32x4*>(HR + m * gx.ldr + lnc);
+      }
+    }
+    lead_loads();
+#pragma unroll
+    for (int it = 0; it < ITERS; ++it) {
+      const int row = lrow0 + it * RSTEP;
+      *reinterpret_cast<u32x4*>(sX + row * LDA + lnc) = ha0[it];
+      *reinterpret_cast<u32x4*>(sH + row * LDA + lnc) = ha1[it];
+    }
+  } else if constexpr (LEAD) {
+    lead_loads();
+    lead_rows();
   } else if constexpr (!X_IN_LDS)
   {
     const T* X = reinterpret_cast<const T*>(HEAD ? gx.A : g1.A);
@@ -264,20 +315,47 @@
     __syncthreads();
     auto xstage = [&](auto sc) {
       constexpr int s = decltype(sc)::value;
-      if constexpr (s < KST) {
+      if constexpr (s < XST) {
         constexpr int t = s + AHEAD;
-        if constexpr (t < KST) load_stage(cx, t, ring[t % RING]);
-        else if constexpr (HEAD) load_stage(0, t - KST, ring[t % RING]);
-        mma_stage(acc1, sX + s * BK, s & 1, ring[s % RING], no_hook);
-        if constexpr (s + 1 < KST) store_stage((s + 1) & 1, ring[(s + 1) % RING]);
+        if constexpr (t < XST) load_stage(cx, t, ring[t % RING]);
+        else if constexpr (HEAD) load_stage(0, t - XST, ring[t % RING]);
+        mma_stage(acc1, (((s / KST) & 1) ? sH : sX) + (s % KST) * BK, s & 1, ring[s % RING], no_hook);
+        if constexpr (s + 1 < XST) store_stage((s + 1) & 1, ring[(s + 1) % RING]);
         __syncthreads();
+        if constexpr (BHEAD && (s == KST - 1 || s == 2 * KST - 1)) {
+#pragma unroll
+          for (int it = 0; it < L_ITERS; ++it)
+            *reinterpret_cast<u32x4*>((s == KST - 1 ? sX : sH) + (lrow0 + it * L_RSTEP) * LDA + lnc) = s == KST - 1 ? ha2[it] : hres[it];
+        }
       }
     };
-    static_assert(!EXTRA || (KST <= 4 && KST % RING == 0), "the extra GEMM stage list / ring slots");
+    static_assert(!EXTRA || (XST <= 12 && XST % RING == 0 && XST % 2 == 0), "the extra GEMM stage list / ring slots");
     xstage(std::integral_constant<int, 0>()); xstage(std::integral_constant<int, 1>());
     xstage(std::integral_constant<int, 2>()); xstage(std::integral_constant<int, 3>());
-  };
-  if constexpr (HEAD) {
+    xstage(std::integral_constant<int, 4>()); xstage(std::integral_constant<int, 5>());
+    xstage(std::integral_constant<int, 6>()); xstage(std::integral_constant<int, 7>());
+    xstage(std::integral_constant<int, 8>()); xstage(std::integral_constant<int, 9>());
+    xstage(std::integral_constant<int, 10>()); xstage(std::integral_constant<int, 11>());
+  };
+  if constexpr (BHEAD) {
+    extra_gemm(-1);
+#pragma unroll
+    for (int j = 0; j < TN; ++j)
+#pragma unroll
+      for (int i = 0; i < TM; ++i) {
+        const int row = wm * WTM + i * 16 + frow, n = wn * WTN + j * 16 + fq * 4;
+        const u32x2 rb = *reinterpret_cast<const u32x2*>(sH + row * LDA + n);
+        uint16_t hb[4];
+#pragma unroll
+        for (int e = 0; e < 4; ++e)
+          hb[e] = f32_to_bits<T>(acc1[j][i][e] + bits_to_f32<T>((uint16_t)(rb[e >> 1] >> ((e & 1) * 16))));
+        *reinterpret_cast<u32x2*>(sX + row * LDA + n) =
+            u32x2{(uint32_t)hb[0] | ((uint32_t)hb[1] << 16), (uint32_t)hb[2] | ((uint32_t)hb[3] << 16)};
+      }
+    __syncthreads();
+    lead_rows();
+  }
+  if constexpr (FHEAD) {
     extra_gemm(-1);
     gemm_epilogue_ln<T, BM, BN, WGM, WGN, 1>(gx, lnx, smem, acc1, m0, nullptr, 0, sX, LDA, sPar + 3 * BN, &seedx);
     __syncthreads();
diff --git a/musicstyletransfer_amd/csrc/runtime.hip b/musicstyletransfer_amd/csrc/runtime.hip
--- a/musicstyletransfer_amd/csrc/runtime.hip
+++ b/musicstyletransfer_amd/csrc/runtime.hip
@@ -14,7 +14,7 @@
 
 using namespace mst;
 
-extern "C" int mst_version(void) { return 115; }
+extern "C" int mst_version(void) { return 116; }
 extern "C" const char* mst_last_error(void) { return g_err; }
 
 #define HIP_TRY(expr)                                             \
diff --git a/musicstyletransfer_amd/engine.py b/musicstyletransfer_amd/engine.py
--- a/musicstyletransfer_amd/engine.py
+++ b/musicstyletransfer_amd/engine.py
@@ -475,7 +475,8 @@
                 resid=None if P.self_resid else t.dh, partials=partials_buf, row_groups=row_groups, **ln1)
 
 
-def row_block_bwd(P, L, t, dy, rows, drop, form, partials, dy_done=False, row_groups=None, tail=None, launch=True, proj_dgrad=True):
+def row_block_bwd(P, L, t, dy, rows, drop, form, partials, dy_done=False, row_groups=None, tail=None, launch=True, proj_dgrad=True,
+                  head=None):
     D, v = P.proj.w.shape[0], rows.view
     if form == "tail":
         o.row_tail_bwd(v(dy), v(L.h2), v(L.h1), v(L.a), L.mean1, L.rstd1, L.mean2, L.rstd2, P.ln1.gamma, P.ln2.gamma, P.ff2.t, P.ff1.t,
@@ -485,7 +486,8 @@
     M = L.h1.shape[0]
     lead = None
     if not dy_done and form == "fused" and P.mask_mode == 1:
-        lead = dict(dy=dy, x=L.h2, gamma=P.ln2.gamma, mean=L.mean2, rstd=L.rstd2, dx=t.dh, dgamma=P.ln2.dgamma, dbeta=P.ln2.dbeta,
+        lead = dict(dy=None if head is not None else dy, x=L.h2, gamma=P.ln2.gamma, mean=L.mean2, rstd=L.rstd2, dx=t.dh,
+                    dgamma=P.ln2.dgamma, dbeta=P.ln2.dbeta,
                     partials=partials(P.ln2, o.gemm_nt_ln_parts(M)), **_lead_mask(P, t, drop))
     elif not dy_done:
         mask = _lead_mask(P, t, drop)
@@ -499,8 +501,10 @@
     ln1 = dict(dx_masked=t.dh1m, mask_mode=1, **drop.at(0)) if drop.p > 0 else {}
     if form == "fused":
         buf = partials(P.ln1, ffn_bwd_parts(L, row_groups))
+        if head is not None and (lead is None or not launch):
+            raise ValueError("row_block_bwd(head=) needs the one launch that starts with the leading LayerNorm backward")
         if launch:
-            o.ffn_ln_bwd(lead=lead, **ffn_bwd_kw(P, L, t, drop, buf, row_groups))
+            o.ffn_ln_bwd(lead=lead, head=head, **ffn_bwd_kw(P, L, t, drop, buf, row_groups))
         elif lead is not None:
             raise ValueError("row_block_bwd(launch=False) needs dy_done: the block that ran elsewhere has no leading LayerNorm backward")
     else:
@@ -596,7 +600,7 @@
 
 
 Forms = namedtuple("Forms", "tails riders shadows fuse_bce bce_dgrad skip_row0 cls_fold ffn_e ffn_d ln_bwd_e ln_bwd_d sched dec_tail gnorm ema "
-                            "attn_proj_e attn_proj_d")
+                            "attn_proj_e attn_proj_d kqv_head_e")
 
 
 def roll_scores(tp, pred, pos, cells):
@@ -701,6 +705,7 @@
                      o.can_ride(B * T, 3 * Dd, Dd, T) and o.can_ride(B * T, Dd, 3 * Dd, T))
         self.shadows_on_tail = True
         self.dec_tail = True
+        self.kqv_head = True
         self.n_cu = torch.cuda.get_device_properties(self.dev).multi_processor_count if self.dev.type == "cuda" else 0
         self.forms = self._resolve_forms()
         if cfg.kind == "token":
@@ -829,7 +834,9 @@
             sched=self.scheduled,
             gnorm=self.clip_global_norm > 0,
             ema=self.ema_decay > 0,
-            attn_proj_e=self._attn_proj(T, cfg.e_heads, De), attn_proj_d=not cfg.d_causal and self._attn_proj(T + 1, cfg.d_heads, Dd))
+            attn_proj_e=self._attn_proj(T, cfg.e_heads, De), attn_proj_d=not cfg.d_causal and self._attn_proj(T + 1, cfg.d_heads, Dd),
+            kqv_head_e=bool(self.kqv_head and cfg.e_layers >= 2 and o.ffn_fusion_pays(De, 4 * De) and not o.ln_bwd_fusion_pays(De) and
+                            o.kqv_head_pays(self.adt, B * T, De)))
 
     def _attn_proj(self, S, H, D):
         return bool(o.attn_bwd_form(self.adt, self.B, S, H, D // H, 0, D, 2 * D, 3 * D, D, 3 * D, proj=True)["proj"])
@@ -1109,14 +1116,14 @@
         return dict(x=L.h2, gamma=P.ln2.gamma, mean=L.mean2, rstd=L.rstd2, dgamma=P.ln2.dgamma, dbeta=P.ln2.dbeta,
                     partials=self._ln_partials(P.ln2, o.gemm_nt_ln_parts(M)), **_lead_mask(P, t, self._dropout(p, site0)))
 
-    def _layer_bwd(self, side, i, L, x_in, dy, dx_in, keymask, D, H, S, p, site0, t, dy_done=False, next_ln=None, ride=False):
+    def _layer_bwd(self, side, i, L, x_in, dy, dx_in, keymask, D, H, S, p, site0, t, dy_done=False, next_ln=None, ride=False, head=None):
         F, P = self.forms, self.store.layer(side, i)
         ffn, ln = (F.ffn_e, F.ln_bwd_e) if side == "encoder" else (F.ffn_d, F.ln_bwd_d)
         in_loss = F.dec_tail and side == "decoder" and i == self.cfg.d_layers - 1
         proj = F.attn_proj_e if side == "encoder" else F.attn_proj_d
         dff, dproj = row_block_bwd(P, L, t, dy, ALL_ROWS, self._dropout(p, site0), "fused" if ffn else ("ln_fused" if ln else "launches"),
                                    self._ln_partials, dy_done=dy_done, row_groups=self._row0_groups(side, i), launch=not in_loss,
-                                   proj_dgrad=not proj)
+                                   proj_dgrad=not proj, head=head)
         if side == "decoder" and self.cfg.d_causal:
             o.attn_causal_bwd(L.qkv, keymask, L.lse, t.datt, t.dqkv, t.delta, self.B, S, H, D // H, 0, D, 2 * D)
         elif proj:
@@ -1127,6 +1134,8 @@
         if next_ln is not None:
             kw, t_below = next_ln
             o.gemm_nt_ln_bwd(t.dqkv, P.kqv.t, t_below.dh, N=D, K=3 * D, resid=t.dh1, **kw)
+        elif side == "encoder" and i > 0 and F.kqv_head_e:
+            handed = dict(A=t.dqkv, B=P.kqv.t, resid=t.dh1, N=D, K=3 * D)
         elif ride:
             T_ = self.T
             handed = (dict(A=t.dqkv, B=P.kqv.t, C_out=dx_in, M=self.B * T_, N=D, K=3 * D, resid=t.dh1, resid_phys=True,
@@ -1140,6 +1149,7 @@
     def _top_encoder_layer_bwd(self, i, L, x_in, dx_in, next_ln=None, rider=None):
         cfg, st, B, S, F = self.cfg, self.store, self.B, self.T, self.forms
         D, H = cfg.e_model, cfg.e_heads
+        self._kqv_head = None
         P, c, rows = st.layer("encoder", i), self.top, position0_rows(B, S)
         self._tail_used["bwd"] = F.tails
         tail = None
@@ -1152,6 +1162,8 @@
         if next_ln is not None:
             kw, t_below = next_ln
             o.gemm_nt_ln_bwd(c.dqkv, P.kqv.t, t_below.dh, N=D, K=3 * D, resid=c.dh1, **kw)
+        elif i > 0 and F.kqv_head_e:
+            self._kqv_head = dict(A=c.dqkv, B=P.kqv.t, resid=c.dh1, N=D, K=3 * D)
         else:
             o.gemm_nt(c.dqkv, P.kqv.t, dx_in, N=D, K=3 * D, resid=c.dh1)
         self._wgrads += layer_wgrads(P, L, c, x_in, dff, dproj, rows)
@@ -1228,10 +1240,12 @@
         De, Se = cfg.e_model, T
         sq_e = math.sqrt(float(De))
         dy, pingpong = self.be_l[0].dx_a, (self.be_l[0].dx_b, self.be_l[0].dx_a)
+        head = self._kqv_head
         for n, i in enumerate(reversed(range(cfg.e_layers - 1))):
             x_in = self.enc[i - 1].x2 if i > 0 else self.x0_e
-            self._layer_bwd("encoder", i, self.enc[i], x_in, dy, pingpong[n % 2], self.keymask_e, De, cfg.e_heads, Se, cfg.e_dropout,
-                            self._site_e(i), self.be_l[i], dy_done=F.ln_bwd_e, next_ln=self._below("encoder", i, F.ln_bwd_e))
+            head = self._layer_bwd("encoder", i, self.enc[i], x_in, dy, pingpong[n % 2], self.keymask_e, De, cfg.e_heads, Se, cfg.e_dropout,
+                                   self._site_e(i), self.be_l[i], dy_done=F.ln_bwd_e, next_ln=self._below("encoder", i, F.ln_bwd_e),
+                                   head=head)
             dy = pingpong[n % 2]
         d_x0_e = dy
         if cfg.kind == "token":
diff --git a/musicstyletransfer_amd/ops.py b/musicstyletransfer_amd/ops.py
--- a/musicstyletransfer_amd/ops.py
+++ b/musicstyletransfer_amd/ops.py
@@ -301,15 +301,53 @@
          C.byref(l3b), C.byref(b1), C.byref(b2), C.byref(l1b), stream())
 
 
+def _kqv_head_args(A, B, C_out=None, **kw):
+    g = _gemm_args(A, B, A if C_out is None else C_out, **kw)
+    if C_out is None:
+        g.C, g.ldc = None, 0
+    return g
+
+
+def ffn_ln_bwd_head_form(head, dff, W2t, dpre_out, gate, W1t, dx_out, row_groups=None):
+    rg = {}
+    if row_groups is not None:
+        M, remap = _row_groups(dff.shape[0], row_groups)
+        rg = dict(M=M, a_remap=remap)
+    g1 = _gemm_args(dff, W2t, dpre_out, gate=gate, **rg)
+    g2 = _gemm_args(dpre_out, W1t, dx_out, **({"M": rg["M"]} if rg else {}))
+    form = (C.c_int64 * 1)()
+    call("mst_kqv_ffn_ln_bwd_form", C.byref(_kqv_head_args(**head)), C.byref(g1), C.byref(g2), form)
+    return int(form[0])
+
+
+def kqv_head_pays(dtype, M, D):
+    g = lambda m, n, k, lda, ldb, ldc: _plain_gemm_args(dtype, m, n, k, lda, ldb, ldc)
+    head = g(M, D, 3 * D, 3 * D, 3 * D, 0)
+    head.C, head.resid, head.ldr = None, 4096, D
+    form = (C.c_int64 * 1)()
+    call("mst_kqv_ffn_ln_bwd_form", C.byref(head), C.byref(g(M, 4 * D, D, D, D, 4 * D)), C.byref(g(M, D, 4 * D, 4 * D, 4 * D, D)), form)
+    return bool(form[0])
+
+
+def _plain_gemm_args(dtype, M, N, K, lda, ldb, ldc):
+    g = GemmArgs()
+    g.dtype, g.M, g.N, g.K, g.alpha = dt(dtype), M, N, K, 1.0
+    g.A, g.lda, g.B, g.ldb, g.C, g.ldc = 4096, lda, 4096, ldb, 4096, ldc
+    return g
+
+
 def ffn_ln_bwd(dff, W2t, dpre_out, gate, W1t, dx_out, x, gamma, mean, rstd, dgamma, dbeta, alpha=1.0, dx_masked=None, mask_mode=0,
-               partials=None, lead=None, row_groups=None, **kw):
+               partials=None, lead=None, row_groups=None, head=None, **kw):
     g1, g2, l = _ffn_ln_bwd_args(dff, W2t, dpre_out, gate, W1t, dx_out, x, gamma, mean, rstd, dgamma, dbeta, alpha, dx_masked, mask_mode,
                                  partials, row_groups, **kw)
     if lead is None:
+        if head is not None:
+            raise ValueError("ffn_ln_bwd(head=) computes lead's incoming gradient: it needs lead=")
         call("mst_ffn_ln_bwd", C.byref(g1), C.byref(g2), C.byref(l), stream())
         return
     q = LnBwdIn()
-    q.dy, q.ld_dy = ptr(lead["dy"]), ld(lead["dy"])
+    dy = lead.get("dy") if head is None else head.get("C_out")
+    q.dy, q.ld_dy = ptr(dy), (ld(dy) if dy is not None else 0)
     q.x, q.ld_x = ptr(lead["x"]), ld(lead["x"])
     q.gamma, q.mean, q.rstd = ptr(lead["gamma"]), ptr(lead["mean"]), ptr(lead["rstd"])
     q.dx, q.ld_dx = ptr(lead["dx"]), ld(lead["dx"])
@@ -321,6 +359,9 @@
     q.dropout_seed_ptr, q.dropout_site = ptr(lead.get("dropout_seed_ptr")), lead.get("dropout_site", 0)
     if lead.get("partials") is not None:
         assert lead["partials"].shape[0] >= gemm_nt_ln_parts(g1.M) and lead["partials"].shape[1] == 2 * g2.N
+    if head is not None:
+        call("mst_kqv_ffn_ln_bwd", C.byref(_kqv_head_args(**head)), C.byref(q), C.byref(g1), C.byref(g2), C.byref(l), stream())
+        return
     call("mst_ffn_ln_bwd_lead", C.byref(q), C.byref(g1), C.byref(g2), C.byref(l), stream())
 
 
```

Result: faster. 27.56 million frames/s, median of 6 (+1.5%).
